# ru-wang/slam-plus-plus

Measured on AMD Instinct MI355X. Metric: Λ-solve block-nnz/sec + batch GN iters/sec, Venice BA, 1→8 MI355X, higher is better.
Workload: dtype f64; 1 GPU; venice871-shaped synthetic BA (871 cams, 530304 points, 2838740 observations, LM-damped); nnzb=3369915, n=1596138, mode=schur+dense, n_reduced=5226, schur_pairs=12875640, parallelism=single GPU

## Files before the change

include/spp_hip.h:

```cpp
#ifndef SPP_HIP_H
#define SPP_HIP_H

#include <stddef.h>
#include <stdint.h>

#ifdef __cplusplus
extern "C" {
#endif

#define SPP_OK            0
#define SPP_NOT_POSDEF    1
#define SPP_E_BADARG     -1
#define SPP_E_NOMEM      -2
#define SPP_E_HIP        -3
#define SPP_E_NO_DEVICE  -4
#define SPP_E_STATE      -5
#define SPP_E_UNSUPPORTED -6

#define SPP_MODE_AUTO     0
#define SPP_MODE_SPARSE   1
#define SPP_MODE_SCHUR    2
#define SPP_MODE_SCHUR_SPARSE 3

#define SPP_FLAG_PROFILE  1
#define SPP_FLAG_SCHUR_PARTIAL 2

typedef struct spp_ctx spp_ctx;

spp_ctx *spp_create(int device, int flags);
void spp_destroy(spp_ctx *ctx);
int spp_free_memory(spp_ctx *ctx);
int spp_last_error(const spp_ctx *ctx, char *buf, size_t buf_size);
double *spp_host_staging(spp_ctx *ctx, int64_t n_doubles);
int spp_set_stream(spp_ctx *ctx, void *hip_stream);
int spp_synchronize(spp_ctx *ctx);

int spp_analyze(spp_ctx *ctx, int64_t nb, const int64_t *h_col_ptr, const int64_t *h_row_idx,
	const int64_t *h_blk_off, const int32_t *h_dim, int mode);

int spp_set_shard(spp_ctx *ctx, int rank, int world_size);

#define SPP_MODE_SCHUR_MIS 4

#define SPP_INFO_MODE           0
#define SPP_INFO_N              1
#define SPP_INFO_NNZB           2
#define SPP_INFO_NVALS          3
#define SPP_INFO_FACTOR_NNZ     4
#define SPP_INFO_FACTOR_FLOPS   5
#define SPP_INFO_N_REDUCED      6
#define SPP_INFO_N_POSES        7
#define SPP_INFO_N_LANDMARKS    8
#define SPP_INFO_SCHUR_PAIRS    9
#define SPP_INFO_N_OBS          10
#define SPP_INFO_SOLVE_BYTES    11
#define SPP_INFO_N_SUPERNODES   12
#define SPP_INFO_N_LEVELS       13
#define SPP_INFO_S_LD           14
#define SPP_INFO_S_NNZB         15
#define SPP_INFO_DENSE_STREAMED 16
#define SPP_INFO_LM_STREAM      17
#define SPP_INFO_BS_GROUPS      18
#define SPP_INFO_SCHUR_SIDE     19
#define SPP_INFO_S_CLEAR        20
#define SPP_INFO_S_DEVICE_PTR   21
#define SPP_INFO_ASM_HUB_CHUNK   22
int spp_get_info(const spp_ctx *ctx, int what, int64_t *out);
int spp_get_ordering(const spp_ctx *ctx, int64_t *h_order);
int64_t spp_sparse_fronts(const spp_ctx *ctx, int64_t capacity, int32_t *h, int32_t *w, int32_t *pad, int32_t *cls, int32_t *level,
	int32_t *parent, int32_t *team);

#define SPP_ORDER_AMD 0
#define SPP_ORDER_ND  1
int spp_block_ordering(int64_t nb, const int64_t *col_ptr, const int64_t *row_idx, int method, int64_t *h_order);

int spp_schur_plan_host(int64_t nb, const int32_t *dim, const int64_t *col_ptr, const int64_t *row_idx, int shard_rank,
	int shard_world, int sparse_S, int64_t *out, double *seconds);

int spp_factor_solve(spp_ctx *ctx, const double *h_vals, double *h_rhs_inout);

int spp_factor_solve_device(spp_ctx *ctx, const double *d_vals, double *d_rhs_inout);

int spp_schur_buffer_size(const spp_ctx *ctx, int64_t *n_doubles);
int spp_schur_form(spp_ctx *ctx, const double *d_vals, const double *d_rhs, double *d_S_rhs);
int spp_schur_finish(spp_ctx *ctx, const double *d_vals, double *d_S_rhs, double *d_rhs_inout);
int spp_schur_packed_size(const spp_ctx *ctx, int64_t *n_doubles);
int spp_schur_pack(spp_ctx *ctx, const double *d_S_rhs, double *d_packed);
int spp_schur_unpack(spp_ctx *ctx, const double *d_packed, double *d_S_rhs);

int spp_assemble_analyze(spp_ctx *ctx, int64_t nv, const int32_t *h_dim,
	int64_t ne, const int64_t *h_v0, const int64_t *h_v1, int d0, int d1, int rd,
	int64_t unary_vertex);
int spp_assemble_get_structure(const spp_ctx *ctx, int64_t *h_col_ptr, int64_t *h_row_idx,
	int64_t *h_blk_off);
int spp_assemble_device(spp_ctx *ctx, const double *d_J0, const double *d_J1,
	const double *d_Omega, const double *d_r, double damping, double *d_vals_out, double *d_eta_out);
int spp_assemble_set_edge_weights(spp_ctx *ctx, const double *d_w);
#define SPP_MAX_EDGE_GROUPS 4
int spp_assemble_analyze_groups(spp_ctx *ctx, int64_t nv, const int32_t *h_dim, int n_groups,
	const int64_t *h_ne, const int64_t *const *h_v0, const int64_t *const *h_v1, const int64_t *const *h_seq,
	const int32_t *h_d0, const int32_t *h_d1, const int32_t *h_rd, int64_t unary_vertex);
int spp_assemble_groups_device(spp_ctx *ctx, const double *const *d_J0, const double *const *d_J1,
	const double *const *d_Omega, const double *const *d_r, double damping, double *d_vals_out, double *d_eta_out);
int spp_assemble_set_group_edge_weights(spp_ctx *ctx, int group, const double *d_w);
int spp_assemble_analyze_ternary(spp_ctx *ctx, int64_t nv, const int32_t *h_dim, int64_t ne, const int64_t *h_v0,
	const int64_t *h_v1, const int64_t *h_v2, int d0, int d1, int d2, int live2, int rd, int64_t unary_vertex);
int spp_assemble_ternary_device(spp_ctx *ctx, const double *d_J0, const double *d_J1, const double *d_J2,
	const double *d_Omega, const double *d_r, double damping, double *d_vals_out, double *d_eta_out);
int spp_edge_robust_weights_device(spp_ctx *ctx, int64_t n_edges, int rd, int kind, double scale, double param,
	const double *d_r, double *d_w_out);

int spp_se2_linearize_device(spp_ctx *ctx, int64_t n_edges, const int32_t *d_v0, const int32_t *d_v1,
	const double *d_poses, const double *d_measurements, double *d_J0, double *d_J1, double *d_r);
int spp_se2_update_device(spp_ctx *ctx, int64_t n_vertices, double *d_poses, const double *d_dx, int apply,
	double *h_dx_norm2);

int spp_se2_linearize_at_device(spp_ctx *ctx, int64_t n_edges, const int64_t *d_off0, const int64_t *d_off1,
	const double *d_state, const double *d_measurements, double *d_J0, double *d_J1, double *d_r);
int spp_se2_rb_linearize_device(spp_ctx *ctx, int64_t n_edges, const int64_t *d_pose_off, const int64_t *d_lm_off,
	const double *d_state, const double *d_measurements, double *d_J0, double *d_J1, double *d_r);
int spp_slam2d_update_device(spp_ctx *ctx, int64_t n, double *d_state, const double *d_dx, int64_t n_pose_angles,
	const int64_t *d_angle_off, int apply, double *h_dx_norm2);

int spp_se3_linearize_device(spp_ctx *ctx, int64_t n_edges, const int32_t *d_v0, const int32_t *d_v1,
	const double *d_poses, const double *d_measurements, double *d_J0, double *d_J1, double *d_r);
int spp_se3_update_device(spp_ctx *ctx, int64_t n_vertices, double *d_poses, const double *d_dx, int apply,
	double *h_dx_norm2);

int spp_se3_linearize_at_device(spp_ctx *ctx, int64_t n_edges, const int64_t *d_off0, const int64_t *d_off1,
	const double *d_state, const double *d_measurements, double *d_J0, double *d_J1, double *d_r);
int spp_se3_xyz_linearize_device(spp_ctx *ctx, int64_t n_edges, const int64_t *d_pose_off, const int64_t *d_lm_off,
	const double *d_state, const double *d_measurements, double *d_J0, double *d_J1, double *d_r);
int spp_slam3d_update_device(spp_ctx *ctx, int64_t n, double *d_state, const double *d_dx, int64_t n_poses,
	const int64_t *d_pose_off, int apply, double *h_dx_norm2);

int spp_rocv_range_linearize_device(spp_ctx *ctx, int64_t n_edges, const int64_t *d_recv_off, const int64_t *d_lm_off,
	const double *d_state, const double *d_measurements, double *d_J0, double *d_J1, double *d_r);
int spp_rocv_cv_linearize_device(spp_ctx *ctx, int64_t n_edges, const int64_t *d_off0, const int64_t *d_off1,
	const double *d_state, const double *d_dt, double *d_J0, double *d_J1, double *d_r);

int spp_ba_linearize_device(spp_ctx *ctx, int64_t n_obs, const int32_t *d_cam_of, const int32_t *d_pt_of,
	const double *d_cams, const double *d_intrinsics, const double *d_points, const double *d_measurements,
	double *d_J0, double *d_J1, double *d_r);
int spp_ba_update_device(spp_ctx *ctx, int64_t n_cams, double *d_cams, const int64_t *d_cam_dxoff,
	int64_t n_points, double *d_points, const int64_t *d_pt_dxoff, const double *d_dx, int64_t n_dx, int apply,
	double *h_dx_norm2);

int spp_ba_stereo_linearize_device(spp_ctx *ctx, int64_t n_obs, const int32_t *d_cam_of, const int32_t *d_pt_of,
	const double *d_cams, const double *d_intrinsics, const double *d_points, const double *d_measurements,
	double *d_J0, double *d_J1, double *d_r);

int spp_ba_intrinsics_linearize_device(spp_ctx *ctx, int64_t n_obs, const int32_t *d_cam_of, const int32_t *d_pt_of,
	const int32_t *d_intr_of, const double *d_cams, const double *d_intrinsics, const double *d_points,
	const double *d_measurements, double *d_J0, double *d_J1, double *d_J2, double *d_r);
int spp_ba_intrinsics_update_device(spp_ctx *ctx, int64_t n_intrinsics, double *d_intrinsics, const int64_t *d_intr_dxoff,
	const double *d_dx, int apply, double *h_dx_norm2);

int spp_edge_chi2_device(spp_ctx *ctx, int64_t n_edges, int rd, const double *d_r, const double *d_Omega, double *h_chi2);
int spp_edge_hessian_maxdiag_device(spp_ctx *ctx, int64_t n_edges, int rd, int d0, int d1, const double *d_J0,
	const double *d_J1, const double *d_Omega, double *h_max);
int spp_lm_gain_denominator_device(spp_ctx *ctx, int64_t n, const double *d_dx, const double *d_eta, double alpha,
	double *h_out);

int spp_device_malloc(spp_ctx *ctx, size_t bytes, void **d_ptr);
int spp_device_free(spp_ctx *ctx, void *d_ptr);
int spp_memcpy_h2d(spp_ctx *ctx, void *d_dst, const void *h_src, size_t bytes);
int spp_memcpy_d2h(spp_ctx *ctx, void *h_dst, const void *d_src, size_t bytes);
int spp_memcpy_d2d(spp_ctx *ctx, void *d_dst, const void *d_src, size_t bytes);

int spp_set_profiling(spp_ctx *ctx, int on);

#define SPP_PHASE_PERMUTE   0
#define SPP_PHASE_SCHUR_INV 1
#define SPP_PHASE_SCHUR_GEMM 2
#define SPP_PHASE_SCHUR_RHS 3
#define SPP_PHASE_FACTOR    4
#define SPP_PHASE_TRISOLVE  5
#define SPP_PHASE_BACKSUBST 6
#define SPP_PHASE_ASSEMBLE  7
#define SPP_PHASE_TOTAL     8
#define SPP_N_PHASES        9
int spp_get_phase_ms(spp_ctx *ctx, double *ms_out );
int spp_get_dominant_kernel(spp_ctx *ctx, double *ms_total, int64_t *n_launches, double *flops);

int spp_microbench_copy(spp_ctx *ctx, size_t bytes, int iters, double *gb_per_s);
int spp_microbench_mfma_f64(spp_ctx *ctx, int iters, double *tflops);
int spp_microbench_ctile(spp_ctx *ctx, int n, int iters, double *gb_per_s);
int spp_microbench_update(spp_ctx *ctx, int64_t m, int iters, double *ms_per_launch);

int spp_dense_potrf_upper(spp_ctx *ctx, double *d_A, int64_t n, int64_t ld);
int spp_dense_posv(spp_ctx *ctx, double *d_A, int64_t n, int64_t ld, double *d_b);
int spp_dense_posv_masked(spp_ctx *ctx, double *d_A, int64_t n, int64_t ld, double *d_b, const uint64_t *words, int64_t nwords);
int spp_tile_mask_host(int64_t n, int bs, int64_t nblk, const int32_t *i1, const int32_t *i2, int has_rhs, int fill,
	uint64_t *words, int64_t *n_updates);
int spp_schur_tile_mask_host(int64_t nb, const int32_t *dim, const int64_t *col_ptr, const int64_t *row_idx, int shard_rank,
	int shard_world, uint64_t *words);
int spp_schur_cam_order_host(int64_t nb, const int32_t *dim, const int64_t *col_ptr, const int64_t *row_idx, int shard_rank,
	int shard_world, int flags, const int64_t *order_in, int64_t *cam_order, double *figures);
int spp_tail_order_host(int64_t n, int has_rhs, const uint64_t *words, int64_t nwords, int resident, int early, double beta,
	int32_t *table, int32_t *info);
int spp_dense_gemm_tn_sub(spp_ctx *ctx, int64_t m, int64_t n, int64_t k,
	const double *d_A, int64_t lda, const double *d_B, int64_t ldb, double *d_C, int64_t ldc);
int spp_dense_gemm_tn_sub_upper(spp_ctx *ctx, int64_t m, int64_t n, int64_t k,
	const double *d_A, int64_t lda, const double *d_B, int64_t ldb, double *d_C, int64_t ldc);
int spp_dense_front_factor(spp_ctx *ctx, double *d_F, int64_t ld, int64_t w, int64_t h, double *d_image);

const char *spp_version(void);

#ifdef __cplusplus
}
#endif
#endif
```

slam_plus_plus_amd/api.py:

```python
import ctypes
import os

import numpy as np

_HERE = os.path.dirname(os.path.abspath(__file__))
LIB_PATH = os.environ.get("SPP_LIB") or os.path.join(_HERE, "libspp_hip.so")

SPP_OK, SPP_NOT_POSDEF = 0, 1
MODE_AUTO, MODE_SPARSE, MODE_SCHUR, MODE_SCHUR_SPARSE, MODE_SCHUR_MIS = 0, 1, 2, 3, 4
FLAG_PROFILE = 1
INFO = dict(MODE=0, N=1, NNZB=2, NVALS=3, FACTOR_NNZ=4, FACTOR_FLOPS=5, N_REDUCED=6, N_POSES=7,
            N_LANDMARKS=8, SCHUR_PAIRS=9, N_OBS=10, SOLVE_BYTES=11, N_SUPERNODES=12, N_LEVELS=13, S_LD=14, S_NNZB=15, DENSE_STREAMED=16,
            LM_STREAM=17, BS_GROUPS=18, SCHUR_SIDE=19, S_CLEAR=20, S_DEVICE_PTR=21, ASM_HUB_CHUNK=22)
PHASES = ["permute", "schur_inv", "schur_gemm", "schur_rhs", "factor", "trisolve", "backsubst", "assemble", "total"]

EXPORTS = [
    "spp_create", "spp_destroy", "spp_free_memory", "spp_last_error", "spp_host_staging", "spp_set_stream", "spp_synchronize",
    "spp_analyze", "spp_set_shard", "spp_get_info", "spp_get_ordering", "spp_sparse_fronts", "spp_factor_solve",
    "spp_factor_solve_device", "spp_schur_buffer_size", "spp_schur_form", "spp_schur_finish",
    "spp_schur_packed_size", "spp_schur_pack", "spp_schur_unpack",
    "spp_assemble_analyze", "spp_assemble_get_structure", "spp_assemble_device", "spp_assemble_set_edge_weights",
    "spp_assemble_analyze_groups", "spp_assemble_groups_device", "spp_assemble_set_group_edge_weights",
    "spp_assemble_analyze_ternary", "spp_assemble_ternary_device", "spp_ba_intrinsics_linearize_device",
    "spp_ba_intrinsics_update_device",
    "spp_se2_linearize_at_device", "spp_se2_rb_linearize_device", "spp_slam2d_update_device",
    "spp_se3_linearize_at_device", "spp_se3_xyz_linearize_device", "spp_slam3d_update_device", "spp_rocv_range_linearize_device",
    "spp_rocv_cv_linearize_device", "spp_device_malloc",
    "spp_device_free", "spp_memcpy_h2d", "spp_memcpy_d2h", "spp_memcpy_d2d", "spp_get_phase_ms", "spp_get_dominant_kernel",
    "spp_microbench_copy", "spp_microbench_mfma_f64", "spp_microbench_ctile", "spp_microbench_update", "spp_block_ordering", "spp_schur_plan_host", "spp_set_profiling", "spp_se2_linearize_device", "spp_se2_update_device", "spp_ba_linearize_device", "spp_ba_stereo_linearize_device", "spp_ba_update_device", "spp_se3_linearize_device", "spp_se3_update_device", "spp_edge_chi2_device", "spp_edge_robust_weights_device", "spp_edge_hessian_maxdiag_device",
    "spp_lm_gain_denominator_device", "spp_dense_potrf_upper", "spp_dense_posv",
    "spp_dense_posv_masked", "spp_tile_mask_host", "spp_schur_tile_mask_host", "spp_tail_order_host", "spp_schur_cam_order_host",
    "spp_dense_gemm_tn_sub", "spp_dense_gemm_tn_sub_upper", "spp_dense_front_factor", "spp_version",
]

_lib = None
_c_i64p = ctypes.POINTER(ctypes.c_int64)
_c_i32p = ctypes.POINTER(ctypes.c_int32)
_c_f64p = ctypes.POINTER(ctypes.c_double)


class SppError(RuntimeError):
    """std::runtime_error of the C++ adapter (reference LinearSolver_Schur_GPU.cpp:734-797)."""


def load_library():
    global _lib
    if _lib is not None:
        return _lib
    if not os.path.exists(LIB_PATH):
        raise SppError("libspp_hip.so is not built: run `python -m slam_plus_plus_amd.build` "
                       "(hipcc --offload-arch=gfx950); there is no CPU fallback")
    lib = ctypes.CDLL(LIB_PATH)
    vp, i64, i32, dbl, cint = ctypes.c_void_p, ctypes.c_int64, ctypes.c_int32, ctypes.c_double, ctypes.c_int
    sig = {
        "spp_create": (vp, [cint, cint]),
        "spp_destroy": (None, [vp]),
        "spp_free_memory": (cint, [vp]),
        "spp_last_error": (cint, [vp, ctypes.c_char_p, ctypes.c_size_t]),
        "spp_host_staging": (vp, [vp, i64]),
        "spp_set_stream": (cint, [vp, vp]),
        "spp_synchronize": (cint, [vp]),
        "spp_analyze": (cint, [vp, i64, vp, vp, vp, vp, cint]),
        "spp_set_shard": (cint, [vp, cint, cint]),
        "spp_get_info": (cint, [vp, cint, _c_i64p]),
        "spp_get_ordering": (cint, [vp, vp]),
        "spp_sparse_fronts": (i64, [vp, i64, vp, vp, vp, vp, vp, vp, vp]),
        "spp_factor_solve": (cint, [vp, vp, vp]),
        "spp_factor_solve_device": (cint, [vp, vp, vp]),
        "spp_schur_buffer_size": (cint, [vp, _c_i64p]),
        "spp_schur_form": (cint, [vp, vp, vp, vp]),
        "spp_schur_finish": (cint, [vp, vp, vp, vp]),
        "spp_schur_packed_size": (cint, [vp, _c_i64p]),
        "spp_schur_pack": (cint, [vp, vp, vp]),
        "spp_schur_unpack": (cint, [vp, vp, vp]),
        "spp_assemble_analyze": (cint, [vp, i64, vp, i64, vp, vp, cint, cint, cint, i64]),
        "spp_assemble_get_structure": (cint, [vp, vp, vp, vp]),
        "spp_assemble_device": (cint, [vp, vp, vp, vp, vp, dbl, vp, vp]),
        "spp_assemble_set_edge_weights": (cint, [vp, vp]),
        "spp_assemble_analyze_groups": (cint, [vp, i64, vp, cint, vp, vp, vp, vp, vp, vp, vp, i64]),
        "spp_assemble_groups_device": (cint, [vp, vp, vp, vp, vp, dbl, vp, vp]),
        "spp_assemble_set_group_edge_weights": (cint, [vp, cint, vp]),
        "spp_assemble_analyze_ternary": (cint, [vp, i64, vp, i64, vp, vp, vp, cint, cint, cint, cint, cint, i64]),
        "spp_assemble_ternary_device": (cint, [vp, vp, vp, vp, vp, vp, dbl, vp, vp]),
        "spp_ba_intrinsics_linearize_device": (cint, [vp, i64, vp, vp, vp, vp, vp, vp, vp, vp, vp, vp, vp]),
        "spp_ba_intrinsics_update_device": (cint, [vp, i64, vp, vp, vp, cint, _c_f64p]),
        "spp_se2_linearize_at_device": (cint, [vp, i64, vp, vp, vp, vp, vp, vp, vp]),
        "spp_se2_rb_linearize_device": (cint, [vp, i64, vp, vp, vp, vp, vp, vp, vp]),
        "spp_slam2d_update_device": (cint, [vp, i64, vp, vp, i64, vp, cint, _c_f64p]),
        "spp_se3_linearize_at_device": (cint, [vp, i64, vp, vp, vp, vp, vp, vp, vp]),
        "spp_se3_xyz_linearize_device": (cint, [vp, i64, vp, vp, vp, vp, vp, vp, vp]),
        "spp_slam3d_update_device": (cint, [vp, i64, vp, vp, i64, vp, cint, _c_f64p]),
        "spp_rocv_range_linearize_device": (cint, [vp, i64, vp, vp, vp, vp, vp, vp, vp]),
        "spp_rocv_cv_linearize_device": (cint, [vp, i64, vp, vp, vp, vp, vp, vp, vp]),
        "spp_device_malloc": (cint, [vp, ctypes.c_size_t, ctypes.POINTER(vp)]),
        "spp_device_free": (cint, [vp, vp]),
        "spp_memcpy_h2d": (cint, [vp, vp, vp, ctypes.c_size_t]),
        "spp_memcpy_d2h": (cint, [vp, vp, vp, ctypes.c_size_t]),
        "spp_memcpy_d2d": (cint, [vp, vp, vp, ctypes.c_size_t]),
        "spp_get_phase_ms": (cint, [vp, _c_f64p]),
        "spp_get_dominant_kernel": (cint, [vp, _c_f64p, _c_i64p, _c_f64p]),
        "spp_microbench_copy": (cint, [vp, ctypes.c_size_t, cint, _c_f64p]),
        "spp_microbench_mfma_f64": (cint, [vp, cint, _c_f64p]),
        "spp_microbench_ctile": (cint, [vp, cint, cint, _c_f64p]),
        "spp_microbench_update": (cint, [vp, ctypes.c_int64, cint, _c_f64p]),
        "spp_block_ordering": (cint, [ctypes.c_int64, vp, vp, cint, vp]),
        "spp_schur_plan_host": (cint, [ctypes.c_int64, vp, vp, vp, cint, cint, cint, vp, vp]),
        "spp_set_profiling": (cint, [vp, cint]),
        "spp_se2_linearize_device": (cint, [vp, ctypes.c_int64, vp, vp, vp, vp, vp, vp, vp]),
        "spp_se2_update_device": (cint, [vp, ctypes.c_int64, vp, vp, cint, _c_f64p]),
        "spp_se3_linearize_device": (cint, [vp, ctypes.c_int64, vp, vp, vp, vp, vp, vp, vp]),
        "spp_se3_update_device": (cint, [vp, ctypes.c_int64, vp, vp, cint, _c_f64p]),
        "spp_edge_chi2_device": (cint, [vp, ctypes.c_int64, cint, vp, vp, _c_f64p]),
        "spp_edge_robust_weights_device": (cint, [vp, ctypes.c_int64, cint, cint, dbl, dbl, vp, vp]),
        "spp_edge_hessian_maxdiag_device": (cint, [vp, ctypes.c_int64, cint, cint, cint, vp, vp, vp, _c_f64p]),
        "spp_lm_gain_denominator_device": (cint, [vp, ctypes.c_int64, vp, vp, ctypes.c_double, _c_f64p]),
        "spp_ba_linearize_device": (cint, [vp, ctypes.c_int64, vp, vp, vp, vp, vp, vp, vp, vp, vp]),
        "spp_ba_stereo_linearize_device": (cint, [vp, ctypes.c_int64, vp, vp, vp, vp, vp, vp, vp, vp, vp]),
        "spp_ba_update_device": (cint, [vp, ctypes.c_int64, vp, vp, ctypes.c_int64, vp, vp, vp, ctypes.c_int64, cint, _c_f64p]),
        "spp_dense_potrf_upper": (cint, [vp, vp, i64, i64]),
        "spp_dense_posv": (cint, [vp, vp, i64, i64, vp]),
        "spp_dense_posv_masked": (cint, [vp, vp, i64, i64, vp, vp, i64]),
        "spp_tile_mask_host": (cint, [i64, cint, i64, vp, vp, cint, cint, vp, vp]),
        "spp_schur_tile_mask_host": (cint, [i64, vp, vp, vp, cint, cint, vp]),
        "spp_tail_order_host": (cint, [i64, cint, vp, i64, cint, cint, dbl, vp, vp]),
        "spp_schur_cam_order_host": (cint, [i64, vp, vp, vp, cint, cint, cint, vp, vp, vp]),
        "spp_dense_gemm_tn_sub": (cint, [vp, i64, i64, i64, vp, i64, vp, i64, vp, i64]),
        "spp_dense_gemm_tn_sub_upper": (cint, [vp, i64, i64, i64, vp, i64, vp, i64, vp, i64]),
        "spp_dense_front_factor": (cint, [vp, vp, i64, i64, i64, vp]),
        "spp_version": (ctypes.c_char_p, []),
    }
    for name, (res, args) in sig.items():
        fn = getattr(lib, name)
        fn.restype = res
        fn.argtypes = args
    _lib = lib
    return lib


def _ptr(a):
    return a.ctypes.data_as(ctypes.c_void_p)


ORDER_AMD, ORDER_ND = 0, 1


def block_ordering(lam, method=ORDER_AMD):
    lib = load_library()
    col_ptr = np.ascontiguousarray(lam.col_ptr, dtype=np.int64)
    row_idx = np.ascontiguousarray(lam.row_idx, dtype=np.int64)
    out = np.empty(lam.nb, dtype=np.int64)
    code = lib.spp_block_ordering(lam.nb, _ptr(col_ptr), _ptr(row_idx), method, _ptr(out))
    if code != 0:
        raise SppError("spp_block_ordering failed: %d" % code)
    return out


def schur_plan_host(lam, shard_rank=0, shard_world=1, sparse_S=False, mis=False):
    lib = load_library()
    col_ptr = np.ascontiguousarray(lam.col_ptr, dtype=np.int64)
    row_idx = np.ascontiguousarray(lam.row_idx, dtype=np.int64)
    dim = np.ascontiguousarray(lam.dim, dtype=np.int32)
    out = np.zeros(9, dtype=np.int64)
    sec = ctypes.c_double(0.0)
    code = lib.spp_schur_plan_host(lam.nb, _ptr(dim), _ptr(col_ptr), _ptr(row_idx), shard_rank, shard_world,
                                   (1 if sparse_S else 0) | (2 if mis else 0), _ptr(out), ctypes.byref(sec))
    if code != 0:
# ... 435 lines not shown
```

slam_plus_plus_amd/csrc/spp_api.cpp:

```cpp

#include "spp_internal.h"
#include <string.h>
#include <new>

using namespace spp;

namespace spp {

void phases_reset(spp_ctx *ctx)
{
	if(!(ctx->flags & SPP_FLAG_PROFILE))
		return;
	if(!ctx->timer.created) {
		for(int i = 0; i < 2 * SPP_N_PHASES; ++ i)
			SPP_HIP_CHECK(hipEventCreate(&ctx->timer.ev[i]));
		ctx->timer.created = true;
	}
	for(int i = 0; i < SPP_N_PHASES; ++ i) {
		ctx->timer.used[i] = false;
		ctx->phase_ms[i] = 0;
	}
	ctx->dom_used = 0;
	ctx->dom_flops = 0;
}

void phase_begin(spp_ctx *ctx, int phase)
{
	if(!(ctx->flags & SPP_FLAG_PROFILE) || !ctx->timer.created)
		return;
	SPP_HIP_CHECK(hipEventRecord(ctx->timer.ev[2 * phase], ctx->stream));
}

void phase_end(spp_ctx *ctx, int phase)
{
	if(!(ctx->flags & SPP_FLAG_PROFILE) || !ctx->timer.created)
		return;
	SPP_HIP_CHECK(hipEventRecord(ctx->timer.ev[2 * phase + 1], ctx->stream));
	ctx->timer.used[phase] = true;
}

void phases_collect(spp_ctx *ctx)
{
	if(!(ctx->flags & SPP_FLAG_PROFILE) || !ctx->timer.created)
		return;
	SPP_HIP_CHECK(hipStreamSynchronize(ctx->stream));
	for(int i = 0; i < SPP_N_PHASES; ++ i) {
		if(!ctx->timer.used[i])
			continue;
		float ms = 0;
		if(hipEventElapsedTime(&ms, ctx->timer.ev[2 * i], ctx->timer.ev[2 * i + 1]) == hipSuccess)
			ctx->phase_ms[i] = ms;
	}
}

void dom_begin(spp_ctx *ctx)
{
	if(!(ctx->flags & SPP_FLAG_PROFILE))
		return;
	if(ctx->dom_used + 2 > ctx->dom_events.size()) {
		size_t old = ctx->dom_events.size();
		ctx->dom_events.resize(old + 64);
		for(size_t i = old; i < ctx->dom_events.size(); ++ i)
			SPP_HIP_CHECK(hipEventCreate(&ctx->dom_events[i]));
	}
	SPP_HIP_CHECK(hipEventRecord(ctx->dom_events[ctx->dom_used], ctx->stream));
}

void dom_end(spp_ctx *ctx, double flops)
{
	if(!(ctx->flags & SPP_FLAG_PROFILE))
		return;
	SPP_HIP_CHECK(hipEventRecord(ctx->dom_events[ctx->dom_used + 1], ctx->stream));
	ctx->dom_used += 2;
	ctx->dom_flops += flops;
}

}

#define SPP_TRY(ctx) try {
#define SPP_CATCH(ctx) } catch(const spp::Error &e) { if(ctx) (ctx)->last_error = e.what(); return e.code; } \
	catch(const std::bad_alloc &) { if(ctx) (ctx)->last_error = "host allocation failed"; return SPP_E_NOMEM; } \
	catch(const std::exception &e) { if(ctx) (ctx)->last_error = e.what(); return SPP_E_HIP; }

static inline void store_if(double *h_out, double value)
{
	if(h_out)
		*h_out = value;
}

template <class Body>
static int geometry_call(spp_ctx *ctx, Body body)
{
	SPP_TRY(ctx)
	SPP_HIP_CHECK(hipSetDevice(ctx->device));
	body();
	return SPP_OK;
	SPP_CATCH(ctx)
}

extern "C" {

const char *spp_version(void)
{
	return "slam_plus_plus_amd 0.1 (gfx950, fp64)";
}

spp_ctx *spp_create(int device, int flags)
{
	int count = 0;
	if(hipGetDeviceCount(&count) != hipSuccess || count <= 0 || device < 0 || device >= count)
		return nullptr;
	if(hipSetDevice(device) != hipSuccess)
		return nullptr;
	spp_ctx *ctx = new(std::nothrow) spp_ctx;
	if(!ctx)
		return nullptr;
	ctx->device = device;
	ctx->flags = flags;
	if(hipStreamCreateWithFlags(&ctx->stream, hipStreamNonBlocking) != hipSuccess) {
		delete ctx;
		return nullptr;
	}
	ctx->own_stream = true;
	return ctx;
}

int spp_free_memory(spp_ctx *ctx)
{
	if(!ctx)
		return SPP_E_BADARG;
	SPP_TRY(ctx)
	(void)hipSetDevice(ctx->device);
	(void)hipStreamSynchronize(ctx->stream);
	ctx->schur.release_all();
	sparse_release(ctx);
	assemble_release(ctx);
	ctx->dense.tinv.release();
	ctx->dense.tinv_all.release();
	ctx->dense.xtmp.release();
	ctx->dense.la_cnt.release();
	ctx->dense.la_trace.release();
	ctx->geom_partial.release();
	ctx->dense.flags.release();
	ctx->dense.trsv_pay.release();
	ctx->dense.trsv_m.release();
	ctx->dense.tail_pub.release();
	ctx->dense.tail_order.release();
	ctx->dense.tail_order_tr = ctx->dense.tail_order_tc = 0;
	ctx->dense.tail_order_bits.clear();
	ctx->dense.tail_dinv.release();
	ctx->dense.tail_epoch = 0;
	ctx->dense.epoch = 0;
	ctx->dense.sync.release();
	ctx->dense.fuse_cnt.release();
	ctx->dense.fuse_expect.clear();
	ctx->dense.sync_epoch = 0;
	ctx->d_vals.release();
	ctx->d_rhs.release();
	ctx->mode = -1;
	return SPP_OK;
	SPP_CATCH(ctx)
}

void spp_destroy(spp_ctx *ctx)
{
	if(!ctx)
		return;
	if(ctx->plan_trash.joinable())
		ctx->plan_trash.join();
	spp_free_memory(ctx);
	ctx->dense.info.release();
	if(ctx->dense.aux) {
		dense_aux_park(ctx->device, ctx->dense.aux);
		(void)hipEventDestroy(ctx->dense.ev[0]);
		(void)hipEventDestroy(ctx->dense.ev[1]);
	}
	if(ctx->dense.chain) {
		(void)hipStreamDestroy(ctx->dense.chain);
		if(ctx->dense.ev_chain)
			(void)hipEventDestroy(ctx->dense.ev_chain);
	}
	if(ctx->side_stream) {
		(void)hipStreamDestroy(ctx->side_stream);
		(void)hipEventDestroy(ctx->side_ev[0]);
		(void)hipEventDestroy(ctx->side_ev[1]);
	}
	if(ctx->dense.h_chain_err)
		(void)hipHostFree(ctx->dense.h_chain_err);
	if(ctx->h_staging)
		(void)hipHostFree(ctx->h_staging);
	if(ctx->timer.created)
		for(int i = 0; i < 2 * SPP_N_PHASES; ++ i)
			(void)hipEventDestroy(ctx->timer.ev[i]);
	for(size_t i = 0; i < ctx->dom_events.size(); ++ i)
		(void)hipEventDestroy(ctx->dom_events[i]);
	if(ctx->own_stream && ctx->stream)
		(void)hipStreamDestroy(ctx->stream);
	delete ctx;
}

int spp_last_error(const spp_ctx *ctx, char *buf, size_t buf_size)
{
	if(!ctx || !buf || !buf_size)
		return SPP_E_BADARG;
	strncpy(buf, ctx->last_error.c_str(), buf_size - 1);
	buf[buf_size - 1] = 0;
	return SPP_OK;
}

double *spp_host_staging(spp_ctx *ctx, int64_t n_doubles)
{
	if(!ctx || n_doubles < 0)
		return nullptr;
	if((size_t)n_doubles <= ctx->h_staging_cap && ctx->h_staging)
		return ctx->h_staging;
	(void)hipSetDevice(ctx->device);
	(void)hipStreamSynchronize(ctx->stream);
	if(ctx->h_staging) {
		(void)hipHostFree(ctx->h_staging);
		ctx->h_staging = nullptr;
		ctx->h_staging_cap = 0;
	}
	const size_t want = (size_t)(n_doubles > 0 ? n_doubles : 1);
	if(hipHostMalloc((void**)&ctx->h_staging, want * sizeof(double), hipHostMallocDefault) != hipSuccess) {
		(void)hipGetLastError();
		ctx->h_staging = nullptr;
		ctx->last_error = "hipHostMalloc of the staging buffer failed";
		return nullptr;
	}
	ctx->h_staging_cap = want;
	return ctx->h_staging;
}

int spp_set_stream(spp_ctx *ctx, void *hip_stream)
{
	if(!ctx)
		return SPP_E_BADARG;
	(void)hipStreamSynchronize(ctx->stream);
	if(ctx->own_stream && ctx->stream)
		(void)hipStreamDestroy(ctx->stream);
	ctx->stream = (hipStream_t)hip_stream;
	ctx->own_stream = false;
	return SPP_OK;
}

int spp_synchronize(spp_ctx *ctx)
{
	if(!ctx)
		return SPP_E_BADARG;
	SPP_TRY(ctx)
	SPP_HIP_CHECK(hipStreamSynchronize(ctx->stream));
	dense_chain_check(ctx);
	return SPP_OK;
	SPP_CATCH(ctx)
}

int spp_set_profiling(spp_ctx *ctx, int on)
{
	if(!ctx)
		return SPP_E_BADARG;
	ctx->flags = on ? (ctx->flags | SPP_FLAG_PROFILE) : (ctx->flags & ~SPP_FLAG_PROFILE);
	return SPP_OK;
}

int spp_set_shard(spp_ctx *ctx, int rank, int world_size)
{
	if(!ctx || world_size < 1 || rank < 0 || rank >= world_size)
		return SPP_E_BADARG;
	ctx->shard_rank = rank;
	ctx->shard_world = world_size;
	return SPP_OK;
}

int spp_analyze(spp_ctx *ctx, int64_t nb, const int64_t *col_ptr, const int64_t *row_idx,
	const int64_t *blk_off, const int32_t *dim, int mode)
{
	if(!ctx)
		return SPP_E_BADARG;
	SPP_TRY(ctx)
	SPP_REQUIRE(nb > 0 && col_ptr && row_idx && blk_off && dim, SPP_E_BADARG, "spp_analyze: null or empty structure");
	SPP_REQUIRE(col_ptr[0] == 0 && col_ptr[nb] >= nb, SPP_E_BADARG, "spp_analyze: column pointers must start at 0 and hold every diagonal block");
	SPP_HIP_CHECK(hipSetDevice(ctx->device));
	ctx->mode = -1;
	VClock clk("spp_analyze");
	Structure st;
	st.nb = nb;
	st.nnzb = col_ptr[nb];
	st.col_ptr.assign(col_ptr, col_ptr + nb + 1);
	SPP_REQUIRE(st.nnzb >= nb, SPP_E_BADARG, "spp_analyze: fewer blocks than block columns");
	for(int64_t j = 0; j < nb; ++ j)
		SPP_REQUIRE(col_ptr[j + 1] > col_ptr[j], SPP_E_BADARG, "every block column needs its diagonal block");
	st.dim.assign(dim, dim + nb);
	st.base.resize(nb + 1);
	st.base[0] = 0;
	for(int64_t j = 0; j < nb; ++ j) {
		SPP_REQUIRE(dim[j] > 0 && dim[j] <= 8, SPP_E_BADARG, "block widths must be in 1..8");
		st.base[j + 1] = st.base[j] + dim[j];
	}
	st.n = st.base[nb];
	st.row_idx.resize(st.nnzb);
	st.blk_off.resize(st.nnzb);
	{
		const int nt = plan_threads(st.nnzb);
		std::vector<int64_t> jcut, nvals_t(nt, 0);
		balanced_cuts(st.col_ptr, nt, jcut);
		run_threads(nt, [&](int t) {
			const int64_t p0 = col_ptr[jcut[t]], p1 = col_ptr[jcut[t + 1]];
			if(p1 > p0) {
				memcpy(st.row_idx.data() + p0, row_idx + p0, (size_t)(p1 - p0) * sizeof(int64_t));
				memcpy(st.blk_off.data() + p0, blk_off + p0, (size_t)(p1 - p0) * sizeof(int64_t));
			}
			int64_t nv = 0;
			for(int64_t j = jcut[t]; j < jcut[t + 1]; ++ j) {
				for(int64_t p = col_ptr[j]; p < col_ptr[j + 1]; ++ p) {
					const int64_t i = row_idx[p];
					SPP_REQUIRE(i >= 0 && i <= j, SPP_E_BADARG, "only the upper triangle may be stored");
					SPP_REQUIRE(p == col_ptr[j] || row_idx[p - 1] < i, SPP_E_BADARG, "rows must ascend within a column");
					SPP_REQUIRE(blk_off[p] >= 0, SPP_E_BADARG, "negative block offset");
					nv = std::max<int64_t>(nv, blk_off[p] + (int64_t)dim[i] * dim[j]);
				}
				SPP_REQUIRE(row_idx[col_ptr[j + 1] - 1] == j, SPP_E_BADARG, "diagonal block missing (must be last in its column)");
			}
			nvals_t[t] = nv;
		});
		st.nvals = 0;
		for(int t = 0; t < nt; ++ t)
			st.nvals = std::max(st.nvals, nvals_t[t]);
	}
	ctx->st = std::move(st);
	Structure &st_ref = ctx->st;
	clk.lap("structure copied + validated");
	ctx->schur.release_all();
	sparse_release(ctx);
	clk.lap("old plans released");
	int dp, dl;
	int chosen = mode;
	if(mode == SPP_MODE_AUTO) {
		chosen = SPP_MODE_SPARSE;
		if(schur_applicable(st_ref, &dp, &dl)) {
			int64_t n_red = 0;
			for(int64_t j = 0; j < nb; ++ j)
				n_red += (dim[j] == dp) ? dp : 0;
			chosen = (n_red <= 16384) ? SPP_MODE_SCHUR : SPP_MODE_SCHUR_SPARSE;
		}
	}
	SPP_REQUIRE(chosen == SPP_MODE_SCHUR || chosen == SPP_MODE_SPARSE || chosen == SPP_MODE_SCHUR_SPARSE ||
		chosen == SPP_MODE_SCHUR_MIS, SPP_E_BADARG, "unknown mode");
	SPP_REQUIRE((chosen != SPP_MODE_SPARSE && chosen != SPP_MODE_SCHUR_MIS) || ctx->shard_world == 1, SPP_E_UNSUPPORTED,
		"only the Schur modes shard (over landmarks); pose graphs run as replicas (DESIGN.md, multi-GPU)");
	ctx->mode = -1;
	if(chosen == SPP_MODE_SCHUR || chosen == SPP_MODE_SCHUR_SPARSE || chosen == SPP_MODE_SCHUR_MIS) {
		const bool mis = chosen == SPP_MODE_SCHUR_MIS;
		const bool sparse_S = chosen != SPP_MODE_SCHUR;
		build_schur_plan(ctx, sparse_S, mis);
		clk.lap("schur plan (all of it)");
		ctx->schur.mis = mis;
		ctx->order.clear();
		ctx->order.reserve((size_t)st_ref.nb);
		if(sparse_S) {
			sparse_analyze(ctx, ctx->schur.s_st);
			std::vector<int64_t> red = ctx->order;
			ctx->order.clear();
			for(size_t i = 0; i < red.size(); ++ i)
				ctx->order.push_back(ctx->schur.pose_block[red[i]]);
			chosen = SPP_MODE_SCHUR;
		} else
		for(size_t i = 0; i < ctx->schur.pose_block.size(); ++ i)
			ctx->order.push_back(ctx->schur.pose_block[i]);
		for(int64_t j = 0; j < st_ref.nb; ++ j)
			if(ctx->schur.is_lm[j])
				ctx->order.push_back(j);
	} else
		sparse_analyze(ctx, ctx->st);
	ctx->mode = chosen;
	clk.lap("plan + ordering");
	return SPP_OK;
	SPP_CATCH(ctx)
}

int spp_get_info(const spp_ctx *ctx, int what, int64_t *out)
{
	if(!ctx || !out)
		return SPP_E_BADARG;
	if(ctx->mode < 0 && what != SPP_INFO_NNZB && what != SPP_INFO_NVALS && what != SPP_INFO_N && what != SPP_INFO_DENSE_STREAMED &&
	   what != SPP_INFO_ASM_HUB_CHUNK)
		return SPP_E_STATE;
	switch(what) {
	case SPP_INFO_MODE: *out = (ctx->mode != SPP_MODE_SCHUR) ? ctx->mode : ctx->schur.mis ? SPP_MODE_SCHUR_MIS :
		ctx->schur.sparse_S ? SPP_MODE_SCHUR_SPARSE : SPP_MODE_SCHUR; break;
	case SPP_INFO_N: *out = ctx->st.n; break;
	case SPP_INFO_NNZB: *out = ctx->st.nnzb; break;
	case SPP_INFO_NVALS: *out = ctx->st.nvals; break;
	case SPP_INFO_FACTOR_NNZ: *out = ctx->factor_nnz; break;
	case SPP_INFO_FACTOR_FLOPS: *out = ctx->factor_flops; break;
	case SPP_INFO_N_REDUCED: *out = (ctx->mode == SPP_MODE_SCHUR) ? ctx->schur.n_red : 0; break;
	case SPP_INFO_N_POSES: *out = (ctx->mode == SPP_MODE_SCHUR) ? ctx->schur.nc : ctx->st.nb; break;
	case SPP_INFO_N_LANDMARKS: *out = (ctx->mode == SPP_MODE_SCHUR) ? ctx->schur.nl : 0; break;
	case SPP_INFO_SCHUR_PAIRS: *out = (ctx->mode == SPP_MODE_SCHUR) ? ctx->schur.n_pairs : 0; break;
	case SPP_INFO_N_OBS: *out = (ctx->mode == SPP_MODE_SCHUR) ? ctx->schur.no : 0; break;
	case SPP_INFO_SOLVE_BYTES: *out = ctx->solve_bytes; break;
	case SPP_INFO_N_SUPERNODES: *out = ctx->sparse ? sparse_info(ctx, what) : 0; break;
	case SPP_INFO_N_LEVELS: *out = ctx->sparse ? sparse_info(ctx, what) : 0; break;
	case SPP_INFO_S_LD: *out = (ctx->mode == SPP_MODE_SCHUR && !ctx->schur.sparse_S) ? ctx->schur.ld : 0; break;
	case SPP_INFO_S_NNZB: *out = (ctx->mode == SPP_MODE_SCHUR) ? ctx->schur.n_sblk : 0; break;
	case SPP_INFO_DENSE_STREAMED: *out = ctx->dense.tail_rows_last; break;
	case SPP_INFO_LM_STREAM: *out = (ctx->mode == SPP_MODE_SCHUR) ? ctx->schur.lm_stream_last : 0; break;
	case SPP_INFO_BS_GROUPS: *out = (ctx->mode == SPP_MODE_SCHUR) ? ctx->schur.n_bs : 0; break;
	case SPP_INFO_SCHUR_SIDE: *out = (ctx->mode == SPP_MODE_SCHUR) ? ctx->schur.side_last : 0; break;
	case SPP_INFO_S_CLEAR: *out = (ctx->mode == SPP_MODE_SCHUR) ? ctx->schur.clear_last : 0; break;
	case SPP_INFO_S_DEVICE_PTR: *out = (ctx->mode == SPP_MODE_SCHUR) ? (int64_t)(uintptr_t)ctx->schur.S.p : 0; break;
	case SPP_INFO_ASM_HUB_CHUNK: *out = ASM_HUB_CHUNK; break;
	default: return SPP_E_BADARG;
	}
	return SPP_OK;
}

int spp_get_ordering(const spp_ctx *ctx, int64_t *h_order)
{
	if(!ctx || !h_order)
		return SPP_E_BADARG;
	if(ctx->mode < 0)
		return SPP_E_STATE;
	for(size_t i = 0; i < ctx->order.size(); ++ i)
		h_order[i] = ctx->order[i];
	return SPP_OK;
}

int64_t spp_sparse_fronts(const spp_ctx *ctx, int64_t capacity, int32_t *h, int32_t *w, int32_t *pad, int32_t *cls, int32_t *level,
	int32_t *parent, int32_t *team)
{
	if(!ctx || capacity < 0)
		return SPP_E_BADARG;
#ifdef SPP_HAVE_SPARSE
	if(ctx->sparse)
		return sparse_fronts(ctx, capacity, h, w, pad, cls, level, parent, team);
#endif
	return 0;
}

int spp_block_ordering(int64_t nb, const int64_t *col_ptr, const int64_t *row_idx, int method, int64_t *h_order)
{
	if(nb <= 0 || !col_ptr || !row_idx || !h_order || (method != SPP_ORDER_AMD && method != SPP_ORDER_ND))
		return SPP_E_BADARG;
	try {
		for(int64_t j = 0; j < nb; ++ j)
			for(int64_t p = col_ptr[j]; p < col_ptr[j + 1]; ++ p)
				if(row_idx[p] < 0 || row_idx[p] > j)
					return SPP_E_BADARG;
		std::vector<int64_t> order;
		if(method == SPP_ORDER_AMD)
			min_degree_order(nb, col_ptr, row_idx, order);
		else
			nested_dissection_order(nb, col_ptr, row_idx, order);
		for(int64_t k = 0; k < nb; ++ k)
			h_order[k] = order[k];
		return SPP_OK;
	} catch(const std::bad_alloc &) {
		return SPP_E_NOMEM;
	} catch(...) {
		return SPP_E_HIP;
	}
}

static bool structure_of_pattern(int64_t nb, const int32_t *dim, const int64_t *col_ptr, const int64_t *row_idx, Structure &st)
{
	st.nb = nb;
	st.nnzb = col_ptr[nb];
	st.col_ptr.assign(col_ptr, col_ptr + nb + 1);
	st.row_idx.assign(row_idx, row_idx + st.nnzb);
	st.dim.assign(dim, dim + nb);
	st.base.resize(nb + 1);
	st.base[0] = 0;
	for(int64_t j = 0; j < nb; ++ j)
		st.base[j + 1] = st.base[j] + dim[j];
	st.n = st.base[nb];
	st.blk_off.resize(st.nnzb);
	int64_t off = 0;
	for(int64_t j = 0; j < nb; ++ j)
		for(int64_t p = col_ptr[j]; p < col_ptr[j + 1]; ++ p) {
			if(row_idx[p] < 0 || row_idx[p] > j)
				return false;
			st.blk_off[p] = off;
			off += (int64_t)dim[row_idx[p]] * dim[j];
		}
	st.nvals = off;
	return true;
}

extern "C++" {
template <class F>
static int schur_host_entry(int64_t nb, const int32_t *dim, const int64_t *col_ptr, const int64_t *row_idx, int shard_rank,
	int shard_world, const void *out, F fn)
{
	if(nb <= 0 || !dim || !col_ptr || !row_idx || !out || shard_world < 1 || shard_rank < 0 || shard_rank >= shard_world)
		return SPP_E_BADARG;
	try {
		Structure st;
		if(!structure_of_pattern(nb, dim, col_ptr, row_idx, st))
			return SPP_E_BADARG;
		return fn(st);
	} catch(const Error &e) {
		return e.code;
	} catch(const std::bad_alloc &) {
		return SPP_E_NOMEM;
	} catch(...) {
		return SPP_E_HIP;
	}
}
}

int spp_schur_plan_host(int64_t nb, const int32_t *dim, const int64_t *col_ptr, const int64_t *row_idx, int shard_rank,
	int shard_world, int sparse_S, int64_t *out, double *seconds)
{
	return schur_host_entry(nb, dim, col_ptr, row_idx, shard_rank, shard_world, out, [&](const Structure &st) {
		const double sec = schur_plan_host_probe(st, shard_rank, shard_world, (sparse_S & 1) != 0, (sparse_S & 2) != 0, out);
		if(seconds)
			*seconds = sec;
		return (int)SPP_OK;
	});
}

int spp_schur_tile_mask_host(int64_t nb, const int32_t *dim, const int64_t *col_ptr, const int64_t *row_idx, int shard_rank,
	int shard_world, uint64_t *words)
{
	return schur_host_entry(nb, dim, col_ptr, row_idx, shard_rank, shard_world, words, [&](const Structure &st) {
		std::vector<uint64_t> w;
		schur_tile_mask_host_probe(st, w);
		for(size_t q = 0; q < w.size(); ++ q)
			words[q] = w[q];
		return (int)w.size();
	});
}

int spp_schur_cam_order_host(int64_t nb, const int32_t *dim, const int64_t *col_ptr, const int64_t *row_idx, int shard_rank,
	int shard_world, int flags, const int64_t *order_in, int64_t *cam_order, double *figures)
{
	if(!figures)
		return SPP_E_BADARG;
	return schur_host_entry(nb, dim, col_ptr, row_idx, shard_rank, shard_world, cam_order, [&](const Structure &st) {
		if(order_in) {
			int64_t nc = 0;
			const int dmax = *std::max_element(dim, dim + nb);
			for(int64_t j = 0; j < nb; ++ j)
				nc += dim[j] == dmax;
			std::vector<char> seen((size_t)nc, 0);
			for(int64_t q = 0; q < nc; ++ q) {
				if(order_in[q] < 0 || order_in[q] >= nc || seen[order_in[q]])
					return (int)SPP_E_BADARG;
				seen[order_in[q]] = 1;
			}
		}
		std::vector<int32_t> order;
		TileDagCost cost[2];
		const bool used = schur_cam_order_host_probe(st, shard_rank, shard_world, (flags & 1) != 0, (flags & 2) != 0, order_in, order, cost);
		for(size_t q = 0; q < order.size(); ++ q)
			cam_order[q] = order[q];
		for(int side = 0; side < 2; ++ side) {
			figures[4 * side] = (double)cost[side].tiles;
			figures[4 * side + 1] = (double)cost[side].updates;
			figures[4 * side + 2] = (double)cost[side].path;
			figures[4 * side + 3] = cost[side].cost_us;
		}
		return used ? 1 : 0;
	});
}

int spp_schur_buffer_size(const spp_ctx *ctx, int64_t *n_doubles)
{
	if(!ctx || !n_doubles)
		return SPP_E_BADARG;
	if(ctx->mode != SPP_MODE_SCHUR)
		return SPP_E_STATE;
	*n_doubles = schur_buffer_doubles(ctx);
	return SPP_OK;
}

int spp_schur_form(spp_ctx *ctx, const double *d_vals, const double *d_rhs, double *d_S_rhs)
{
	if(!ctx || !d_vals || !d_rhs || !d_S_rhs)
		return SPP_E_BADARG;
	SPP_TRY(ctx)
	SPP_REQUIRE(ctx->mode == SPP_MODE_SCHUR, SPP_E_STATE, "spp_schur_form: analyze in Schur mode first");
	SPP_HIP_CHECK(hipSetDevice(ctx->device));
	phases_reset(ctx);
	phase_begin(ctx, SPP_PHASE_TOTAL);
	schur_form(ctx, d_vals, d_rhs, d_S_rhs);
	return SPP_OK;
	SPP_CATCH(ctx)
}

int spp_schur_packed_size(const spp_ctx *ctx, int64_t *n_doubles)
{
	if(!ctx || !n_doubles)
		return SPP_E_BADARG;
	if(ctx->mode != SPP_MODE_SCHUR)
		return SPP_E_STATE;
	if(ctx->schur.sparse_S) {
		*n_doubles = schur_buffer_doubles(ctx);
		return SPP_OK;
	}
	const int64_t nblk = ctx->schur.ld / DENSE_NB;
	*n_doubles = (int64_t)DENSE_NB * DENSE_NB * (nblk * (nblk + 1) / 2);
	return SPP_OK;
}

int spp_schur_pack(spp_ctx *ctx, const double *d_S_rhs, double *d_packed)
{
	if(!ctx || !d_S_rhs || !d_packed)
		return SPP_E_BADARG;
	SPP_TRY(ctx)
	SPP_REQUIRE(ctx->mode == SPP_MODE_SCHUR, SPP_E_STATE, "spp_schur_pack: analyze in Schur mode first");
	SPP_HIP_CHECK(hipSetDevice(ctx->device));
	if(ctx->schur.sparse_S)
		SPP_HIP_CHECK(hipMemcpyAsync(d_packed, d_S_rhs, (size_t)schur_buffer_doubles(ctx) * sizeof(double),
			hipMemcpyDeviceToDevice, ctx->stream));
	else
		schur_pack(ctx, const_cast<double*>(d_S_rhs), d_packed, true);
	return SPP_OK;
	SPP_CATCH(ctx)
}

int spp_schur_unpack(spp_ctx *ctx, const double *d_packed, double *d_S_rhs)
{
	if(!ctx || !d_S_rhs || !d_packed)
		return SPP_E_BADARG;
	SPP_TRY(ctx)
	SPP_REQUIRE(ctx->mode == SPP_MODE_SCHUR, SPP_E_STATE, "spp_schur_unpack: analyze in Schur mode first");
	SPP_HIP_CHECK(hipSetDevice(ctx->device));
	if(ctx->schur.sparse_S)
		SPP_HIP_CHECK(hipMemcpyAsync(d_S_rhs, d_packed, (size_t)schur_buffer_doubles(ctx) * sizeof(double),
			hipMemcpyDeviceToDevice, ctx->stream));
	else
		schur_pack(ctx, d_S_rhs, const_cast<double*>(d_packed), false);
	return SPP_OK;
	SPP_CATCH(ctx)
}

int spp_schur_finish(spp_ctx *ctx, const double *d_vals, double *d_S_rhs, double *d_rhs_inout)
{
	if(!ctx || !d_vals || !d_rhs_inout || !d_S_rhs)
		return SPP_E_BADARG;
	SPP_TRY(ctx)
	SPP_REQUIRE(ctx->mode == SPP_MODE_SCHUR, SPP_E_STATE, "spp_schur_finish: analyze in Schur mode first");
	SPP_HIP_CHECK(hipSetDevice(ctx->device));
	int ret = schur_finish(ctx, d_vals, d_S_rhs, d_rhs_inout);
	phase_end(ctx, SPP_PHASE_TOTAL);
	phases_collect(ctx);
	dense_chain_check(ctx);
	return ret;
	SPP_CATCH(ctx)
}

int spp_factor_solve_device(spp_ctx *ctx, const double *d_vals, double *d_rhs)
{
	if(!ctx || !d_vals || !d_rhs)
		return SPP_E_BADARG;
	SPP_TRY(ctx)
	SPP_REQUIRE(ctx->mode >= 0, SPP_E_STATE, "spp_factor_solve: call spp_analyze first");
	SPP_HIP_CHECK(hipSetDevice(ctx->device));
	phases_reset(ctx);
	phase_begin(ctx, SPP_PHASE_TOTAL);
	int ret;
	if(ctx->mode == SPP_MODE_SCHUR) {
		SPP_REQUIRE(ctx->shard_world == 1, SPP_E_STATE,
			"sharded ctx: use spp_schur_form / all-reduce / spp_schur_finish");
		if(!ctx->schur.S.p || ctx->schur.S.cap < (size_t)schur_buffer_doubles(ctx))
			ctx->schur.unlisted_dirty = true;
		ctx->schur.S.reserve((size_t)schur_buffer_doubles(ctx));
		schur_form(ctx, d_vals, d_rhs, ctx->schur.S.p, true);
		ret = schur_finish(ctx, d_vals, ctx->schur.S.p, d_rhs);
	} else
		ret = sparse_factor_solve(ctx, d_vals, d_rhs);
	phase_end(ctx, SPP_PHASE_TOTAL);
	phases_collect(ctx);
	SPP_HIP_CHECK(hipStreamSynchronize(ctx->stream));
	dense_chain_check(ctx);
	return ret;
	SPP_CATCH(ctx)
}

int spp_factor_solve(spp_ctx *ctx, const double *h_vals, double *h_rhs)
{
	if(!ctx || !h_vals || !h_rhs)
		return SPP_E_BADARG;
	SPP_TRY(ctx)
	SPP_REQUIRE(ctx->mode >= 0, SPP_E_STATE, "spp_factor_solve: call spp_analyze first");
	SPP_HIP_CHECK(hipSetDevice(ctx->device));
	ctx->d_vals.reserve((size_t)ctx->st.nvals);
	ctx->d_rhs.reserve((size_t)ctx->st.n);
	SPP_HIP_CHECK(hipMemcpyAsync(ctx->d_vals.p, h_vals, ctx->st.nvals * sizeof(double), hipMemcpyHostToDevice, ctx->stream));
	SPP_HIP_CHECK(hipMemcpyAsync(ctx->d_rhs.p, h_rhs, ctx->st.n * sizeof(double), hipMemcpyHostToDevice, ctx->stream));
	int ret = spp_factor_solve_device(ctx, ctx->d_vals.p, ctx->d_rhs.p);
	if(ret != SPP_OK)
		return ret;
	SPP_HIP_CHECK(hipMemcpyAsync(h_rhs, ctx->d_rhs.p, ctx->st.n * sizeof(double), hipMemcpyDeviceToHost, ctx->stream));
	SPP_HIP_CHECK(hipStreamSynchronize(ctx->stream));
	return SPP_OK;
	SPP_CATCH(ctx)
}

int spp_assemble_analyze(spp_ctx *ctx, int64_t nv, const int32_t *h_dim, int64_t ne, const int64_t *h_v0,
	const int64_t *h_v1, int d0, int d1, int rd, int64_t unary_vertex)
{
	if(!ctx)
		return SPP_E_BADARG;
	assemble_release(ctx);
	if(!h_dim || !h_v0 || !h_v1 || nv <= 0 || ne <= 0)
		return SPP_E_BADARG;
	SPP_TRY(ctx)
	SPP_HIP_CHECK(hipSetDevice(ctx->device));
	assemble_analyze(ctx, nv, h_dim, 1, &ne, &h_v0, &h_v1, nullptr, &d0, &d1, &rd, unary_vertex);
	return SPP_OK;
	SPP_CATCH(ctx)
}

int spp_assemble_analyze_groups(spp_ctx *ctx, int64_t nv, const int32_t *h_dim, int n_groups, const int64_t *h_ne,
	const int64_t *const *h_v0, const int64_t *const *h_v1, const int64_t *const *h_seq, const int32_t *h_d0,
	const int32_t *h_d1, const int32_t *h_rd, int64_t unary_vertex)
{
	if(!ctx)
		return SPP_E_BADARG;
	assemble_release(ctx);
	if(!h_dim || nv <= 0 || n_groups <= 0 || !h_ne || !h_v0 || !h_v1 || !h_d0 || !h_d1 || !h_rd)
		return SPP_E_BADARG;
	SPP_TRY(ctx)
	SPP_HIP_CHECK(hipSetDevice(ctx->device));
	SPP_REQUIRE(n_groups <= SPP_MAX_EDGE_GROUPS, SPP_E_UNSUPPORTED, "more than SPP_MAX_EDGE_GROUPS edge groups");
	int64_t total = 0;
	for(int g = 0; g < n_groups; ++ g) {
		SPP_REQUIRE(h_ne[g] >= 0 && (!h_ne[g] || (h_v0[g] && (h_v1[g] || h_d1[g] == 0))), SPP_E_BADARG, "edge group without vertex arrays");
		total += h_ne[g];
	}
	SPP_REQUIRE(total > 0, SPP_E_BADARG, "no edges");
	assemble_analyze(ctx, nv, h_dim, n_groups, h_ne, h_v0, h_v1, h_seq, h_d0, h_d1, h_rd, unary_vertex);
	return SPP_OK;
	SPP_CATCH(ctx)
}

int spp_assemble_get_structure(const spp_ctx *ctx, int64_t *h_col_ptr, int64_t *h_row_idx, int64_t *h_blk_off)
{
	if(!ctx || !ctx->assemble)
		return SPP_E_STATE;
	assemble_get_structure(ctx, h_col_ptr, h_row_idx, h_blk_off);
	return SPP_OK;
}

int spp_assemble_device(spp_ctx *ctx, const double *d_J0, const double *d_J1, const double *d_Omega,
	const double *d_r, double damping, double *d_vals_out, double *d_eta_out)
{
	if(!ctx || !d_J0 || !d_J1 || !d_Omega || !d_r || !d_vals_out || !d_eta_out)
		return SPP_E_BADARG;
	SPP_TRY(ctx)
	SPP_REQUIRE(ctx->assemble, SPP_E_STATE, "spp_assemble_device: call spp_assemble_analyze first");
	SPP_REQUIRE(assemble_n_groups(ctx) == 1, SPP_E_STATE, "spp_assemble_device: the plan has several edge groups (spp_assemble_groups_device)");
	SPP_REQUIRE(!assemble_is_ternary(ctx), SPP_E_STATE, "spp_assemble_device: the plan is one of ternary edges (spp_assemble_ternary_device)");
	SPP_REQUIRE(!assemble_group_is_unary(ctx, 0), SPP_E_STATE, "spp_assemble_device: the plan is one of unary edges (spp_assemble_groups_device)");
	SPP_HIP_CHECK(hipSetDevice(ctx->device));
	phases_reset(ctx);
	phase_begin(ctx, SPP_PHASE_ASSEMBLE);
	assemble_run(ctx, d_J0, d_J1, d_Omega, d_r, damping, d_vals_out, d_eta_out);
	phase_end(ctx, SPP_PHASE_ASSEMBLE);
	phases_collect(ctx);
	return SPP_OK;
	SPP_CATCH(ctx)
}

int spp_assemble_groups_device(spp_ctx *ctx, const double *const *d_J0, const double *const *d_J1,
	const double *const *d_Omega, const double *const *d_r, double damping, double *d_vals_out, double *d_eta_out)
{
	if(!ctx || !d_J0 || !d_J1 || !d_Omega || !d_r || !d_vals_out || !d_eta_out)
		return SPP_E_BADARG;
	SPP_TRY(ctx)
	SPP_REQUIRE(ctx->assemble, SPP_E_STATE, "spp_assemble_groups_device: call spp_assemble_analyze_groups first");
	SPP_REQUIRE(!assemble_is_ternary(ctx), SPP_E_STATE, "spp_assemble_groups_device: the plan is one of ternary edges (spp_assemble_ternary_device)");
	for(int g = 0; g < assemble_n_groups(ctx); ++ g)
		SPP_REQUIRE(!assemble_group_edges(ctx, g) || (d_J0[g] && (d_J1[g] || assemble_group_is_unary(ctx, g)) && d_Omega[g] && d_r[g]), SPP_E_BADARG,
			"spp_assemble_groups_device: null array of an edge group");
	SPP_HIP_CHECK(hipSetDevice(ctx->device));
	phases_reset(ctx);
	phase_begin(ctx, SPP_PHASE_ASSEMBLE);
	assemble_groups_run(ctx, d_J0, d_J1, d_Omega, d_r, damping, d_vals_out, d_eta_out);
	phase_end(ctx, SPP_PHASE_ASSEMBLE);
	phases_collect(ctx);
	return SPP_OK;
	SPP_CATCH(ctx)
}

int spp_assemble_analyze_ternary(spp_ctx *ctx, int64_t nv, const int32_t *h_dim, int64_t ne, const int64_t *h_v0,
	const int64_t *h_v1, const int64_t *h_v2, int d0, int d1, int d2, int live2, int rd, int64_t unary_vertex)
{
	if(!ctx)
		return SPP_E_BADARG;
	assemble_release(ctx);
	if(!h_dim || !h_v0 || !h_v1 || !h_v2 || nv <= 0 || ne <= 0)
		return SPP_E_BADARG;
	SPP_TRY(ctx)
	SPP_REQUIRE(d0 == 6 && d1 == 3 && d2 == 6 && live2 == 5 && rd == 2, SPP_E_UNSUPPORTED,
		"ternary edge shape (d0, d1, d2, rd) / live2 not instantiated: (6,3,6,2) / 5");
	SPP_HIP_CHECK(hipSetDevice(ctx->device));
	assemble_analyze_ternary(ctx, nv, h_dim, ne, h_v0, h_v1, h_v2, unary_vertex);
	return SPP_OK;
	SPP_CATCH(ctx)
}

int spp_assemble_ternary_device(spp_ctx *ctx, const double *d_J0, const double *d_J1, const double *d_J2,
	const double *d_Omega, const double *d_r, double damping, double *d_vals_out, double *d_eta_out)
{
	if(!ctx || !d_J0 || !d_J1 || !d_J2 || !d_Omega || !d_r || !d_vals_out || !d_eta_out)
		return SPP_E_BADARG;
	SPP_TRY(ctx)
	SPP_REQUIRE(ctx->assemble && assemble_is_ternary(ctx), SPP_E_STATE, "spp_assemble_ternary_device: call spp_assemble_analyze_ternary first");
	SPP_HIP_CHECK(hipSetDevice(ctx->device));
	phases_reset(ctx);
	phase_begin(ctx, SPP_PHASE_ASSEMBLE);
	assemble_ternary_run(ctx, d_J0, d_J1, d_J2, d_Omega, d_r, damping, d_vals_out, d_eta_out);
	phase_end(ctx, SPP_PHASE_ASSEMBLE);
	phases_collect(ctx);
	return SPP_OK;
	SPP_CATCH(ctx)
}

int spp_ba_intrinsics_linearize_device(spp_ctx *ctx, int64_t n_obs, const int32_t *d_cam_of, const int32_t *d_pt_of,
	const int32_t *d_intr_of, const double *d_cams, const double *d_intrinsics, const double *d_points,
	const double *d_measurements, double *d_J0, double *d_J1, double *d_J2, double *d_r)
{
	if(!ctx || n_obs < 0 || !d_cam_of || !d_pt_of || !d_intr_of || !d_cams || !d_intrinsics || !d_points || !d_measurements ||
	   !d_J0 || !d_J1 || !d_J2 || !d_r)
		return SPP_E_BADARG;
	return geometry_call(ctx, [&] {
		ba_intrinsics_linearize(ctx, n_obs, d_cam_of, d_pt_of, d_intr_of, d_cams, d_intrinsics, d_points, d_measurements, d_J0, d_J1,
			d_J2, d_r);
	});
}

int spp_ba_intrinsics_update_device(spp_ctx *ctx, int64_t n_intrinsics, double *d_intrinsics, const int64_t *d_intr_dxoff,
	const double *d_dx, int apply, double *h_dx_norm2)
{
	if(!ctx || n_intrinsics < 0 || !d_dx || (n_intrinsics && (!d_intrinsics || !d_intr_dxoff)))
		return SPP_E_BADARG;
	return geometry_call(ctx, [&] { store_if(h_dx_norm2, ba_intrinsics_update(ctx, n_intrinsics, d_intrinsics, d_intr_dxoff, d_dx, apply != 0)); });
}

int spp_assemble_set_edge_weights(spp_ctx *ctx, const double *d_w)
{
	if(!ctx)
		return SPP_E_BADARG;
	SPP_TRY(ctx)
	SPP_REQUIRE(ctx->assemble, SPP_E_STATE, "spp_assemble_set_edge_weights: call spp_assemble_analyze first");
	SPP_REQUIRE(!assemble_is_ternary(ctx), SPP_E_UNSUPPORTED, "robust weights on ternary edges");
// ... 63 lines not shown
	return geometry_call(ctx, [&] { se3_linearize(ctx, n_edges, d_v0, d_v1, d_poses, d_measurements, d_J0, d_J1, d_r); });
}

int spp_se3_update_device(spp_ctx *ctx, int64_t n_vertices, double *d_poses, const double *d_dx, int apply,
	double *h_dx_norm2)
{
	if(!ctx || n_vertices < 0 || !d_poses || !d_dx)
		return SPP_E_BADARG;
	return geometry_call(ctx, [&] { store_if(h_dx_norm2, se3_update(ctx, n_vertices, d_poses, d_dx, apply != 0)); });
}

int spp_ba_linearize_device(spp_ctx *ctx, int64_t n_obs, const int32_t *d_cam_of, const int32_t *d_pt_of,
	const double *d_cams, const double *d_intrinsics, const double *d_points, const double *d_measurements,
	double *d_J0, double *d_J1, double *d_r)
{
	if(!ctx || n_obs < 0 || !d_cam_of || !d_pt_of || !d_cams || !d_intrinsics || !d_points || !d_measurements ||
	   !d_J0 || !d_J1 || !d_r)
		return SPP_E_BADARG;
	return geometry_call(ctx, [&] { ba_linearize(ctx, n_obs, d_cam_of, d_pt_of, d_cams, d_intrinsics, d_points, d_measurements, d_J0, d_J1, d_r); });
}

int spp_ba_stereo_linearize_device(spp_ctx *ctx, int64_t n_obs, const int32_t *d_cam_of, const int32_t *d_pt_of,
	const double *d_cams, const double *d_intrinsics, const double *d_points, const double *d_measurements,
	double *d_J0, double *d_J1, double *d_r)
{
	if(!ctx || n_obs < 0 || !d_cam_of || !d_pt_of || !d_cams || !d_intrinsics || !d_points || !d_measurements ||
	   !d_J0 || !d_J1 || !d_r)
		return SPP_E_BADARG;
	return geometry_call(ctx, [&] { ba_stereo_linearize(ctx, n_obs, d_cam_of, d_pt_of, d_cams, d_intrinsics, d_points, d_measurements, d_J0, d_J1, d_r); });
}

int spp_ba_update_device(spp_ctx *ctx, int64_t n_cams, double *d_cams, const int64_t *d_cam_dxoff,
	int64_t n_points, double *d_points, const int64_t *d_pt_dxoff, const double *d_dx, int64_t n_dx, int apply,
	double *h_dx_norm2)
{
	if(!ctx || n_cams < 0 || n_points < 0 || n_dx < 0 || !d_dx || (n_cams && (!d_cams || !d_cam_dxoff)) ||
	   (n_points && (!d_points || !d_pt_dxoff)))
		return SPP_E_BADARG;
	return geometry_call(ctx, [&] { store_if(h_dx_norm2, ba_update(ctx, n_cams, d_cams, d_cam_dxoff, n_points, d_points, d_pt_dxoff, d_dx, n_dx, apply != 0)); });
}

int spp_edge_robust_weights_device(spp_ctx *ctx, int64_t n_edges, int rd, int kind, double scale, double param,
	const double *d_r, double *d_w_out)
{
	if(!ctx || n_edges < 0 || !d_r || !d_w_out)
		return SPP_E_BADARG;
	return geometry_call(ctx, [&] { edge_robust_weights(ctx, n_edges, rd, kind, scale, param, d_r, d_w_out); });
}

int spp_se3_linearize_at_device(spp_ctx *ctx, int64_t n_edges, const int64_t *d_off0, const int64_t *d_off1,
	const double *d_state, const double *d_measurements, double *d_J0, double *d_J1, double *d_r)
{
	if(!ctx || n_edges < 0 || !d_off0 || !d_off1 || !d_state || !d_measurements || !d_J0 || !d_J1 || !d_r)
		return SPP_E_BADARG;
	return geometry_call(ctx, [&] { se3_linearize_at(ctx, n_edges, d_off0, d_off1, d_state, d_measurements, d_J0, d_J1, d_r); });
}

int spp_se3_xyz_linearize_device(spp_ctx *ctx, int64_t n_edges, const int64_t *d_pose_off, const int64_t *d_lm_off,
	const double *d_state, const double *d_measurements, double *d_J0, double *d_J1, double *d_r)
{
	if(!ctx || n_edges < 0 || !d_pose_off || !d_lm_off || !d_state || !d_measurements || !d_J0 || !d_J1 || !d_r)
		return SPP_E_BADARG;
	return geometry_call(ctx, [&] { se3_xyz_linearize(ctx, n_edges, d_pose_off, d_lm_off, d_state, d_measurements, d_J0, d_J1, d_r); });
}

int spp_slam3d_update_device(spp_ctx *ctx, int64_t n, double *d_state, const double *d_dx, int64_t n_poses,
	const int64_t *d_pose_off, int apply, double *h_dx_norm2)
{
	if(!ctx || n < 0 || n_poses < 0 || !d_state || !d_dx || (n_poses && !d_pose_off))
		return SPP_E_BADARG;
	return geometry_call(ctx, [&] { store_if(h_dx_norm2, slam3d_update(ctx, n, d_state, d_dx, n_poses, d_pose_off, apply != 0)); });
}

int spp_rocv_range_linearize_device(spp_ctx *ctx, int64_t n_edges, const int64_t *d_recv_off, const int64_t *d_lm_off,
	const double *d_state, const double *d_measurements, double *d_J0, double *d_J1, double *d_r)
{
	if(!ctx || n_edges < 0 || !d_recv_off || !d_lm_off || !d_state || !d_measurements || !d_J0 || !d_J1 || !d_r)
		return SPP_E_BADARG;
	return geometry_call(ctx, [&] { rocv_range_linearize(ctx, n_edges, d_recv_off, d_lm_off, d_state, d_measurements, d_J0, d_J1, d_r); });
}

int spp_rocv_cv_linearize_device(spp_ctx *ctx, int64_t n_edges, const int64_t *d_off0, const int64_t *d_off1,
	const double *d_state, const double *d_dt, double *d_J0, double *d_J1, double *d_r)
{
	if(!ctx || n_edges < 0 || !d_off0 || !d_off1 || !d_state || !d_dt || !d_J0 || !d_J1 || !d_r)
		return SPP_E_BADARG;
	return geometry_call(ctx, [&] { rocv_cv_linearize(ctx, n_edges, d_off0, d_off1, d_state, d_dt, d_J0, d_J1, d_r); });
}

int spp_edge_chi2_device(spp_ctx *ctx, int64_t n_edges, int rd, const double *d_r, const double *d_Omega, double *h_chi2)
{
	if(!ctx || n_edges < 0 || !d_r || !d_Omega || !h_chi2)
		return SPP_E_BADARG;
	return geometry_call(ctx, [&] { *h_chi2 = edge_chi2(ctx, n_edges, rd, d_r, d_Omega); });
}

int spp_edge_hessian_maxdiag_device(spp_ctx *ctx, int64_t n_edges, int rd, int d0, int d1, const double *d_J0,
	const double *d_J1, const double *d_Omega, double *h_max)
{
	if(!ctx || n_edges < 0 || !d_J0 || !d_J1 || !d_Omega || !h_max)
		return SPP_E_BADARG;
	return geometry_call(ctx, [&] { *h_max = edge_hessian_maxdiag(ctx, n_edges, rd, d0, d1, d_J0, d_J1, d_Omega); });
}

int spp_lm_gain_denominator_device(spp_ctx *ctx, int64_t n, const double *d_dx, const double *d_eta, double alpha,
	double *h_out)
{
	if(!ctx || n < 0 || !d_dx || !d_eta || !h_out)
		return SPP_E_BADARG;
	return geometry_call(ctx, [&] { *h_out = lm_gain_denominator(ctx, n, d_dx, d_eta, alpha); });
}

int spp_device_malloc(spp_ctx *ctx, size_t bytes, void **d_ptr)
{
	if(!ctx || !d_ptr)
		return SPP_E_BADARG;
	(void)hipSetDevice(ctx->device);
	if(hipMalloc(d_ptr, bytes ? bytes : 8) != hipSuccess) {
		ctx->last_error = "hipMalloc failed";
		return SPP_E_NOMEM;
	}
	return SPP_OK;
}

int spp_device_free(spp_ctx *ctx, void *d_ptr)
{
	if(!ctx)
		return SPP_E_BADARG;
	(void)hipSetDevice(ctx->device);
	(void)hipStreamSynchronize(ctx->stream);
	return hipFree(d_ptr) == hipSuccess ? SPP_OK : SPP_E_HIP;
}

int spp_memcpy_h2d(spp_ctx *ctx, void *d_dst, const void *h_src, size_t bytes)
{
	if(!ctx)
		return SPP_E_BADARG;
	SPP_TRY(ctx)
	SPP_HIP_CHECK(hipSetDevice(ctx->device));
	SPP_HIP_CHECK(hipMemcpyAsync(d_dst, h_src, bytes, hipMemcpyHostToDevice, ctx->stream));
	SPP_HIP_CHECK(hipStreamSynchronize(ctx->stream));
	return SPP_OK;
	SPP_CATCH(ctx)
}

int spp_memcpy_d2h(spp_ctx *ctx, void *h_dst, const void *d_src, size_t bytes)
{
	if(!ctx)
		return SPP_E_BADARG;
	SPP_TRY(ctx)
	SPP_HIP_CHECK(hipSetDevice(ctx->device));
	SPP_HIP_CHECK(hipMemcpyAsync(h_dst, d_src, bytes, hipMemcpyDeviceToHost, ctx->stream));
	SPP_HIP_CHECK(hipStreamSynchronize(ctx->stream));
	return SPP_OK;
	SPP_CATCH(ctx)
}

int spp_memcpy_d2d(spp_ctx *ctx, void *d_dst, const void *d_src, size_t bytes)
{
	if(!ctx)
		return SPP_E_BADARG;
	SPP_TRY(ctx)
	SPP_HIP_CHECK(hipSetDevice(ctx->device));
	SPP_HIP_CHECK(hipMemcpyAsync(d_dst, d_src, bytes, hipMemcpyDeviceToDevice, ctx->stream));
	return SPP_OK;
	SPP_CATCH(ctx)
}

int spp_get_phase_ms(spp_ctx *ctx, double *ms_out)
{
	if(!ctx || !ms_out)
		return SPP_E_BADARG;
	for(int i = 0; i < SPP_N_PHASES; ++ i)
		ms_out[i] = ctx->phase_ms[i];
	return SPP_OK;
}

int spp_get_dominant_kernel(spp_ctx *ctx, double *ms_total, int64_t *n_launches, double *flops)
{
	if(!ctx || !ms_total || !n_launches || !flops)
		return SPP_E_BADARG;
	SPP_TRY(ctx)
	SPP_HIP_CHECK(hipStreamSynchronize(ctx->stream));
	double total = 0;
	for(size_t i = 0; i + 1 < ctx->dom_used; i += 2) {
		float ms = 0;
		SPP_HIP_CHECK(hipEventElapsedTime(&ms, ctx->dom_events[i], ctx->dom_events[i + 1]));
		total += ms;
	}
	*ms_total = total;
	*n_launches = (int64_t)(ctx->dom_used / 2);
	*flops = ctx->dom_flops;
	return SPP_OK;
	SPP_CATCH(ctx)
}

int spp_microbench_copy(spp_ctx *ctx, size_t bytes, int iters, double *gb_per_s)
{
	if(!ctx || !gb_per_s)
		return SPP_E_BADARG;
	SPP_TRY(ctx)
	SPP_HIP_CHECK(hipSetDevice(ctx->device));
	*gb_per_s = microbench_copy(ctx, bytes, iters);
	return SPP_OK;
	SPP_CATCH(ctx)
}

int spp_microbench_ctile(spp_ctx *ctx, int n, int iters, double *gb_per_s)
{
	if(!ctx || !gb_per_s)
		return SPP_E_BADARG;
	SPP_TRY(ctx)
	SPP_HIP_CHECK(hipSetDevice(ctx->device));
	*gb_per_s = microbench_ctile(ctx, n, iters);
	return SPP_OK;
	SPP_CATCH(ctx)
}

int spp_microbench_update(spp_ctx *ctx, int64_t m, int iters, double *ms_per_launch)
{
	if(!ctx || !ms_per_launch || m < 128 || iters < 1)
		return SPP_E_BADARG;
	SPP_TRY(ctx)
	SPP_HIP_CHECK(hipSetDevice(ctx->device));
	*ms_per_launch = microbench_update(ctx, m, iters);
	return SPP_OK;
	SPP_CATCH(ctx)
}

int spp_microbench_mfma_f64(spp_ctx *ctx, int iters, double *tflops)
{
	if(!ctx || !tflops)
		return SPP_E_BADARG;
	SPP_TRY(ctx)
	SPP_HIP_CHECK(hipSetDevice(ctx->device));
	*tflops = microbench_mfma_f64(ctx, iters);
	return SPP_OK;
	SPP_CATCH(ctx)
}

int spp_dense_potrf_upper(spp_ctx *ctx, double *d_A, int64_t n, int64_t ld)
{
	if(!ctx || !d_A || n <= 0 || ld < n)
		return SPP_E_BADARG;
	SPP_TRY(ctx)
	SPP_HIP_CHECK(hipSetDevice(ctx->device));
	const int64_t ldp = ((n + 1 + DENSE_NB - 1) / DENSE_NB) * DENSE_NB;
	DevBuf<double> tmp;
	tmp.reserve((size_t)ldp * ldp);
	SPP_HIP_CHECK(hipMemsetAsync(tmp.p, 0, (size_t)ldp * ldp * sizeof(double), ctx->stream));
	SPP_HIP_CHECK(hipMemcpy2DAsync(tmp.p, ldp * sizeof(double), d_A, ld * sizeof(double), n * sizeof(double), n,
		hipMemcpyDeviceToDevice, ctx->stream));
	dense_set_padding(ctx, tmp.p, ldp, n);
	int ret = dense_potrf_upper(ctx, tmp.p, n, ldp, true);
	SPP_HIP_CHECK(hipMemcpy2DAsync(d_A, ld * sizeof(double), tmp.p, ldp * sizeof(double), n * sizeof(double), n,
		hipMemcpyDeviceToDevice, ctx->stream));
	SPP_HIP_CHECK(hipStreamSynchronize(ctx->stream));
	return ret;
	SPP_CATCH(ctx)
}

int spp_dense_posv(spp_ctx *ctx, double *d_A, int64_t n, int64_t ld, double *d_b)
{
	return spp_dense_posv_masked(ctx, d_A, n, ld, d_b, nullptr, 0);
}

int spp_tile_mask_host(int64_t n, int bs, int64_t nblk, const int32_t *i1, const int32_t *i2, int has_rhs, int fill,
	uint64_t *words, int64_t *n_updates)
{
	if(n <= 0 || bs <= 0 || nblk < 0 || (nblk && (!i1 || !i2)) || !words)
		return SPP_E_BADARG;
	try {
		std::vector<uint64_t> w;
		tile_mask_mark(n, bs, nblk, i1, i2, w);
		const int64_t upd = tile_mask_close(n, has_rhs != 0, fill != 0, w);
		if(n_updates)
			*n_updates = upd;
		for(size_t q = 0; q < w.size(); ++ q)
			words[q] = w[q];
		return (int)w.size();
	} catch(...) {
		return SPP_E_NOMEM;
	}
}

int spp_tail_order_host(int64_t n, int has_rhs, const uint64_t *words, int64_t nwords, int resident, int early, double beta,
	int32_t *table, int32_t *info)
{
	const int64_t Tr = (n + DENSE_NB - 1) / DENSE_NB, Tc = has_rhs ? n / DENSE_NB + 1 : Tr;
	if(n <= 0 || Tr > 64 || Tc > 64 || nwords < 0 || (nwords && (!words || nwords != Tr)) || !table || !(beta >= 0))
		return SPP_E_BADARG;
	try {
		std::vector<uint64_t> bits((size_t)Tr + 1);
		const uint64_t all_cols = Tc == 64 ? ~0ull : (1ull << Tc) - 1;
		bits[0] = all_cols;
		for(int64_t i = 0; i < Tr; ++ i)
			bits[(size_t)i + 1] = (((nwords ? words[i] : all_cols) | (1ull << i)) & ~((1ull << i) - 1)) & all_cols;
		std::vector<int> order;
		int oinfo[5];
		const bool use = nwords && early;
		tail_order_table(bits, (int)Tr, (int)Tc, false, beta, use ? resident : 0, use, order, oinfo);
		for(size_t q = 0; q < order.size(); ++ q)
			table[q] = order[q];
		if(info)
			for(int q = 0; q < 5; ++ q)
				info[q] = oinfo[q];
// ... 79 lines not shown
```

slam_plus_plus_amd/csrc/spp_dense.hip:

```cpp

#include "spp_internal.h"
#include "spp_tiles.h"
#include "spp_dense_dev.h"
#include <stdio.h>
#include <stdlib.h>
#include <string.h>
#include <algorithm>
#include <vector>
#include <mutex>

namespace spp {


constexpr int BK = 16;
constexpr int LDS_STRIDE = 18;

template <int BM, int BN, int WM, int WN, int MODE, int DEPTH, int BKT, int SC1 = 0>
__device__ __forceinline__ void gemm_tn_tile(const int64_t m0, const int64_t n0, int64_t M, int64_t N, int K,
	const double *__restrict__ A, int64_t lda, const double *B, int64_t ldb, double *C, int64_t ldc, double *gemm_lds)
{
	constexpr int NWM = BM / WM, NWN = BN / WN, NT = NWM * NWN * 64;
	constexpr int TA = WM / 16, TB = WN / 16;
	constexpr int PPC = BKT / 2, LSTR = BKT + 2;
	constexpr int PA = (BM * PPC) / NT, PB = (BN * PPC) / NT;
// ... 358 lines not shown
		const int r = e & 63, c = e >> 6;
		T0[r + c * TF_STRIDE] = tv[r + (size_t)c * NB];
		R01[r + c * TF_STRIDE] = tv[r + (size_t)(64 + c) * NB];
		T1[r + c * TF_STRIDE] = tv[64 + r + (size_t)(64 + c) * NB];
	}
	__syncthreads();
	const int it = wave & 3, jt = wave >> 2;
	{
		v4f64 acc = (v4f64){0, 0, 0, 0};
		for(int kt = 0; kt <= jt; ++ kt) {
			const v4f64 m = tile_atb(R01 + 16 * it + 16 * kt * TF_STRIDE, TF_STRIDE, 1, T1 + 16 * kt + 16 * jt * TF_STRIDE, 1, TF_STRIDE, lane);
			acc += m;
		}
#pragma unroll
		for(int r = 0; r < 4; ++ r)
			Nm[16 * it + l4 + 4 * r + (16 * jt + l15) * TF_STRIDE] = acc[r];
	}
	__syncthreads();
	{
		v4f64 acc = (v4f64){0, 0, 0, 0};
		for(int kt = it; kt < 4; ++ kt) {
			const v4f64 m = tile_atb(T0 + 16 * it + 16 * kt * TF_STRIDE, TF_STRIDE, 1, Nm + 16 * kt + 16 * jt * TF_STRIDE, 1, TF_STRIDE, lane);
			acc += m;
		}
#pragma unroll
		for(int r = 0; r < 4; ++ r)
			tv[16 * it + l4 + 4 * r + (size_t)(64 + 16 * jt + l15) * NB] = -acc[r];
	}
}


__global__ __launch_bounds__(POTRF_THREADS)
void update_potrf_kernel(int64_t M, int64_t N, const double *P, int64_t ld, double *C, int nA, int target, int do_potrf,
	int n_valid, int has_rhs, double *tinv, int *info, int64_t k0_next, int *counter, int *abort, long long timeout_ticks)
{
	extern __shared__ double sm[];
	const int b = (int)blockIdx.x, tid = threadIdx.x;
	if(b < nA) {
		if(tid >= 256)
			return;
		const int ti = (int)((((M < NB) ? M : NB) + 31) >> 5);
		int j = 0, rem = b;
		for(;; ++ j) {
			const int cnt = ((j < ti - 1) ? j : ti - 1) + 1;
			if(rem < cnt)
				break;
			rem -= cnt;
		}
		gemm_tn_staged_tile<32, 32, 16, 16, 0, 0>((int64_t)rem * 32, (int64_t)j * 32, M, N, P, ld, P, ld, C, ld, sm);
		asm volatile("s_waitcnt vmcnt(0)" ::: "memory");
		__syncthreads();
		if(tid == 0) {
			__builtin_amdgcn_fence(__ATOMIC_RELEASE, "agent");
			asm volatile("s_waitcnt vmcnt(0)" ::: "memory");
			__hip_atomic_fetch_add(counter, 1, __ATOMIC_RELAXED, __HIP_MEMORY_SCOPE_AGENT);
		}
		return;
	}
	if(do_potrf && b == nA) {
		__shared__ int go;
		if(tid == 0) {
			const long long t0 = wall_clock64();
			int ok = 1;
			for(int it = 0; __hip_atomic_load(counter, __ATOMIC_RELAXED, __HIP_MEMORY_SCOPE_AGENT) < target; ++ it) {
				if((it & 15) == 15) {
					if(__hip_atomic_load(abort, __ATOMIC_RELAXED, __HIP_MEMORY_SCOPE_AGENT) != 0) {
						ok = 0;
						break;
					}
					if(wall_clock64() - t0 > timeout_ticks) {
						__hip_atomic_store(abort, 1, __ATOMIC_RELAXED, __HIP_MEMORY_SCOPE_AGENT);
						ok = 0;
						break;
					}
				}
				__builtin_amdgcn_s_sleep(1);
			}
			__builtin_amdgcn_fence(__ATOMIC_ACQUIRE, "agent");
			asm volatile("s_waitcnt vmcnt(0)" ::: "memory");
			go = ok;
		}
		__syncthreads();
		if(!go)
			return;
		potrf_diag_body<false, 0, 1>(C, ld, n_valid, has_rhs, tinv, info, k0_next, sm);
		return;
	}
	const int64_t q = b - nA - (do_potrf ? 1 : 0);
	const int64_t nbi = (M + 63) >> 6;
	const int64_t bi = q % nbi, bj = q / nbi;
	if(bi > bj || (bi < 2 && bj < 2))
		return;
	gemm_tn_staged_tile<64, 64, 16, 16, 0, 0>(bi * 64, bj * 64, M, N, P, ld, P, ld, C, ld, sm);
}

}
#include "spp_dense_la.h"
#include "spp_dense_tail.h"
namespace spp {

__global__ __launch_bounds__(256)
void trsv_back_kernel(const double *__restrict__ R, int64_t ld, int64_t k0, int nv, const double *__restrict__ tinv,
	double *__restrict__ y, double *__restrict__ xout)
{
	__shared__ double xk[NB];
	__shared__ double part[2][NB];
	const int tid = threadIdx.x;
	{
		const int r = tid & (NB - 1), h = tid >> 7;
		double s8[8] = {0, 0, 0, 0, 0, 0, 0, 0};
#pragma unroll
		for(int c8 = 0; c8 < 64; c8 += 8) {
#pragma unroll
			for(int u = 0; u < 8; ++ u) {
				const int c = h * 64 + c8 + u;
				const double t = tinv[r + c * NB], yy = y[k0 + c];
				s8[u] += (c < nv) ? t * yy : 0.0;
			}
		}
		part[h][r] = ((s8[0] + s8[1]) + (s8[2] + s8[3])) + ((s8[4] + s8[5]) + (s8[6] + s8[7]));
	}
	__syncthreads();
	if(tid < NB)
		xk[tid] = part[0][tid] + part[1][tid];
	__syncthreads();
	if(blockIdx.x == 0 && tid < NB)
		xout[k0 + tid] = xk[tid];
	if(blockIdx.x == 0)
		return;
	const int64_t i = (int64_t)(blockIdx.x - 1) * 256 + tid;
	if(i < k0) {
		const double *row = R + i + k0 * ld;
		double s16[16];
#pragma unroll
		for(int u = 0; u < 16; ++ u)
			s16[u] = 0;
		int c = 0;
		for(; c + 16 <= nv; c += 16) {
#pragma unroll
			for(int u = 0; u < 16; ++ u)
				s16[u] += row[(int64_t)(c + u) * ld] * xk[c + u];
		}
		for(; c < nv; ++ c)
			s16[0] += row[(int64_t)c * ld] * xk[c];
		double s = 0;
#pragma unroll
		for(int u = 0; u < 16; ++ u)
			s += s16[u];
		y[i] -= s;
	}
}


__global__ __launch_bounds__(256)
void trsv_back_chain_kernel(const double *__restrict__ R, int64_t ld, int64_t n, int nblk,
	const double *__restrict__ tinv_all, const double *__restrict__ y, double *xout, int *flags, int epoch, int *err)
{
	__shared__ double xs[NB];
	__shared__ double part[2][NB];
	__shared__ int ok;
	const int b = nblk - 1 - (int)blockIdx.x, tid = threadIdx.x, r = tid & (NB - 1), h = tid >> 7;
	const int64_t r0 = (int64_t)NB * b;
	double tv[64], rt[64];
	{
		const double *tinv = tinv_all + (size_t)b * NB * NB + r + (size_t)(64 * h) * NB;
#pragma unroll
		for(int c = 0; c < 64; ++ c)
			tv[c] = tinv[(size_t)c * NB];
	}
	auto load_tile = [&](int k) {
		const double *row = R + (r0 + r) + ((int64_t)NB * k + 64 * h) * ld;
#pragma unroll
		for(int c = 0; c < 64; ++ c)
			rt[c] = row[(int64_t)c * ld];
	};
	if(nblk - 1 > b)
		load_tile(nblk - 1);
	double acc = (h == 0 && r0 + r < n) ? y[r0 + r] : 0.0;
	for(int k = nblk - 1; k > b; -- k) {
		if(tid == 0) {
			int spins = 0;
			while(__hip_atomic_load(&flags[k], __ATOMIC_RELAXED, __HIP_MEMORY_SCOPE_AGENT) != epoch && spins < (1 << 22)) {
				__builtin_amdgcn_s_sleep(1);
				++ spins;
			}
			ok = spins < (1 << 22);
		}
		__syncthreads();
		if(!ok) {
			if(tid == 0)
				*err = 1;
			return;
		}
		if(tid < NB)
			xs[tid] = __hip_atomic_load(&xout[(int64_t)NB * k + tid], __ATOMIC_RELAXED, __HIP_MEMORY_SCOPE_AGENT);
		__syncthreads();
		const int64_t c0 = (int64_t)NB * k;
		const int nvk = (int)((n - c0 < NB) ? (n - c0) : NB);
		double s8[8] = {0, 0, 0, 0, 0, 0, 0, 0};
#pragma unroll
		for(int c = 0; c < 64; ++ c)
			s8[c & 7] += (64 * h + c < nvk) ? rt[c] * xs[64 * h + c] : 0.0;
		acc -= ((s8[0] + s8[1]) + (s8[2] + s8[3])) + ((s8[4] + s8[5]) + (s8[6] + s8[7]));
		if(k - 1 > b)
			load_tile(k - 1);
		__syncthreads();
	}
	part[h][r] = acc;
	__syncthreads();
	if(tid < NB)
		xs[tid] = part[0][tid] + part[1][tid];
	__syncthreads();
	{
		const int nv = (int)((n - r0 < NB) ? (n - r0) : NB);
		double s8[8] = {0, 0, 0, 0, 0, 0, 0, 0};
#pragma unroll
		for(int c = 0; c < 64; ++ c)
			s8[c & 7] += (64 * h + c < nv) ? tv[c] * xs[64 * h + c] : 0.0;
		part[h][r] = ((s8[0] + s8[1]) + (s8[2] + s8[3])) + ((s8[4] + s8[5]) + (s8[6] + s8[7]));
	}
	__syncthreads();
	if(tid < NB)
		__hip_atomic_store(&xout[r0 + tid], part[0][tid] + part[1][tid], __ATOMIC_RELAXED, __HIP_MEMORY_SCOPE_AGENT);
	asm volatile("s_waitcnt vmcnt(0)" ::: "memory");
	__syncthreads();
	if(tid == 0)
		__hip_atomic_store(&flags[b], epoch, __ATOMIC_RELAXED, __HIP_MEMORY_SCOPE_AGENT);
}

struct TrsvPay { double v; unsigned long long c; };

__device__ __forceinline__ void pay_store(TrsvPay *p, double v, unsigned long long K)
{
	__hip_atomic_store(&p->v, v, __ATOMIC_RELAXED, __HIP_MEMORY_SCOPE_AGENT);
	__hip_atomic_store(&p->c, (unsigned long long)__double_as_longlong(v) ^ K, __ATOMIC_RELAXED, __HIP_MEMORY_SCOPE_AGENT);
}

__device__ __forceinline__ bool pay_load(const TrsvPay *p, double &v, unsigned long long K)
{
	v = __hip_atomic_load(&p->v, __ATOMIC_RELAXED, __HIP_MEMORY_SCOPE_AGENT);
	const unsigned long long c = __hip_atomic_load(&p->c, __ATOMIC_RELAXED, __HIP_MEMORY_SCOPE_AGENT);
	return ((unsigned long long)__double_as_longlong(v) ^ c) == K;
}

template <int NW>
struct TileRegs { double2 v[NB / NW]; };

template <bool TRI, int NW>
__device__ __forceinline__ void tile_fetch(TileRegs<NW> &t, const double *T, const int64_t ld, const int lane, const int wave)
{
#pragma unroll
	for(int j = 0; j < NB / NW; ++ j) {
		const int c = wave + NW * j;
		const double *col = T + (int64_t)c * ld;
		const uint32_t loff = 2u * (uint32_t)lane;
		if(!TRI || 2 * lane <= c)
			t.v[j] = *(const double2*)(col + loff);
		else
			t.v[j] = make_double2(0, 0);
	}
}

template <int NW>
__device__ __forceinline__ void tile_dot(double2 &a, const TileRegs<NW> &t, const double *x, const int wave, const int nv)
{
	double2 s0 = make_double2(0, 0), s1 = make_double2(0, 0);
	if(nv >= NB) {
#pragma unroll
		for(int j = 0; j < NB / NW; j += 2) {
			const double x0 = x[wave + NW * j], x1 = x[wave + NW * j + NW];
			s0.x += t.v[j].x * x0; s0.y += t.v[j].y * x0;
			s1.x += t.v[j + 1].x * x1; s1.y += t.v[j + 1].y * x1;
		}
	} else {
#pragma unroll
		for(int j = 0; j < NB / NW; ++ j) {
			const int c = wave + NW * j;
			const double xv = (c < nv) ? x[c] : 0.0;
			s0.x += (c < nv) ? t.v[j].x * xv : 0.0;
			s0.y += (c < nv) ? t.v[j].y * xv : 0.0;
		}
	}
	a.x += s0.x + s1.x;
	a.y += s0.y + s1.y;
}

template <int NW, bool MFORM>
__global__ __launch_bounds__(64 * NW)
void trsv_back_chain2_kernel(const double *__restrict__ R, int64_t ld, int64_t n, int nblk,
	const double *__restrict__ tinv_all, const double *__restrict__ mbuf, double *y, TrsvPay *xpay, TrsvPay *wpay, unsigned long long K, int *err)
{
	__shared__ double xs[2][NB];
	__shared__ double zs[NB];
	__shared__ __attribute__((aligned(16))) double part[NW][NB];
	__shared__ int ok[2];
	constexpr int L = 1;
	const int tid = threadIdx.x, lane = tid & 63, wave = __builtin_amdgcn_readfirstlane(tid >> 6);
	constexpr int SPIN_MAX = 1 << 22;
	auto part_sum = [&](const int row) {
		double s = 0;
#pragma unroll
		for(int w = 0; w < NW; w += 2)
			s += part[w][row] + part[w + 1][row];
		return s;
	};
	if(blockIdx.x > 0) {
		const int b = nblk - (int)blockIdx.x;
		const int64_t r0 = (int64_t)NB * b;
		TileRegs<NW> ra, rb;
		TileRegs<NW> tvh;
		if(MFORM)
			tile_fetch<true, NW>(tvh, tinv_all + (size_t)b * NB * NB, NB, lane, wave);
		const int klast = b + L + 1;
		double2 acc = make_double2(0, 0);
		const double yb = (tid < NB && r0 + tid < n) ? y[r0 + tid] : 0.0;
		bool alive = true;
		auto step = [&](const int k, TileRegs<NW> &t, const int slot) {
			double *xk = xs[slot];
			if(tid < 64) {
				const TrsvPay *src = xpay + (size_t)k * NB + 2 * tid;
				double v0 = 0, v1 = 0;
				int spins = 0;
				for(;;) {
					const bool g0 = pay_load(src, v0, K), g1 = pay_load(src + 1, v1, K);
					if(__all(g0 && g1) || ++ spins >= SPIN_MAX)
						break;
					__builtin_amdgcn_s_sleep(2);
				}
				xk[2 * tid] = v0;
				xk[2 * tid + 1] = v1;
				if(tid == 0)
					ok[slot] = spins < SPIN_MAX;
			}
			lds_barrier();
			if(!ok[slot]) {
				if(tid == 0)
					*err = 1;
				alive = false;
				return;
			}
			const int64_t c0 = (int64_t)NB * k;
			const int nvk = (int)((n - c0 < NB) ? (n - c0) : NB);
			double2 s = make_double2(0, 0);
			tile_dot<NW>(s, t, xk, wave, nvk);
			acc.x -= s.x;
			acc.y -= s.y;
			asm volatile("" ::: "memory");
			__builtin_amdgcn_sched_barrier(0);
			if(k - 2 >= klast)
				tile_fetch<false, NW>(t, R + r0 + (int64_t)NB * (k - 2) * ld, ld, lane, wave);
		};
		int k = nblk - 1;
		if(k >= klast)
			tile_fetch<false, NW>(ra, R + r0 + (int64_t)NB * k * ld, ld, lane, wave);
		if(k - 1 >= klast)
			tile_fetch<false, NW>(rb, R + r0 + (int64_t)NB * (k - 1) * ld, ld, lane, wave);
		while(k >= klast && alive) {
			step(k, ra, 0);
			-- k;
			if(k < klast || !alive)
				break;
			step(k, rb, 1);
			-- k;
		}
		if(!alive)
			return;
		*(double2*)&part[wave][2 * lane] = acc;
		lds_barrier();
		if(!MFORM) {
			if(tid < NB)
				pay_store(wpay + (size_t)b * NB + tid, yb + part_sum(tid), K);
			return;
		}
		if(tid < NB)
			zs[tid] = yb + part_sum(tid);
		lds_barrier();
		{
			double2 s2 = make_double2(0, 0);
			tile_dot<NW>(s2, tvh, zs, wave, (int)((n - r0 < NB) ? (n - r0) : NB));
			*(double2*)&part[wave][2 * lane] = s2;
		}
		lds_barrier();
		if(tid < NB)
			pay_store(wpay + (size_t)b * NB + tid, part_sum(tid), K);
		return;
	}
	if(MFORM) {
		TileRegs<NW> ma, mb2;
		double uv = 0;
		unsigned long long uc = 0;
		auto ask_u = [&](int b, double &v, unsigned long long &c) {
			const TrsvPay *p = wpay + (size_t)b * NB + tid;
			v = __hip_atomic_load(&p->v, __ATOMIC_RELAXED, __HIP_MEMORY_SCOPE_AGENT);
			c = __hip_atomic_load(&p->c, __ATOMIC_RELAXED, __HIP_MEMORY_SCOPE_AGENT);
		};
		auto fetch_m = [&](int b, TileRegs<NW> &t) {
			if(b >= 0 && b + 1 < nblk)
				tile_fetch<false, NW>(t, mbuf + (size_t)b * NB * NB, NB, lane, wave);
		};
		auto hop = [&](const int b, TileRegs<NW> &t) {
			const int64_t r0 = (int64_t)NB * b;
			{
				double2 s2 = make_double2(0, 0);
				if(b + 1 < nblk)
					tile_dot<NW>(s2, t, xs[(b + 1) & 1], wave, NB);
				*(double2*)&part[wave][2 * lane] = s2;
			}
			asm volatile("" ::: "memory");
			__builtin_amdgcn_sched_barrier(0);
			fetch_m(b - 2, t);
			lds_barrier();
			if(tid < NB) {
				int spins = 0;
				while(((unsigned long long)__double_as_longlong(uv) ^ uc) != K && spins < SPIN_MAX) {
					__builtin_amdgcn_s_sleep(1);
					ask_u(b, uv, uc);
					++ spins;
				}
				if(spins >= SPIN_MAX)
					*err = 1;
				const double xr = uv - part_sum(tid);
				xs[b & 1][tid] = xr;
				pay_store(xpay + (size_t)b * NB + tid, xr, K);
				if(r0 + tid < n)
					y[r0 + tid] = xr;
				if(b > 0)
					ask_u(b - 1, uv, uc);
			}
			lds_barrier();
		};
		fetch_m(nblk - 2, mb2);
		if(tid < NB)
			ask_u(nblk - 1, uv, uc);
		for(int b = nblk - 1; b >= 0; b -= 2) {
			hop(b, ma);
			if(b >= 1)
				hop(b - 1, mb2);
		}
		return;
	}
	TileRegs<NW> t1a, tva;
	auto ask_w = [&](int b, double &v, unsigned long long &c) {
		const TrsvPay *p = wpay + (size_t)b * NB + tid;
		v = __hip_atomic_load(&p->v, __ATOMIC_RELAXED, __HIP_MEMORY_SCOPE_AGENT);
		c = __hip_atomic_load(&p->c, __ATOMIC_RELAXED, __HIP_MEMORY_SCOPE_AGENT);
	};
	auto fetch_tile = [&](int b, TileRegs<NW> &t1) {
		if(b >= 0 && b + 1 < nblk)
			tile_fetch<false, NW>(t1, R + (int64_t)NB * b + (int64_t)NB * (b + 1) * ld, ld, lane, wave);
	};
	auto fetch_inv = [&](int b, TileRegs<NW> &tv) {
		if(b >= 0)
			tile_fetch<true, NW>(tv, tinv_all + (size_t)b * NB * NB, NB, lane, wave);
	};
	double wv = 0;
	unsigned long long wc = 0;
	auto hop = [&](const int b, TileRegs<NW> &t1, TileRegs<NW> &tv) {
		const int64_t r0 = (int64_t)NB * b;
		{
			double2 s = make_double2(0, 0);
			if(b + 1 < nblk) {
				const int64_t c0 = (int64_t)NB * (b + 1);
				tile_dot<NW>(s, t1, xs[(b + 1) & 1], wave, (int)((n - c0 < NB) ? (n - c0) : NB));
			}
			*(double2*)&part[wave][2 * lane] = s;
		}
		asm volatile("" ::: "memory");
		__builtin_amdgcn_sched_barrier(0);
		fetch_tile(b - 1, t1);
		lds_barrier();
		if(tid < NB) {
			int spins = 0;
			while(((unsigned long long)__double_as_longlong(wv) ^ wc) != K && spins < SPIN_MAX) {
				__builtin_amdgcn_s_sleep(1);
				ask_w(b, wv, wc);
				++ spins;
			}
			if(spins >= SPIN_MAX)
				*err = 1;
			zs[tid] = wv - part_sum(tid);
		}
		lds_barrier();
		{
			double2 s = make_double2(0, 0);
			tile_dot<NW>(s, tv, zs, wave, (int)((n - r0 < NB) ? (n - r0) : NB));
			*(double2*)&part[wave][2 * lane] = s;
		}
		asm volatile("" ::: "memory");
		__builtin_amdgcn_sched_barrier(0);
		fetch_inv(b - 1, tv);
		lds_barrier();
		if(tid < NB) {
			const double xr = part_sum(tid);
			xs[b & 1][tid] = xr;
			pay_store(xpay + (size_t)b * NB + tid, xr, K);
			if(r0 + tid < n)
				y[r0 + tid] = xr;
			if(b > 0)
				ask_w(b - 1, wv, wc);
		}
		lds_barrier();
	};
	fetch_inv(nblk - 1, tva);
	if(tid < NB)
		ask_w(nblk - 1, wv, wc);
	for(int b = nblk - 1; b >= 0; -- b)
		hop(b, t1a, tva);
}

constexpr int TRSVM_LDS_DOUBLES = NB * TS + 16 * TS;
__global__ __launch_bounds__(1024)
void trsv_m_kernel(const double *__restrict__ R, int64_t ld, int64_t n, const double *__restrict__ tinv_all, double *__restrict__ mbuf)
{
	extern __shared__ double sm[];
	double *Ti = sm, *Xs = sm + NB * TS;
	const int b = blockIdx.x, sl = blockIdx.y, tid = threadIdx.x, lane = tid & 63, wave = tid >> 6, l15 = lane & 15, l4 = lane >> 4;
	const double *tv = tinv_all + (size_t)b * NB * NB;
	for(int e = tid; e < NB * NB / 2; e += 1024) {
		const int i = (e & (NB / 2 - 1)) * 2, k = e >> 6;
		if((i >> 4) <= (k >> 4)) {
			const double2 v = *(const double2*)(tv + i + (size_t)k * NB);
			Ti[i + k * TS] = (i <= k) ? v.x : 0.0;
			Ti[i + 1 + k * TS] = (i + 1 <= k) ? v.y : 0.0;
		}
	}
	const int64_t c0 = (int64_t)NB * (b + 1) + 16 * sl;
	for(int e = tid; e < NB * 16; e += 1024) {
		const int k = e & (NB - 1), j = e >> 7;
		Xs[k + j * TS] = (c0 + j < n) ? R[(int64_t)NB * b + k + (c0 + j) * ld] : 0.0;
	}
	__syncthreads();
	const int it = wave & 7, half = wave >> 3;
	v4f64 acc = (v4f64){0, 0, 0, 0};
	for(int kt = it + half; kt < NB / 16; kt += 2) {
		const v4f64 m = tile_atb(Ti + 16 * it + 16 * kt * TS, TS, 1, Xs + 16 * kt, 1, TS, lane);
		acc += m;
	}
	double *Pp = Ti + 16 * 7 + (16 * it) * TS;
	if(half && it < 7) {
#pragma unroll
		for(int r = 0; r < 4; ++ r)
			Pp[(l4 + 4 * r) + l15 * TS] = acc[r];
	}
	__syncthreads();
	if(!half) {
		double *M = mbuf + (size_t)b * NB * NB;
#pragma unroll
		for(int r = 0; r < 4; ++ r)
			M[(16 * it + l4 + 4 * r) + (size_t)(16 * sl + l15) * NB] = acc[r] + (it < 7 ? Pp[(l4 + 4 * r) + l15 * TS] : 0.0);
	}
}

__global__ void set_info_kernel(int *info) { info[0] = 0; info[1] = 0; }

__global__ void pad_diag_kernel(double *S, int64_t ld, int64_t n)
{
	const int64_t i = n + (int64_t)blockIdx.x * blockDim.x + threadIdx.x;
	if(i < ld) {
		S[i + n * ld] = 0.0;
		S[i + i * ld] = 1.0;
	}
}

void dense_set_padding_on(hipStream_t st, double *d_A, int64_t ld, int64_t n)
{
	hipLaunchKernelGGL(pad_diag_kernel, dim3((unsigned)((ld - n + 255) / 256)), dim3(256), 0, st,
		d_A, ld, n);
}

void dense_set_padding(spp_ctx *ctx, double *d_A, int64_t ld, int64_t n)
{
	dense_set_padding_on(ctx->stream, d_A, ld, n);
}

static void ensure_info(spp_ctx *ctx)
{
	if(!ctx->dense.info.p) {
		ctx->dense.info.reserve(4);
		SPP_HIP_CHECK(hipMemsetAsync(ctx->dense.info.p, 0, 4 * sizeof(int), ctx->stream));
	}
}

static std::mutex aux_pool_mutex;
static std::vector<std::pair<int, hipStream_t> > aux_pool;

static hipStream_t dense_aux_take(int device)
{
	std::lock_guard<std::mutex> lock(aux_pool_mutex);
	for(size_t i = 0; i < aux_pool.size(); ++ i)
		if(aux_pool[i].first == device) {
			hipStream_t s = aux_pool[i].second;
			aux_pool.erase(aux_pool.begin() + i);
			return s;
		}
	return nullptr;
}

void dense_aux_park(int device, hipStream_t s)
{
	if(hipStreamSynchronize(s) != hipSuccess) {
		(void)hipGetLastError();
		(void)hipStreamDestroy(s);
		return;
	}
	std::lock_guard<std::mutex> lock(aux_pool_mutex);
	if(aux_pool.size() >= 16) {
		(void)hipStreamDestroy(s);
		return;
	}
	static bool registered = false;
	if(!registered) {
		registered = true;
		atexit([]() {
			std::lock_guard<std::mutex> lock2(aux_pool_mutex);
			for(size_t i = 0; i < aux_pool.size(); ++ i)
				(void)hipStreamDestroy(aux_pool[i].second);
			aux_pool.clear();
		});
	}
	aux_pool.push_back(std::make_pair(device, s));
}

static void ensure_dense_work(spp_ctx *ctx, int64_t nblk)
{
	VClock clk("dense workspaces");
	ensure_info(ctx);
	clk.lap("status words");
	if(ctx->dense.tinv_all.cap < (size_t)nblk * NB * NB) {
		ctx->dense.tinv_all.reserve((size_t)nblk * NB * NB);
		SPP_HIP_CHECK(hipMemsetAsync(ctx->dense.tinv_all.p, 0, ctx->dense.tinv_all.cap * sizeof(double), ctx->stream));
	}
	ctx->dense.xtmp.reserve((size_t)(nblk + 1) * NB);
// ... 466 lines not shown
	}
	static_assert(POTRF_LDS_DOUBLES >= (64 + 64) * FS_STRIDE, "the fused kernel's LDS is sized by the factorization");
	auto fused_update_potrf = [&](int64_t r0, int64_t m, int64_t kp0, int64_t kn) {
		const int64_t N = ncols - r0;
		if(m <= 0 || N <= 0)
			return false;
		const int64_t md = std::min<int64_t>(NB, m), nd = std::min<int64_t>(NB, N);
		const int ti = (int)((md + 31) / 32), tj = (int)((nd + 31) / 32);
		int nA = 0;
		for(int j = 0; j < tj; ++ j)
			nA += std::min(j, ti - 1) + 1;
		const int64_t nbi = (m + 63) / 64, nbj = (N + 63) / 64;
		const int do_potrf = kn >= 0 ? 1 : 0;
		const int64_t kn0 = (kn >= 0 ? kn : 0) * NB;
		const int n_valid = (int)std::max<int64_t>(0, std::min<int64_t>(NB, n_id - kn0));
		const size_t slot = (size_t)(kn >= 0 ? kn : nsteps + 1);
		dw.fuse_expect[slot] += nA;
		hipLaunchKernelGGL(update_potrf_kernel, dim3((unsigned)(nA + do_potrf + nbi * nbj)), dim3(POTRF_THREADS),
			POTRF_LDS_DOUBLES * sizeof(double), s, m, N, d_A + kp0 + r0 * ld, ld, d_A + r0 + r0 * ld, nA, dw.fuse_expect[slot], do_potrf,
			n_valid, (has_rhs && n_valid < NB) ? 1 : 0, dw.tinv_all.p + (size_t)(kn >= 0 ? kn : 0) * NB * NB, dw.info.p, kn0,
			dw.fuse_cnt.p + slot, dw.info.p + 2, WAIT_TICKS_DEFAULT);
		return true;
	};
	auto potrf_and_panel = [&](int64_t k, bool potrf_done = false) {
		const int64_t k0 = k * NB;
		const int n_valid = (int)std::max<int64_t>(0, std::min<int64_t>(NB, n_id - k0));
		double *tinv = ctx->dense.tinv_all.p + (size_t)k * NB * NB;
		if(!potrf_done)
			hipLaunchKernelGGL(potrf_diag_kernel, dim3(1), dim3(POTRF_THREADS), POTRF_LDS_DOUBLES * sizeof(double), s,
				d_A + k0 + k0 * ld, ld, n_valid, (has_rhs && n_valid < NB) ? 1 : 0, tinv, ctx->dense.info.p, k0);
		const int64_t c1 = k0 + NB;
		if(c1 < ncols)
			launch_panel_solve(s, ncols - c1, tinv, d_A + k0 + c1 * ld, ld);
	};
	auto tile_row = [&](int64_t r0, int64_t kp0) {
		const int64_t m = std::min<int64_t>(NB, rows - r0);
		if(m <= 0 || r0 >= ncols)
			return;
		const double *P = d_A + kp0 + r0 * ld;
		flush_wait_b();
		launch_gemm_staged<32, 32, 16, 16, 0>(s, m, ncols - r0, NB, P, ld, P, ld, d_A + r0 + r0 * ld, ld, true);
	};
	if(allow_fused && nsteps >= 2 && switches().tail_rows * NB >= rows && dense_tail_applies(ctx, rows, nsteps) &&
		launch_dense_tail(ctx, d_A, ld, rows, ncols, nsteps, -1, has_rhs)) {
		dw.tinv_half = 0;
		SPP_HIP_CHECK(hipGetLastError());
		return;
	}
	potrf_and_panel(0);
	const int64_t single_below = 2560, single_mixed_above = 1280;
	for(int64_t k = 0; k < nsteps; ++ k) {
		const int64_t k0 = k * NB, c1 = k0 + NB, c2 = c1 + NB;
		if(c1 >= ncols || rows - c1 <= 0)
			break;
		if(rows - c1 <= single_below || (allow_fused && switches().tail_rows * NB >= rows - c1 && dense_tail_applies(ctx, rows, nsteps))) {
			if(bulk_pending) {
				wait_b_now();
				bulk_pending = false;
			}
			const double *P = d_A + k0 + c1 * ld;
			if(allow_fused && launch_dense_tail(ctx, d_A, ld, rows, ncols, nsteps, k, has_rhs)) {
				dw.tinv_half = k + 1;
				break;
			}
			if(fused && k + 1 < nsteps && rows - c1 >= NB) {
				fused_update_potrf(c1, rows - c1, k0, k + 1);
				potrf_and_panel(k + 1, true);
				continue;
			}
			if(rows - c1 >= single_mixed_above) {
				dom_begin(ctx);
				const bool big = dense_gemm_tn_sub(ctx, rows - c1, ncols - c1, NB, P, ld, P, ld, d_A + c1 + c1 * ld, ld, true);
				const double mr = (double)(rows - c1);
				if(big)
					dom_end(ctx, 2.0 * NB * (0.5 * mr * (mr + 1.0) + mr * (double)(ncols - rows)));
			} else
				launch_gemm_staged<32, 32, 16, 16, 0>(s, rows - c1, ncols - c1, NB, P, ld, P, ld, d_A + c1 + c1 * ld, ld, true);
			if(k + 1 < nsteps)
				potrf_and_panel(k + 1);
			continue;
		}
		record_a(k);
		if(bulk_pending) {
			wait_b_deferred();
			bulk_pending = false;
		}
		const bool have_bulk = rows - c2 > 0 && c2 < ncols;
		bool fused_done = false;
		if(have_bulk) {
			wait_a_on_bulk();
			const double *P = d_A + k0 + c2 * ld;
			hipStream_t keep = ctx->stream;
			ctx->stream = s2;
			dom_begin(ctx);
			const bool big = dense_gemm_tn_sub(ctx, rows - c2, ncols - c2, NB, P, ld, P, ld, d_A + c2 + c2 * ld, ld, true);
			const double mr = (double)(rows - c2);
			if(big)
				dom_end(ctx, 2.0 * NB * (0.5 * mr * (mr + 1.0) + mr * (double)(ncols - rows)));
			ctx->stream = keep;
			record_b(k);
			bulk_pending = true;
		}
		if(fused && k + 1 < nsteps && rows - c1 >= NB) {
			flush_wait_b();
			fused_update_potrf(c1, NB, k0, k + 1);
			fused_done = true;
		} else
			tile_row(c1, k0);
		flush_wait_b();
		if(k + 1 < nsteps)
			potrf_and_panel(k + 1, fused_done);
	}
	if(bulk_pending) {
		pend_sig_b = -1;
		if(use_flags)
			SPP_HIP_CHECK(hipEventRecord(evB, s2));
		SPP_HIP_CHECK(hipStreamWaitEvent(s, evB, 0));
	}
	SPP_HIP_CHECK(hipGetLastError());
}

void dense_reserve(spp_ctx *ctx, int64_t nblk)
{
	ensure_dense_work(ctx, nblk);
}

void dense_info_ensure(spp_ctx *ctx)
{
	ensure_info(ctx);
}

void dense_info_reset_on(spp_ctx *ctx, hipStream_t st)
{
	hipLaunchKernelGGL(set_info_kernel, dim3(1), dim3(1), 0, st, ctx->dense.info.p);
}

void dense_info_reset(spp_ctx *ctx)
{
	ensure_info(ctx);
	dense_info_reset_on(ctx, ctx->stream);
}

void dense_chain_check(spp_ctx *ctx)
{
	if(ctx->dense.h_chain_err && *ctx->dense.h_chain_err) {
		*ctx->dense.h_chain_err = 0;
		throw Error(SPP_E_HIP, "backward substitution: a workgroup of the chain kernel timed out waiting for its predecessor");
	}
}

int dense_info_fetch(spp_ctx *ctx, bool *dag_aborted)
{
	int h_info[4] = {0, 0, 0, 0};
	SPP_HIP_CHECK(hipMemcpyAsync(h_info, ctx->dense.info.p, 4 * sizeof(int), hipMemcpyDeviceToHost, ctx->stream));
	SPP_HIP_CHECK(hipStreamSynchronize(ctx->stream));
	if(h_info[3]) {
		SPP_HIP_CHECK(hipMemset(ctx->dense.info.p + 3, 0, sizeof(int)));
		sparse_dag_disable(ctx);
		if(dag_aborted) {
			*dag_aborted = true;
			return 0;
		}
		throw Error(SPP_E_HIP, "sparse factorization: a front timed out waiting for another front's flag; "
			"the following calls launch level by level");
	}
	if(h_info[2] && h_info[0]) {
		SPP_HIP_CHECK(hipMemset(ctx->dense.info.p + 2, 0, sizeof(int)));
		return h_info[0];
	}
	if(h_info[2] == TAIL_ABORT_TIMEOUT) {
		SPP_HIP_CHECK(hipMemset(ctx->dense.info.p + 2, 0, sizeof(int)));
		ctx->dense.tail_disabled = true;
		ctx->dense.fuse_dirty = true;
		throw Error(SPP_E_HIP, "dense factorization: the streamed launch (spp_dense_tail.h) timed out waiting for a tile; "
			"the following calls use the per-step schedule");
	}
	if(h_info[2]) {
		SPP_HIP_CHECK(hipMemset(ctx->dense.info.p + 2, 0, sizeof(int)));
		ctx->dense.sync_state = -1;
		ctx->dense.fuse_dirty = true;
		throw Error(SPP_E_HIP, "dense factorization: a cross-stream flag wait timed out (streams not concurrent?); "
			"the following calls use the event schedule");
	}
	return h_info[0];
}

bool dense_potrf_upper_enqueue(spp_ctx *ctx, double *d_A, int64_t n, int64_t ld, bool info_reset)
{
	SPP_REQUIRE(ld % NB == 0 && n < ld, SPP_E_BADARG, "dense_potrf_upper: ld must be a multiple of 128 and > n");
	if(info_reset)
		dense_info_reset(ctx);
	dense_factor_steps(ctx, d_A, ld, n, n, n + 1, (n + NB - 1) / NB, true);
	return ctx->dense.tail_masked_whole;
}

int dense_potrf_upper(spp_ctx *ctx, double *d_A, int64_t n, int64_t ld, bool )
{
	SPP_REQUIRE(ld % NB == 0 && n < ld, SPP_E_BADARG, "dense_potrf_upper: ld must be a multiple of 128 and > n");
	dense_info_reset(ctx);
	dense_factor_steps(ctx, d_A, ld, n, n, n + 1, (n + NB - 1) / NB, true);
	return dense_info_fetch(ctx) ? SPP_NOT_POSDEF : SPP_OK;
}

__global__ __launch_bounds__(256)
void front_image_kernel(double *F, int64_t ld, double *P, int64_t ldp, int w, int pad, int h, int to_image)
{
	const int c = (int)blockIdx.x, hp = h + pad;
	const bool cpad = c >= w && c < w + pad;
	const int cu = c < w ? c : c - pad;
	for(int r = threadIdx.x; r < hp; r += 256) {
		const bool rpad = r >= w && r < w + pad;
		const int ru = r < w ? r : r - pad;
		if(to_image)
			P[r + (int64_t)c * ldp] = (cpad || rpad) ? (r == c ? 1.0 : 0.0) : (r <= c ? F[ru + (int64_t)cu * ld] : 0.0);
		else if(!cpad && !rpad)
			F[ru + (int64_t)cu * ld] = P[r + (int64_t)c * ldp];
	}
}

int dense_front_factor(spp_ctx *ctx, double *d_F, int64_t ld, int64_t w, int64_t h, double *d_image)
{
	SPP_REQUIRE(w > 0 && h >= w && ld >= h && h < (1 << 20), SPP_E_BADARG, "front factor: need 0 < w <= h <= ld");
	hipStream_t s = ctx->stream;
	const int64_t pad = ((w + NB - 1) / NB) * NB - w, hp = h + pad, ldp = (hp + 1) & ~int64_t(1);
	const size_t img = (size_t)ldp * hp, band = (size_t)ldp * NB;
	DevBuf<double> P;
	P.reserve(img + band);
	SPP_HIP_CHECK(hipMemsetAsync(P.p + img, 0xff, band * sizeof(double), s));
	hipLaunchKernelGGL(front_image_kernel, dim3((unsigned)hp), dim3(256), 0, s, d_F, ld, P.p, ldp, (int)w, (int)pad, (int)h, 1);
	dense_info_reset(ctx);
	{
		struct IdentGuard {
			DenseWork &d;
			IdentGuard(DenseWork &dw, int64_t from) : d(dw) { d.ident_from = from; }
			~IdentGuard() { d.ident_from = -1; }
		} guard(ctx->dense, w);
		dense_factor_steps(ctx, P.p, ldp, w + pad, hp, hp, (w + pad) / NB, false);
	}
	const int info = dense_info_fetch(ctx);
	hipLaunchKernelGGL(front_image_kernel, dim3((unsigned)hp), dim3(256), 0, s, d_F, ld, P.p, ldp, (int)w, (int)pad, (int)h, 0);
	if(d_image)
		SPP_HIP_CHECK(hipMemcpyAsync(d_image, P.p, (size_t)hp * ldp * sizeof(double), hipMemcpyDeviceToDevice, s));
	std::vector<unsigned long long> hb(band);
	SPP_HIP_CHECK(hipMemcpyAsync(hb.data(), P.p + img, band * sizeof(double), hipMemcpyDeviceToHost, s));
	SPP_HIP_CHECK(hipStreamSynchronize(s));
	for(size_t q = 0; q < band; ++ q)
		SPP_REQUIRE(hb[q] == ~0ull, SPP_E_HIP, "front factor: a write past the end of the front's image");
	return info ? SPP_NOT_POSDEF : SPP_OK;
}

void dense_potrs_upper(spp_ctx *ctx, const double *d_R, int64_t n, int64_t ld, double *d_b)
{
	const int64_t nblk = (n + NB - 1) / NB;
	hipStream_t s = ctx->stream;
	if(ctx->dense.tinv_half > 0) {
		hipLaunchKernelGGL(tinv_finish_kernel, dim3((unsigned)ctx->dense.tinv_half), dim3(1024), 0, s, ctx->dense.tinv_all.p);
		ctx->dense.tinv_half = 0;
	}
	const int use_chain = capturing(s) ? 0 : switches().trsv_chain;
	if(use_chain == 2 && nblk > 1 && nblk <= 4096) {
		DenseWork &dw = ctx->dense;
		const size_t need = (size_t)nblk * NB * 4;
		if(dw.trsv_pay.cap < need) {
			dw.trsv_pay.reserve(need);
			SPP_HIP_CHECK(hipMemsetAsync(dw.trsv_pay.p, 0, dw.trsv_pay.cap * sizeof(double), s));
		}
		if(!dw.h_chain_err) {
			SPP_HIP_CHECK(hipHostMalloc((void**)&dw.h_chain_err, sizeof(int), hipHostMallocDefault));
			*dw.h_chain_err = 0;
		}
		++ dw.epoch;
		const unsigned long long K = (2ull * (unsigned long long)dw.epoch + 1ull) * 0x9E3779B97F4A7C15ull;
		TrsvPay *xpay = (TrsvPay*)dw.trsv_pay.p, *wpay = xpay + (size_t)nblk * NB;
		if(switches().trsv_mform) {
			if(dw.trsv_m.cap < (size_t)nblk * NB * NB)
				dw.trsv_m.reserve((size_t)nblk * NB * NB);
			static uint64_t attr_seen = 0;
			if(first_on_this_device(attr_seen))
				SPP_HIP_CHECK(hipFuncSetAttribute((const void*)trsv_m_kernel, hipFuncAttributeMaxDynamicSharedMemorySize, TRSVM_LDS_DOUBLES * (int)sizeof(double)));
			hipLaunchKernelGGL(trsv_m_kernel, dim3((unsigned)nblk - 1, 8), dim3(1024), TRSVM_LDS_DOUBLES * sizeof(double), s, d_R, ld, n, dw.tinv_all.p, dw.trsv_m.p);
			hipLaunchKernelGGL((trsv_back_chain2_kernel<8, true>), dim3((unsigned)nblk + 1), dim3(512), 0, s,
				d_R, ld, n, (int)nblk, dw.tinv_all.p, dw.trsv_m.p, d_b, xpay, wpay, K, dw.info.p + 1);
		} else
			hipLaunchKernelGGL((trsv_back_chain2_kernel<8, false>), dim3((unsigned)nblk + 1), dim3(512), 0, s,
				d_R, ld, n, (int)nblk, dw.tinv_all.p, (const double*)nullptr, d_b, xpay, wpay, K, dw.info.p + 1);
		SPP_HIP_CHECK(hipGetLastError());
		SPP_HIP_CHECK(hipMemcpyAsync(dw.h_chain_err, dw.info.p + 1, sizeof(int), hipMemcpyDeviceToHost, s));
		return;
	}
	if(use_chain && nblk > 1 && nblk <= 1024) {
		DenseWork &dw = ctx->dense;
		if(dw.flags.cap < (size_t)nblk) {
			dw.flags.reserve((size_t)nblk);
			SPP_HIP_CHECK(hipMemsetAsync(dw.flags.p, 0, (size_t)nblk * sizeof(int), s));
			dw.epoch = 0;
		}
		if(!dw.h_chain_err) {
			SPP_HIP_CHECK(hipHostMalloc((void**)&dw.h_chain_err, sizeof(int), hipHostMallocDefault));
			*dw.h_chain_err = 0;
		}
		++ dw.epoch;
		hipLaunchKernelGGL(trsv_back_chain_kernel, dim3((unsigned)nblk), dim3(256), 0, s, d_R, ld, n, (int)nblk,
			dw.tinv_all.p, d_b, dw.xtmp.p, dw.flags.p, (int)dw.epoch, dw.info.p + 1);
		SPP_HIP_CHECK(hipGetLastError());
		SPP_HIP_CHECK(hipMemcpyAsync(d_b, dw.xtmp.p, n * sizeof(double), hipMemcpyDeviceToDevice, s));
		SPP_HIP_CHECK(hipMemcpyAsync(dw.h_chain_err, dw.info.p + 1, sizeof(int), hipMemcpyDeviceToHost, s));
		return;
	}
	for(int64_t k = nblk; k > 0;) {
		-- k;
		const int64_t k0 = k * NB;
		const double *tinv = ctx->dense.tinv_all.p + (size_t)k * NB * NB;
		unsigned nwg = 1 + (unsigned)((k0 + 255) / 256);
		const int nv = (int)((n - k0 < NB) ? (n - k0) : NB);
		hipLaunchKernelGGL(trsv_back_kernel, dim3(nwg), dim3(256), 0, s, d_R, ld, k0, nv, tinv, d_b, ctx->dense.xtmp.p);
	}
	SPP_HIP_CHECK(hipGetLastError());
	SPP_HIP_CHECK(hipMemcpyAsync(d_b, ctx->dense.xtmp.p, n * sizeof(double), hipMemcpyDeviceToDevice, s));
}

__global__ void copy_kernel(const double2 *__restrict__ src, double2 *__restrict__ dst, size_t n)
{
	size_t i = (size_t)blockIdx.x * blockDim.x + threadIdx.x, stride = (size_t)gridDim.x * blockDim.x;
	for(; i < n; i += stride)
		dst[i] = src[i];
}

double microbench_copy(spp_ctx *ctx, size_t bytes, int iters)
{
	DevBuf<double2> a, b;
	size_t n = bytes / sizeof(double2);
	a.reserve(n);
	b.reserve(n);
	SPP_HIP_CHECK(hipMemsetAsync(a.p, 0, n * sizeof(double2), ctx->stream));
	hipEvent_t e0, e1;
	SPP_HIP_CHECK(hipEventCreate(&e0));
	SPP_HIP_CHECK(hipEventCreate(&e1));
	hipLaunchKernelGGL(copy_kernel, dim3(2048), dim3(256), 0, ctx->stream, a.p, b.p, n);
	SPP_HIP_CHECK(hipEventRecord(e0, ctx->stream));
	for(int i = 0; i < iters; ++ i)
		hipLaunchKernelGGL(copy_kernel, dim3(2048), dim3(256), 0, ctx->stream, a.p, b.p, n);
	SPP_HIP_CHECK(hipEventRecord(e1, ctx->stream));
	SPP_HIP_CHECK(hipEventSynchronize(e1));
	float ms = 0;
	SPP_HIP_CHECK(hipEventElapsedTime(&ms, e0, e1));
	(void)hipEventDestroy(e0);
	(void)hipEventDestroy(e1);
	return 2.0 * n * sizeof(double2) * iters / (ms * 1e-3) * 1e-9;
}

__global__ __launch_bounds__(1024)
void ctile_rw_kernel(double *C, int64_t ldc)
{
	const int lane = threadIdx.x & 63, wave = threadIdx.x >> 6;
	const int l15 = lane & 15, l4 = lane >> 4;
	const int64_t m0 = (int64_t)blockIdx.x * 128 + (wave % 4) * 32, n0 = (int64_t)blockIdx.y * 128 + (wave / 4) * 32;
	double v[2][2][4];
#pragma unroll
	for(int b = 0; b < 2; ++ b)
#pragma unroll
		for(int a = 0; a < 2; ++ a)
#pragma unroll
			for(int r = 0; r < 4; ++ r)
				v[b][a][r] = C[m0 + a * 16 + l15 + (n0 + b * 16 + l4 + 4 * r) * ldc];
#pragma unroll
	for(int b = 0; b < 2; ++ b)
#pragma unroll
		for(int a = 0; a < 2; ++ a)
#pragma unroll
			for(int r = 0; r < 4; ++ r)
				C[m0 + a * 16 + l15 + (n0 + b * 16 + l4 + 4 * r) * ldc] = -v[b][a][r];
}

double microbench_ctile(spp_ctx *ctx, int n, int iters)
{
	SPP_REQUIRE(n > 0 && n % 128 == 0, SPP_E_BADARG, "ctile microbenchmark: n must be a multiple of 128");
	DevBuf<double> c;
	c.reserve((size_t)n * n);
	SPP_HIP_CHECK(hipMemsetAsync(c.p, 0, (size_t)n * n * sizeof(double), ctx->stream));
	hipEvent_t e0, e1;
	SPP_HIP_CHECK(hipEventCreate(&e0));
	SPP_HIP_CHECK(hipEventCreate(&e1));
	hipLaunchKernelGGL(ctile_rw_kernel, dim3(n / 128, n / 128), dim3(1024), 0, ctx->stream, c.p, (int64_t)n);
	SPP_HIP_CHECK(hipEventRecord(e0, ctx->stream));
	for(int i = 0; i < iters; ++ i)
		hipLaunchKernelGGL(ctile_rw_kernel, dim3(n / 128, n / 128), dim3(1024), 0, ctx->stream, c.p, (int64_t)n);
	SPP_HIP_CHECK(hipEventRecord(e1, ctx->stream));
	SPP_HIP_CHECK(hipEventSynchronize(e1));
	float ms = 0;
	SPP_HIP_CHECK(hipEventElapsedTime(&ms, e0, e1));
	(void)hipEventDestroy(e0);
	(void)hipEventDestroy(e1);
	return 2.0 * n * n * sizeof(double) * iters / (ms * 1e-3) * 1e-9;
}

__global__ __launch_bounds__(256)
void mfma_f64_peak_kernel(double *out, int iters)
{
	double fn[8], fm[2];
#pragma unroll
	for(int i = 0; i < 8; ++ i)
		fn[i] = 0.25 + 1e-3 * ((threadIdx.x * 7 + i * 13) & 63);
#pragma unroll
	for(int i = 0; i < 2; ++ i)
		fm[i] = 0.5 - 1e-3 * ((threadIdx.x * 5 + i * 11 + blockIdx.x) & 63);
	v4f64 acc[2][2];
#pragma unroll
	for(int i = 0; i < 2; ++ i)
#pragma unroll
		for(int j = 0; j < 2; ++ j)
			acc[i][j] = (v4f64){0, 0, 0, 0};
	for(int it = 0; it < iters; ++ it) {
#pragma unroll
		for(int r = 0; r < 4; ++ r)
#pragma unroll
			for(int i = 0; i < 2; ++ i)
#pragma unroll
				for(int j = 0; j < 2; ++ j)
					acc[i][j] = __builtin_amdgcn_mfma_f64_16x16x4f64(fn[i + 2 * r], fm[j], acc[i][j], 0, 0, 0);
		fm[0] = -fm[0];
	}
	double s = 0;
#pragma unroll
	for(int i = 0; i < 2; ++ i)
#pragma unroll
		for(int j = 0; j < 2; ++ j)
			s += acc[i][j][0] + acc[i][j][1] + acc[i][j][2] + acc[i][j][3];
	out[(size_t)blockIdx.x * blockDim.x + threadIdx.x] = s;
}

double microbench_mfma_f64(spp_ctx *ctx, int iters)
{
	const int nblk = 256 * 8;
	DevBuf<double> out;
	out.reserve((size_t)nblk * 256);
	hipEvent_t e0, e1;
	SPP_HIP_CHECK(hipEventCreate(&e0));
	SPP_HIP_CHECK(hipEventCreate(&e1));
	hipLaunchKernelGGL(mfma_f64_peak_kernel, dim3(nblk), dim3(256), 0, ctx->stream, out.p, 16);
	SPP_HIP_CHECK(hipEventRecord(e0, ctx->stream));
	hipLaunchKernelGGL(mfma_f64_peak_kernel, dim3(nblk), dim3(256), 0, ctx->stream, out.p, iters);
	SPP_HIP_CHECK(hipEventRecord(e1, ctx->stream));
	SPP_HIP_CHECK(hipEventSynchronize(e1));
	float ms = 0;
	SPP_HIP_CHECK(hipEventElapsedTime(&ms, e0, e1));
	(void)hipEventDestroy(e0);
	(void)hipEventDestroy(e1);
	double flops = (double)nblk * 4 * (double)iters * 16 * 2048.0;
	return flops / (ms * 1e-3) * 1e-12;
}

double microbench_update(spp_ctx *ctx, int64_t m, int iters)
{
	const int64_t ld = ((m + 1 + 127) / 128) * 128;
	DevBuf<double> p, c;
	p.reserve((size_t)ld * 128);
	c.reserve((size_t)ld * ld);
	SPP_HIP_CHECK(hipMemsetAsync(p.p, 0, (size_t)ld * 128 * sizeof(double), ctx->stream));
	SPP_HIP_CHECK(hipMemsetAsync(c.p, 0, (size_t)ld * ld * sizeof(double), ctx->stream));
// ... 18 lines not shown
```

slam_plus_plus_amd/csrc/spp_internal.h:

```cpp
#pragma once

#include <hip/hip_runtime.h>
#include <stdint.h>
#include <string>
#include <vector>
#include <sys/mman.h>
#include <utility>
#include <new>
#include <exception>
#include <thread>
#include <stdexcept>
#include <algorithm>
#include <string.h>
#include <chrono>
#include <stdio.h>
#include <stdlib.h>
#include "../../include/spp_hip.h"
#include "spp_switches.h"

namespace spp {

struct Error : std::runtime_error {
	int code;
	Error(int c, const std::string &what) : std::runtime_error(what), code(c) {}
// ... 59 lines not shown
	template <class U> bool operator!=(const HugeAlloc<U>&) const { return false; }
};
template <class T> using HVec = std::vector<T, HugeAlloc<T> >;

template <class T>
struct DevBuf {
	T *p = nullptr;
	size_t cap = 0;
	bool owned = true;
	DevBuf() {}
	DevBuf(const DevBuf&) = delete;
	DevBuf &operator=(const DevBuf&) = delete;
	~DevBuf() { release(); }
	void release()
	{
		if(p && owned)
			(void)hipFree(p);
		p = nullptr;
		cap = 0;
		owned = true;
	}
	void view(T *ptr, size_t n)
	{
		release();
		p = ptr;
		cap = n;
		owned = false;
	}
	void reserve(size_t n)
	{
		if(n <= cap && owned)
			return;
		release();
		size_t want = n;
		hipError_t e = hipMalloc((void**)&p, want * sizeof(T));
		if(e != hipSuccess) {
			p = nullptr;
			throw Error(SPP_E_NOMEM, "hipMalloc of " + std::to_string(want * sizeof(T)) + " bytes failed");
		}
		cap = want;
	}
	template <class A>
	void upload(const std::vector<T, A> &h, hipStream_t s)
	{
		reserve(h.size() ? h.size() : 1);
		if(!h.empty())
			SPP_HIP_CHECK(hipMemcpyAsync(p, h.data(), h.size() * sizeof(T), hipMemcpyHostToDevice, s));
	}
};

struct UploadArena {
	hipStream_t stream;
	std::vector<unsigned char> host;
	struct Item { void **pp; size_t *pcap; bool *powned; size_t off, n; };
	std::vector<Item> items;
	explicit UploadArena(hipStream_t s) : stream(s) { host.reserve(size_t(1) << 20); }
	template <class T, class A>
	void add(DevBuf<T> &b, const std::vector<T, A> &v)
	{
		if(v.size() * sizeof(T) > (size_t(256) << 10)) {
			b.upload(v, stream);
			return;
		}
		b.release();
		const size_t off = (host.size() + 255) & ~(size_t)255, bytes = std::max<size_t>(v.size(), 1) * sizeof(T);
		host.resize(off + bytes);
		if(!v.empty())
			memcpy(host.data() + off, v.data(), v.size() * sizeof(T));
		Item it = {(void**)&b.p, &b.cap, &b.owned, off, std::max<size_t>(v.size(), 1)};
		items.push_back(it);
	}
	void commit(DevBuf<unsigned char> &store)
	{
		store.release();
		store.reserve(std::max<size_t>(host.size(), 256));
		if(!host.empty())
			SPP_HIP_CHECK(hipMemcpyAsync(store.p, host.data(), host.size(), hipMemcpyHostToDevice, stream));
		for(size_t i = 0; i < items.size(); ++ i) {
			*items[i].pp = store.p + items[i].off;
			*items[i].pcap = items[i].n;
			*items[i].powned = false;
		}
	}
};

struct Structure {
	int64_t nb = 0, n = 0, nnzb = 0, nvals = 0;
	HVec<int64_t> col_ptr, row_idx, blk_off, base;
	HVec<int32_t> dim;
};

struct SaccItem {
	int32_t beg, end;
	int32_t kind;
	int32_t a_tr;
	int64_t dst;
	int64_t aoff;
};

struct SchurDims {
	int dp = 0, dl = 0;
	int64_t nc = 0, nl = 0;
	int64_t nl_total = 0;
	int64_t no = 0;
	int64_t n_red = 0, ld = 0;
	int64_t n_sblk = 0;
	int64_t n_pairs = 0;
	int64_t n_items = 0, n_multi = 0;
	int32_t xcd_max_items = 0;
	bool u_landmark_major = true;
	bool factored = true;
};

struct SchurPlan : SchurDims {
	bool add_A = true;
	bool sparse_S = false;
	bool mis = false;
	Structure s_st;
	DevBuf<int64_t> sblk_voff;
	std::vector<int64_t> pose_block;
	std::vector<int64_t> lm_block;
	std::vector<uint8_t> is_lm;
	std::vector<uint64_t> tile_mask;
	DevBuf<int32_t> lm_ptr;
	DevBuf<int32_t> bs_ptr;
	int64_t n_bs = 0;
	int lm_stream_last = 0;
	DevBuf<int64_t> lm_coff;
	DevBuf<int64_t> lm_rbase;
	DevBuf<int32_t> obs_pose;
	DevBuf<int32_t> obs_lm;
	DevBuf<int64_t> obs_off;
	DevBuf<int64_t> pose_rbase;
	DevBuf<int32_t> cam_ptr;
	DevBuf<int32_t> cam_obs;
	DevBuf<int32_t> obs_wpos;
	DevBuf<SaccItem> items;
	DevBuf<int32_t> xcd_beg;
	DevBuf<int32_t> sblk_i1, sblk_i2;
	DevBuf<int64_t> sblk_aoff;
	DevBuf<int32_t> pair_a, pair_b;
	DevBuf<int32_t> multi_blk;
	DevBuf<int32_t> multi_ptr;
	DevBuf<double> cinv;
	DevBuf<double> lfac;
	DevBuf<double> W;
	DevBuf<double> Up;
	DevBuf<double> xw;
	DevBuf<double> partial;
	DevBuf<double> S;
	bool unlisted_dirty = true;
	bool side_pending = false, side_padded = false;
	int side_last = 0, clear_last = 0;
	void release_all();
};

struct DenseWork {
	DevBuf<double> tinv;
	DevBuf<int> info;
	DevBuf<double> tinv_all;
	int64_t tinv_half = 0;
	DevBuf<double> xtmp;
	DevBuf<int> flags;
	DevBuf<int> tail_pub;
	DevBuf<double> tail_dinv;
	int tail_epoch = 0;
	DevBuf<int> tail_order;
	std::vector<int> tail_order_host;
	int tail_order_tr = 0, tail_order_tc = 0;
	std::vector<uint64_t> tail_order_bits;
	bool tail_order_pre = false, tail_order_masked = false;
	int tail_resident = -1;
	const std::vector<uint64_t> *tile_mask = nullptr;
	bool tail_masked_whole = false;
	int tail_rows_last = 0;
	bool tail_disabled = false;
	DevBuf<double> trsv_m;
	DevBuf<double> trsv_pay;
	uint64_t epoch = 0;
	int *h_chain_err = nullptr;
	hipStream_t aux = nullptr;
	hipEvent_t ev[2] = {nullptr, nullptr};
	DevBuf<int> sync;
	DevBuf<int> fuse_cnt;
	std::vector<int> fuse_expect;
	bool fuse_dirty = false;
	int64_t ident_from = -1;
	hipStream_t chain = nullptr;
	hipEvent_t ev_chain = nullptr;
	DevBuf<int> la_cnt;
	DevBuf<long long> la_trace;
	int la_state = 0;
	int la_reserve = 0;
	int la_ncu = 0;
	int sync_epoch = 0;
	int sync_state = 0;
	hipStream_t sync_stream = nullptr;
};

struct SparsePlan;

struct AssemblePlan;

struct PhaseTimer {
	hipEvent_t ev[2 * SPP_N_PHASES];
	bool used[SPP_N_PHASES];
	bool created = false;
};

}

struct spp_ctx {
	int device = 0;
	int flags = 0;
	hipStream_t stream = nullptr;
	bool own_stream = false;
	hipStream_t side_stream = nullptr;
	hipEvent_t side_ev[2] = {nullptr, nullptr};
	std::string last_error;
	int mode = -1;
	int shard_rank = 0, shard_world = 1;
	spp::Structure st;
	std::vector<int64_t> order;
	std::thread plan_trash;
	spp::SchurPlan schur;
	spp::DenseWork dense;
	spp::SparsePlan *sparse = nullptr;
	spp::AssemblePlan *assemble = nullptr;
	spp::DevBuf<double> d_vals, d_rhs;
	double *h_staging = nullptr;
	size_t h_staging_cap = 0;
	spp::DevBuf<double> geom_partial;
	spp::PhaseTimer timer;
	double phase_ms[SPP_N_PHASES] = {0};
	std::vector<hipEvent_t> dom_events;
	size_t dom_used = 0;
	double dom_flops = 0;
	int64_t factor_flops = 0, solve_bytes = 0, factor_nnz = 0;
};

namespace spp {

void se2_linearize(spp_ctx *ctx, int64_t ne, const int32_t *d_v0, const int32_t *d_v1, const double *d_poses,
	const double *d_meas, double *d_J0, double *d_J1, double *d_r);
double se2_update(spp_ctx *ctx, int64_t nv, double *d_poses, const double *d_dx, bool apply);
void se2_linearize_at(spp_ctx *ctx, int64_t ne, const int64_t *d_off0, const int64_t *d_off1, const double *d_state,
	const double *d_meas, double *d_J0, double *d_J1, double *d_r);
void se2_rb_linearize(spp_ctx *ctx, int64_t ne, const int64_t *d_off0, const int64_t *d_off1, const double *d_state,
	const double *d_meas, double *d_J0, double *d_J1, double *d_r);
double slam2d_update(spp_ctx *ctx, int64_t n, double *d_state, const double *d_dx, int64_t n_angles,
	const int64_t *d_angle_off, bool apply);
void se3_linearize_at(spp_ctx *ctx, int64_t ne, const int64_t *d_off0, const int64_t *d_off1, const double *d_state,
	const double *d_meas, double *d_J0, double *d_J1, double *d_r);
void se3_xyz_linearize(spp_ctx *ctx, int64_t ne, const int64_t *d_pose_off, const int64_t *d_lm_off, const double *d_state,
	const double *d_meas, double *d_J0, double *d_J1, double *d_r);
double slam3d_update(spp_ctx *ctx, int64_t n, double *d_state, const double *d_dx, int64_t n_poses,
	const int64_t *d_pose_off, bool apply);
void rocv_range_linearize(spp_ctx *ctx, int64_t ne, const int64_t *d_recv_off, const int64_t *d_lm_off, const double *d_state,
	const double *d_meas, double *d_J0, double *d_J1, double *d_r);
void rocv_cv_linearize(spp_ctx *ctx, int64_t ne, const int64_t *d_off0, const int64_t *d_off1, const double *d_state,
	const double *d_dt, double *d_J0, double *d_J1, double *d_r);
double edge_chi2(spp_ctx *ctx, int64_t ne, int rd, const double *d_r, const double *d_Om);
void edge_robust_weights(spp_ctx *ctx, int64_t ne, int rd, int kind, double scale, double param, const double *d_r, double *d_w);
double edge_hessian_maxdiag(spp_ctx *ctx, int64_t ne, int rd, int d0, int d1, const double *d_J0, const double *d_J1,
	const double *d_Om);
double lm_gain_denominator(spp_ctx *ctx, int64_t n, const double *d_dx, const double *d_rhs, double alpha);
void se3_linearize(spp_ctx *ctx, int64_t ne, const int32_t *d_v0, const int32_t *d_v1, const double *d_poses,
	const double *d_meas, double *d_J0, double *d_J1, double *d_r);
double se3_update(spp_ctx *ctx, int64_t nv, double *d_poses, const double *d_dx, bool apply);
void ba_linearize(spp_ctx *ctx, int64_t no, const int32_t *d_cam_of, const int32_t *d_pt_of, const double *d_cams,
	const double *d_intr, const double *d_pts, const double *d_meas, double *d_J0, double *d_J1, double *d_r);
void ba_stereo_linearize(spp_ctx *ctx, int64_t no, const int32_t *d_cam_of, const int32_t *d_pt_of, const double *d_cams,
	const double *d_intr, const double *d_pts, const double *d_meas, double *d_J0, double *d_J1, double *d_r);
void ba_intrinsics_linearize(spp_ctx *ctx, int64_t no, const int32_t *d_cam_of, const int32_t *d_pt_of, const int32_t *d_intr_of,
	const double *d_cams, const double *d_intr, const double *d_pts, const double *d_meas, double *d_J0, double *d_J1, double *d_J2,
	double *d_r);
double ba_intrinsics_update(spp_ctx *ctx, int64_t ni, double *d_intr, const int64_t *d_intr_dxoff, const double *d_dx, bool apply);
double ba_update(spp_ctx *ctx, int64_t nc, double *d_cams, const int64_t *d_cam_dxoff, int64_t np, double *d_pts,
	const int64_t *d_pt_dxoff, const double *d_dx, int64_t n_dx, bool apply);

void min_degree_order(int64_t nb, const int64_t *col_ptr, const int64_t *row_idx, std::vector<int64_t> &order);
void nested_dissection_order(int64_t nb, const int64_t *col_ptr, const int64_t *row_idx, std::vector<int64_t> &order);

void tile_mask_mark(int64_t n, int bs, int64_t nblk, const int32_t *i1, const int32_t *i2, std::vector<uint64_t> &words);
int64_t tile_mask_close(int64_t n, bool has_rhs, bool fill, std::vector<uint64_t> &words);
constexpr double TAIL_MODEL_STEP_US = 36.5, TAIL_MODEL_UPDATE_US = 2.0, TAIL_MODEL_START_US = 45.0;
constexpr int TAIL_MODEL_RESIDENT = 256;
struct TileDagCost {
	int64_t tiles = 0, updates = 0, path = 0;
	double cost_us = 0;
};
TileDagCost tile_dag_cost(int64_t n, const std::vector<uint64_t> &filled, int resident);
void tail_order_table(const std::vector<uint64_t> &bits, int Tr, int Tc, bool have_pre, double beta, int resident, bool early,
	std::vector<int> &order, int *info);

void build_schur_plan(spp_ctx *ctx, bool sparse_S, bool mis = false);
int64_t schur_buffer_doubles(const spp_ctx *ctx);
bool schur_applicable(const Structure &st, int *dp, int *dl);
double schur_plan_host_probe(const Structure &st, int shard_rank, int shard_world, bool sparse_S, bool mis, int64_t *out);
void schur_tile_mask_host_probe(const Structure &st, std::vector<uint64_t> &words);
bool schur_cam_order_host_probe(const Structure &st, int shard_rank, int shard_world, bool sparse_S, bool mis, const int64_t *order_in,
	std::vector<int32_t> &cam_order, TileDagCost cost[2]);

void sparse_analyze(spp_ctx *ctx, const Structure &st);
int sparse_factor_solve(spp_ctx *ctx, const double *d_vals, double *d_rhs);
void sparse_release(spp_ctx *ctx);
void sparse_dag_disable(spp_ctx *ctx);
int64_t sparse_info(const spp_ctx *ctx, int what);
int64_t sparse_fronts(const spp_ctx *ctx, int64_t capacity, int32_t *h, int32_t *w, int32_t *pad, int32_t *cls, int32_t *level,
	int32_t *parent, int32_t *team);

constexpr int64_t SCHUR_SIDE_MIN_OBS = 500000;
void schur_form(spp_ctx *ctx, const double *d_vals, const double *d_rhs, double *d_S_rhs, bool one_call = false);
int schur_finish(spp_ctx *ctx, const double *d_vals, double *d_S_rhs, double *d_rhs);
void schur_pack(spp_ctx *ctx, double *S, double *packed, bool pack);

constexpr int DENSE_NB = 128;
int dense_potrf_upper(spp_ctx *ctx, double *d_A, int64_t n, int64_t ld, bool keep_inverses);
bool dense_potrf_upper_enqueue(spp_ctx *ctx, double *d_A, int64_t n, int64_t ld, bool info_reset = true);
int dense_info_fetch(spp_ctx *ctx, bool *dag_aborted = nullptr);
void dense_potrs_upper(spp_ctx *ctx, const double *d_R, int64_t n, int64_t ld, double *d_b);
void dense_aux_park(int device, hipStream_t s);
void dense_factor_steps(spp_ctx *ctx, double *d_A, int64_t ld, int64_t n, int64_t rows, int64_t ncols,
	int64_t nsteps, bool has_rhs);
void dense_info_reset(spp_ctx *ctx);
void dense_info_ensure(spp_ctx *ctx);
void dense_info_reset_on(spp_ctx *ctx, hipStream_t st);
void dense_reserve(spp_ctx *ctx, int64_t nblk);

void dense_chain_check(spp_ctx *ctx);
void dense_set_padding(spp_ctx *ctx, double *d_A, int64_t ld, int64_t n);
void dense_set_padding_on(hipStream_t st, double *d_A, int64_t ld, int64_t n);
struct TileMaskGuard {
	DenseWork &d;
	TileMaskGuard(DenseWork &dw, const std::vector<uint64_t> *m) : d(dw) { d.tile_mask = (m && !m->empty()) ? m : nullptr; }
	~TileMaskGuard() { d.tile_mask = nullptr; }
};
int dense_front_factor(spp_ctx *ctx, double *d_F, int64_t ld, int64_t w, int64_t h, double *d_image);
bool dense_gemm_tn_sub(spp_ctx *ctx, int64_t m, int64_t n, int64_t k, const double *A, int64_t lda,
	const double *B, int64_t ldb, double *C, int64_t ldc, bool upper_only);
double microbench_copy(spp_ctx *ctx, size_t bytes, int iters);
double microbench_mfma_f64(spp_ctx *ctx, int iters);
double microbench_ctile(spp_ctx *ctx, int n, int iters);
double microbench_update(spp_ctx *ctx, int64_t m, int iters);

void assemble_analyze(spp_ctx *ctx, int64_t nv, const int32_t *dim, int n_groups, const int64_t *g_ne,
	const int64_t *const *g_v0, const int64_t *const *g_v1, const int64_t *const *g_seq, const int *g_d0, const int *g_d1,
	const int *g_rd, int64_t unary_vertex, const uint8_t *skip_vertex = nullptr);
int assemble_n_groups(const spp_ctx *ctx);
int64_t assemble_group_edges(const spp_ctx *ctx, int group);
bool assemble_group_is_unary(const spp_ctx *ctx, int group);
void assemble_run(spp_ctx *ctx, const double *J0, const double *J1, const double *Om, const double *r,
	double damping, double *vals, double *eta);
void assemble_groups_run(spp_ctx *ctx, const double *const *J0, const double *const *J1, const double *const *Om,
	const double *const *r, double damping, double *vals, double *eta);
void assemble_set_edge_weights(spp_ctx *ctx, int group, const double *d_w);
void assemble_release(spp_ctx *ctx);
bool assemble_is_ternary(const spp_ctx *ctx);
constexpr int ASM_HUB_CHUNK = 4096;
void assemble_analyze_ternary(spp_ctx *ctx, int64_t nv, const int32_t *dim, int64_t ne, const int64_t *v0, const int64_t *v1,
	const int64_t *v2, int64_t unary_vertex);
void assemble_ternary_run(spp_ctx *ctx, const double *J0, const double *J1, const double *J2, const double *Om, const double *r,
	double damping, double *vals, double *eta);
void assemble_get_structure(const spp_ctx *ctx, int64_t *col_ptr, int64_t *row_idx, int64_t *blk_off);

void phase_begin(spp_ctx *ctx, int phase);
void phase_end(spp_ctx *ctx, int phase);
void phases_reset(spp_ctx *ctx);
void phases_collect(spp_ctx *ctx);
void dom_begin(spp_ctx *ctx);
void dom_end(spp_ctx *ctx, double flops);

template <class F>
inline void run_threads(int nt, F fn)
{
	if(nt <= 1) {
		fn(0);
		return;
	}
	std::vector<std::thread> th;
	std::exception_ptr err[64];
	for(int t = 1; t < nt; ++ t)
		th.emplace_back([&, t]() { try { fn(t); } catch(...) { err[t] = std::current_exception(); } });
	try { fn(0); } catch(...) { err[0] = std::current_exception(); }
	for(size_t t = 0; t < th.size(); ++ t)
		th[t].join();
	for(int t = 0; t < nt; ++ t)
		if(err[t])
			std::rethrow_exception(err[t]);
}

inline int plan_threads(int64_t work)
{
	const int env = switches().plan_threads;
	int nt = env ? env : (int)std::min<unsigned>(16u, std::max(1u, std::thread::hardware_concurrency()));
	if(work < switches().plan_min_work)
		nt = 1;
	return std::min(nt, 64);
}

template <class V>
inline void balanced_cuts(const V &w_prefix, int nt, std::vector<int64_t> &cut)
{
	const int64_t n = (int64_t)w_prefix.size() - 1, total = w_prefix[n];
	cut.assign(nt + 1, n);
	cut[0] = 0;
	for(int t = 1; t < nt; ++ t)
		cut[t] = std::lower_bound(w_prefix.begin(), w_prefix.end(), total * t / nt) - w_prefix.begin();
	for(int t = 1; t <= nt; ++ t)
		cut[t] = std::max(cut[t], cut[t - 1]);
	cut[nt] = n;
}


}
```

slam_plus_plus_amd/csrc/spp_schur.hip:

```cpp

#include "spp_internal.h"

namespace spp {

template <int DL>
__device__ __forceinline__ void cinv_block(const double *__restrict__ m, double *o)
{
	if(DL == 3) {
#define M_(i, j) m[(i) + 3 * (j)]
#define COF_(i, j) (M_(((i) + 1) % 3, ((j) + 1) % 3) * M_(((i) + 2) % 3, ((j) + 2) % 3) - \
	M_(((i) + 1) % 3, ((j) + 2) % 3) * M_(((i) + 2) % 3, ((j) + 1) % 3))
		const double c00 = COF_(0, 0), c10 = COF_(1, 0), c20 = COF_(2, 0);
		const double det = c00 * M_(0, 0) + c10 * M_(1, 0) + c20 * M_(2, 0);
		const double id = -1.0 / det;
		o[0] = c00 * id; o[3] = c10 * id; o[6] = c20 * id;
		o[1] = COF_(0, 1) * id; o[4] = COF_(1, 1) * id; o[7] = COF_(2, 1) * id;
		o[2] = COF_(0, 2) * id; o[5] = COF_(1, 2) * id; o[8] = COF_(2, 2) * id;
#undef COF_
#undef M_
	} else if(DL == 2) {
		const double det = m[0] * m[3] - m[2] * m[1];
		const double id = -1.0 / det;
		o[0] = m[3] * id; o[2] = -m[2] * id;
		o[1] = -m[1] * id; o[3] = m[0] * id;
// ... 922 lines not shown
	dbl2_a8 pc[BLK / 2] = {};
	double dv[DP];
	int32_t l0, l1, a0, na;
	bool transposed;
	auto request = [&](int32_t g) {
		l0 = bs_ptr[g], l1 = bs_ptr[g + 1];
		a0 = lm_ptr[l0], na = lm_ptr[l1] - a0;
		const int64_t oo = (t < na) ? obs_off[(int64_t)a0 + t] : 0;
		const double *d = dx + (int64_t)((t < na) ? obs_pose[(int64_t)a0 + t] : 0) * DP;
		transposed = (oo & 1) != 0;
		off[lane] = oo;
		wave_lds_sync();
#pragma unroll
		for(int r = 0; r < DP; ++ r)
			dv[r] = d[r];
		const int rest = na - 64 * wave;
		if(rest > 0)
			fetch_U_pieces<BLK>(vals, off, (rest < 64) ? rest : 64, lane, pc);
	};
	if(g0 < g1)
		request(g0);
	for(int32_t g = g0; g < g1; ++ g) {
		double *tq = tq_all[(g - g0) & 1];
		store_U_pieces<BLK>(img, lane, pc);
		wave_lds_sync();
		if(t < na) {
			double u[BLK];
			take_U<DP, DL>(img + lane * ST, transposed, u);
#pragma unroll
			for(int q = 0; q < DL; ++ q) {
				double sum = 0;
#pragma unroll
				for(int r = 0; r < DP; ++ r)
					sum += dv[r] * u[r + DP * q];
				tq[t * DL + q] = sum;
			}
		}
		const int32_t nlg = l1 - l0, ga0 = a0;
		const bool lm_lane = t < nlg;
		const int64_t l = (int64_t)l0 + (lm_lane ? t : 0);
		const int64_t rb = lm_rbase[l];
		const int32_t pa = lm_ptr[l] - ga0, pe = lm_ptr[l + 1] - ga0;
		double tv[DL], m[DL * DL];
#pragma unroll
		for(int q = 0; q < DL; ++ q)
			tv[q] = -rhs[rb + q];
		{
			const double *src = cinv ? cinv + l * DL * DL : vals + lm_coff[l];
#pragma unroll
			for(int e = 0; e < DL * DL; ++ e)
				m[e] = src[e];
		}
		if(g + 1 < g1)
			request(g + 1);
		else {
#pragma unroll
			for(int q = 0; q < DL; ++ q)
				asm volatile("" : "+v"(tv[q]));
#pragma unroll
			for(int e = 0; e < DL * DL; ++ e)
				asm volatile("" : "+v"(m[e]));
			asm volatile("" :: "v"(pa), "v"(pe));
		}
		asm volatile("s_waitcnt lgkmcnt(0)\n\ts_barrier" ::: "memory");
		if(lm_lane) {
			for(int32_t p = pa; p < pe; ++ p) {
#pragma unroll
				for(int q = 0; q < DL; ++ q)
					tv[q] += tq[p * DL + q];
			}
			double Ci[DL * DL];
			if(cinv) {
#pragma unroll
				for(int e = 0; e < DL * DL; ++ e)
					Ci[e] = m[e];
			} else
				cinv_block<DL>(m, Ci);
#pragma unroll
			for(int q = 0; q < DL; ++ q) {
				double sum = 0;
#pragma unroll
				for(int u = 0; u < DL; ++ u)
					sum += Ci[q + DL * u] * tv[u];
				rhs[rb + q] = sum;
			}
		}
	}
}

template <int DP>
__global__ __launch_bounds__(256)
void scatter_dx_kernel(int64_t nc, const int64_t *__restrict__ pose_rbase, const double *__restrict__ dx,
	double *__restrict__ rhs)
{
	const int64_t e = (int64_t)blockIdx.x * blockDim.x + threadIdx.x;
	if(e >= nc * DP)
		return;
	rhs[pose_rbase[e / DP] + e % DP] = dx[e];
}

template <int DP, int DL>
static int lm_stream_form(const SchurPlan &sp)
{
	if(!(DP == 6 && DL == 3) || !sp.factored)
		return 0;
	const int v = switches().lm_stream;
	return (v == 1 || v == 2) ? v : 0;
}

template <int DP, int DL, typename... Args>
static void launch_obs_fact_stream(bool xw_obs, dim3 grid, hipStream_t s, Args... args)
{
	if constexpr(DP == 6 && DL == 3) {
		if(xw_obs)
			hipLaunchKernelGGL((obs_fact_stream_kernel<DP, DL, true>), grid, dim3(256), 0, s, args...);
		else
			hipLaunchKernelGGL((obs_fact_stream_kernel<DP, DL, false>), grid, dim3(256), 0, s, args...);
	}
}

template <int DP, int DL, typename... Args>
static void launch_backsubst_stream(dim3 grid, hipStream_t s, Args... args)
{
	if constexpr(DP == 6 && DL == 3)
		hipLaunchKernelGGL((backsubst_stream_kernel<DP, DL>), grid, dim3(256), 0, s, args...);
}

struct ClearArgs {
	uint64_t rowbits[64];
	int n_rows;
};

__global__ __launch_bounds__(256)
void s_clear_tiles_kernel(double *__restrict__ S, int64_t ld, ClearArgs a)
{
	const int j = (int)blockIdx.x, i = (int)blockIdx.y;
	if(j < i || (i < a.n_rows && !((a.rowbits[i] >> j) & 1)))
		return;
	double *T = S + (int64_t)i * 128 + (int64_t)j * 128 * ld;
	const int t = threadIdx.x, r = 2 * (t & 63), c0 = t >> 6;
	const dbl2_a8 z = {0.0, 0.0};
#pragma unroll 4
	for(int c = c0; c < 128; c += 4)
		*(dbl2_a8*)(T + r + (int64_t)c * ld) = z;
}

static void side_stream_ensure(spp_ctx *ctx)
{
	if(ctx->side_stream)
		return;
	SPP_HIP_CHECK(hipStreamCreateWithFlags(&ctx->side_stream, hipStreamNonBlocking));
	SPP_HIP_CHECK(hipEventCreateWithFlags(&ctx->side_ev[0], hipEventDisableTiming));
	SPP_HIP_CHECK(hipEventCreateWithFlags(&ctx->side_ev[1], hipEventDisableTiming));
}

static void side_stream_join(spp_ctx *ctx)
{
	if(!ctx->schur.side_pending)
		return;
	SPP_HIP_CHECK(hipStreamWaitEvent(ctx->stream, ctx->side_ev[1], 0));
	ctx->schur.side_pending = false;
}

static bool stream_capturing(hipStream_t s)
{
	hipStreamCaptureStatus cs = hipStreamCaptureStatusNone;
	return hipStreamIsCapturing(s, &cs) != hipSuccess || cs != hipStreamCaptureStatusNone;
}

template <int DP, int DL>
static void schur_form_t(spp_ctx *ctx, const double *d_vals, const double *d_rhs, double *S, bool one_call)
{
	SchurPlan &sp = ctx->schur;
	hipStream_t s = ctx->stream;
	const int64_t ld = sp.ld;
	const int64_t *voff = sp.sparse_S ? sp.sblk_voff.p : nullptr;
	double *xcol = sp.sparse_S ? S + sp.s_st.nvals : S + sp.n_red * ld;
	side_stream_join(ctx);
	sp.side_padded = false;
	phase_begin(ctx, SPP_PHASE_SCHUR_INV);
	const bool own_dense = S == sp.S.p && !sp.sparse_S && ctx->shard_world == 1;
	const int64_t n_trows = ld / 128;
	if(own_dense && sp.n_sblk == sp.nc * (sp.nc + 1) / 2 && sp.n_red == sp.nc * DP) {
		SPP_HIP_CHECK(hipMemsetAsync(S + sp.n_red * ld, 0, (size_t)(schur_buffer_doubles(ctx) - sp.n_red * ld) * sizeof(double), s));
		sp.clear_last = 2;
	} else if(own_dense && !sp.unlisted_dirty && !sp.tile_mask.empty() && (int64_t)sp.tile_mask.size() <= n_trows && n_trows <= 64) {
		ClearArgs ca;
		memset(ca.rowbits, 0, sizeof(ca.rowbits));
		for(size_t q = 0; q < sp.tile_mask.size(); ++ q)
			ca.rowbits[q] = sp.tile_mask[q];
		ca.n_rows = (int)sp.tile_mask.size();
		hipLaunchKernelGGL(s_clear_tiles_kernel, dim3((unsigned)n_trows, (unsigned)n_trows), dim3(256), 0, s, S, ld, ca);
		sp.clear_last = 1;
	} else {
		SPP_HIP_CHECK(hipMemsetAsync(S, 0, (size_t)schur_buffer_doubles(ctx) * sizeof(double), s));
		sp.clear_last = 0;
		if(own_dense)
			sp.unlisted_dirty = false;
	}
	constexpr int VIL = VSplit<DP * DL>::IL;
	double *Vm = sp.W.p, *Vs = sp.W.p + sp.no * VIL;
	const bool onfly = sp.factored && DL <= 3;
	if(sp.nl && !onfly)
		hipLaunchKernelGGL((cinv_kernel<DL>), dim3((unsigned)((sp.nl + 255) / 256)), dim3(256), 0, s,
			sp.nl, sp.lm_coff.p, d_vals, sp.cinv.p, sp.factored ? sp.lfac.p : nullptr);
	const int lm_stream = lm_stream_form<DP, DL>(sp);
	sp.lm_stream_last = lm_stream;
	const double *lfac_arg = onfly ? (const double*)nullptr : (const double*)sp.lfac.p;
	const dim3 obs_grid((unsigned)((sp.no + 255) / 256));
	if(sp.no && lm_stream)
		launch_obs_fact_stream<DP, DL>(lm_stream == 1, obs_grid, s, sp.no, sp.obs_lm.p, sp.obs_off.p, sp.lm_rbase.p, d_vals, d_rhs, lfac_arg,
			sp.lm_coff.p, sp.obs_wpos.p, Vm, Vs, sp.xw.p);
	else if(sp.no && sp.factored)
		hipLaunchKernelGGL((obs_fact_kernel<DP, DL>), obs_grid, dim3(256), 0, s,
			sp.no, sp.obs_lm.p, sp.obs_off.p, sp.lm_rbase.p, d_vals, d_rhs, lfac_arg, sp.lm_coff.p,
			sp.obs_wpos.p, Vm, Vs, sp.xw.p);
	else if(sp.no)
		hipLaunchKernelGGL((obs_kernel<DP, DL>), obs_grid, dim3(256), 0, s,
			sp.no, sp.obs_lm.p, sp.obs_off.p, sp.lm_rbase.p, d_vals, d_rhs, sp.cinv.p, sp.obs_wpos.p, sp.W.p, sp.Up.p, sp.xw.p, sp.u_landmark_major ? 1 : 0);
	phase_end(ctx, SPP_PHASE_SCHUR_INV);
	const int side_sw = switches().schur_side;
	const bool side = side_sw != 0 && sp.nc > 0 && (side_sw == 2 || sp.no >= SCHUR_SIDE_MIN_OBS) &&
		!(ctx->flags & SPP_FLAG_PROFILE) && !stream_capturing(s);
	sp.side_last = side ? 1 : 0;
	auto launch_rhs = [&](hipStream_t st) {
		if(sp.nc && lm_stream == 1)
			hipLaunchKernelGGL((rhs_kernel<DP, true>), dim3((unsigned)((sp.nc + 3) / 4)), dim3(256), 0, st,
				sp.nc, sp.cam_ptr.p, sp.cam_obs.p, sp.pose_rbase.p, sp.xw.p, d_rhs, sp.add_A ? 1 : 0, xcol);
		else if(sp.nc)
			hipLaunchKernelGGL((rhs_kernel<DP, false>), dim3((unsigned)((sp.nc + 3) / 4)), dim3(256), 0, st,
				sp.nc, sp.cam_ptr.p, sp.cam_obs.p, sp.pose_rbase.p, sp.xw.p, d_rhs, sp.add_A ? 1 : 0, xcol);
	};
	if(side) {
		side_stream_ensure(ctx);
		const bool pad_here = one_call && own_dense;
		if(pad_here)
			dense_info_ensure(ctx);
		SPP_HIP_CHECK(hipEventRecord(ctx->side_ev[0], s));
		SPP_HIP_CHECK(hipStreamWaitEvent(ctx->side_stream, ctx->side_ev[0], 0));
		launch_rhs(ctx->side_stream);
		if(pad_here) {
			dense_set_padding_on(ctx->side_stream, S, ld, sp.n_red);
			dense_info_reset_on(ctx, ctx->side_stream);
			sp.side_padded = true;
		}
		SPP_HIP_CHECK(hipEventRecord(ctx->side_ev[1], ctx->side_stream));
		sp.side_pending = true;
	}
	phase_begin(ctx, SPP_PHASE_SCHUR_GEMM);
	if(sp.n_items) {
		int chunk = switches().sacc_chunk;
		if(chunk <= 0)
			chunk = (int)((sp.xcd_max_items + SACC_WAVES * 64 - 1) / (SACC_WAVES * 64));
		const int64_t per = (int64_t)SACC_WAVES * chunk;
		if(sp.factored)
			hipLaunchKernelGGL((s_accum_kernel<DP, DL, true>), dim3((unsigned)(8 * ((sp.xcd_max_items + per - 1) / per))), dim3(SACC_WAVES * 64), 0, s,
				sp.items.p, sp.xcd_beg.p, chunk, sp.pair_a.p, sp.pair_b.p, Vm, Vs, d_vals, S, ld, sp.partial.p);
		else
			hipLaunchKernelGGL((s_accum_kernel<DP, DL, false>), dim3((unsigned)(8 * ((sp.xcd_max_items + per - 1) / per))), dim3(SACC_WAVES * 64), 0, s,
				sp.items.p, sp.xcd_beg.p, chunk, sp.pair_a.p, sp.pair_b.p, sp.W.p, sp.Up.p, d_vals, S, ld, sp.partial.p);
	}
	if(sp.n_multi)
		hipLaunchKernelGGL((s_multi_kernel<DP>), dim3((unsigned)((sp.n_multi + 3) / 4)), dim3(256), 0, s,
			sp.n_multi, sp.multi_blk.p, sp.multi_ptr.p, sp.sblk_i1.p, sp.sblk_i2.p, sp.sblk_aoff.p,
			sp.partial.p, d_vals, sp.add_A ? 1 : 0, S, ld, voff);
	phase_end(ctx, SPP_PHASE_SCHUR_GEMM);
	phase_begin(ctx, SPP_PHASE_SCHUR_RHS);
	if(!side)
		launch_rhs(s);
	else if(!one_call)
		side_stream_join(ctx);
	phase_end(ctx, SPP_PHASE_SCHUR_RHS);
	SPP_HIP_CHECK(hipGetLastError());
}

template <int DP, int DL>
static int schur_finish_t(spp_ctx *ctx, const double *d_vals, double *S, double *d_rhs)
{
	SchurPlan &sp = ctx->schur;
	hipStream_t s = ctx->stream;
	const int64_t ld = sp.ld;
	double *xcol;
	side_stream_join(ctx);
	if(sp.sparse_S) {
		xcol = S + sp.s_st.nvals;
		const int ret = sparse_factor_solve(ctx, S, xcol);
		if(ret != SPP_OK)
			return ret;
	} else {
		phase_begin(ctx, SPP_PHASE_FACTOR);
		if(!sp.side_padded)
			dense_set_padding(ctx, S, ld, sp.n_red);
		{
			TileMaskGuard guard(ctx->dense, &sp.tile_mask);
			const bool own = S == sp.S.p;
			if(own)
				sp.unlisted_dirty = true;
			const bool masked_whole = dense_potrf_upper_enqueue(ctx, S, sp.n_red, ld, !sp.side_padded);
			if(own && masked_whole)
				sp.unlisted_dirty = false;
		}
		sp.side_padded = false;
		phase_end(ctx, SPP_PHASE_FACTOR);
		xcol = S + sp.n_red * ld;
		phase_begin(ctx, SPP_PHASE_TRISOLVE);
		dense_potrs_upper(ctx, S, sp.n_red, ld, xcol);
		phase_end(ctx, SPP_PHASE_TRISOLVE);
	}
	phase_begin(ctx, SPP_PHASE_BACKSUBST);
	static_assert(DL <= DP, "the products U^T dx reuse the W l buffer (DP doubles per observation)");
	const int bs_fused = switches().backsubst_fused;
	const double *cinv_arg = (sp.factored && DL <= 3) ? (const double*)nullptr : (const double*)sp.cinv.p;
	const int32_t bs_per = (sp.n_bs >= 1024) ? 4 : 1;
	const bool bs_stream = bs_fused && sp.n_bs > 0 && lm_stream_form<DP, DL>(sp);
	const int32_t bs_scatter = bs_stream ? (int32_t)((sp.nc * DP + BS_SCATTER_PER - 1) / BS_SCATTER_PER) : 0;
	if(bs_stream)
		launch_backsubst_stream<DP, DL>(dim3((unsigned)((sp.n_bs + bs_per - 1) / bs_per + bs_scatter)), s,
			(int32_t)sp.n_bs, bs_per, (const int32_t*)sp.bs_ptr.p, (const int32_t*)sp.lm_ptr.p, (const int32_t*)sp.obs_pose.p, (const int64_t*)sp.obs_off.p,
			(const int64_t*)sp.lm_rbase.p, cinv_arg, (const int64_t*)sp.lm_coff.p, d_vals, (const double*)xcol, d_rhs,
			bs_scatter, (int64_t)sp.nc, (const int64_t*)sp.pose_rbase.p);
	else if(bs_fused && sp.n_bs > 0)
		hipLaunchKernelGGL((backsubst_fused_kernel<DP, DL>), dim3((unsigned)sp.n_bs), dim3(256), 0, s,
			sp.bs_ptr.p, sp.lm_ptr.p, sp.obs_pose.p, sp.obs_off.p, sp.lm_rbase.p, cinv_arg, sp.lm_coff.p, d_vals, xcol, d_rhs);
	else {
		if(sp.no)
			hipLaunchKernelGGL((backsubst_obs_kernel<DP, DL>), dim3((unsigned)((sp.no + 255) / 256)), dim3(256), 0, s,
				sp.no, sp.obs_pose.p, sp.obs_off.p, d_vals, xcol, sp.xw.p);
		if(sp.nl)
			hipLaunchKernelGGL((backsubst_lm_kernel<DL>), dim3((unsigned)((sp.nl + 255) / 256)), dim3(256), 0, s,
				sp.nl, sp.lm_ptr.p, sp.lm_rbase.p, sp.xw.p, cinv_arg, sp.lm_coff.p, d_vals, d_rhs);
	}
	if(sp.nc && !bs_stream)
		hipLaunchKernelGGL((scatter_dx_kernel<DP>), dim3((unsigned)((sp.nc * DP + 255) / 256)), dim3(256), 0, s,
			sp.nc, sp.pose_rbase.p, xcol, d_rhs);
	phase_end(ctx, SPP_PHASE_BACKSUBST);
	SPP_HIP_CHECK(hipGetLastError());
	if(!sp.sparse_S && dense_info_fetch(ctx))
		return SPP_NOT_POSDEF;
	return SPP_OK;
}

template <bool PACK>
__global__ __launch_bounds__(256)
void schur_pack_kernel(double *__restrict__ S, int64_t ld, double *__restrict__ packed)
{
	const int64_t k = blockIdx.y;
	const int64_t rows = 128 * (k + 1);
	const int64_t e = (int64_t)blockIdx.x * 256 + threadIdx.x;
	if(e >= rows * 128)
		return;
	const int64_t r = e % rows, c = e / rows;
	double *ps = S + r + (128 * k + c) * ld;
	double *pp = packed + 128 * 128 * (k * (k + 1) / 2) + e;
	if(PACK)
		*pp = *ps;
	else
		*ps = *pp;
}

void schur_pack(spp_ctx *ctx, double *S, double *packed, bool pack)
{
	const int64_t ld = ctx->schur.ld, nblk = ld / 128;
	dim3 grid((unsigned)((ld * 128 + 255) / 256), (unsigned)nblk);
	if(pack)
		hipLaunchKernelGGL((schur_pack_kernel<true>), grid, dim3(256), 0, ctx->stream, S, ld, packed);
	else
		hipLaunchKernelGGL((schur_pack_kernel<false>), grid, dim3(256), 0, ctx->stream, S, ld, packed);
	SPP_HIP_CHECK(hipGetLastError());
}

void schur_form(spp_ctx *ctx, const double *d_vals, const double *d_rhs, double *d_S_rhs, bool one_call)
{
	const int dp = ctx->schur.dp, dl = ctx->schur.dl;
	if(dp == 6 && dl == 3) schur_form_t<6, 3>(ctx, d_vals, d_rhs, d_S_rhs, one_call);
	else if(dp == 3 && dl == 2) schur_form_t<3, 2>(ctx, d_vals, d_rhs, d_S_rhs, one_call);
	else if(dp == 3 && dl == 3) schur_form_t<3, 3>(ctx, d_vals, d_rhs, d_S_rhs, one_call);
	else if(dp == 6 && dl == 6) schur_form_t<6, 6>(ctx, d_vals, d_rhs, d_S_rhs, one_call);
	else throw Error(SPP_E_UNSUPPORTED, "Schur kernels: block widths not instantiated");
}

int schur_finish(spp_ctx *ctx, const double *d_vals, double *d_S_rhs, double *d_rhs)
{
	const int dp = ctx->schur.dp, dl = ctx->schur.dl;
	if(dp == 6 && dl == 3) return schur_finish_t<6, 3>(ctx, d_vals, d_S_rhs, d_rhs);
	if(dp == 3 && dl == 2) return schur_finish_t<3, 2>(ctx, d_vals, d_S_rhs, d_rhs);
	if(dp == 3 && dl == 3) return schur_finish_t<3, 3>(ctx, d_vals, d_S_rhs, d_rhs);
	if(dp == 6 && dl == 6) return schur_finish_t<6, 6>(ctx, d_vals, d_S_rhs, d_rhs);
	throw Error(SPP_E_UNSUPPORTED, "Schur kernels: block widths not instantiated");
}

}
```

slam_plus_plus_amd/csrc/spp_switches.h:

```cpp
#pragma once

#include <stdint.h>
#include <stdlib.h>
#include <string.h>
#include <algorithm>

namespace spp {

constexpr long long WAIT_TICKS_PER_MS = 100000;
constexpr long long WAIT_TICKS_DEFAULT = 500 * WAIT_TICKS_PER_MS;

enum Ordering { ORDERING_AUTO, ORDERING_AMD, ORDERING_ND };
constexpr int MID_FRONT_MAX = 640;

struct Switches {
	bool verbose;
	int plan_threads;
	int64_t plan_min_work;

	int dense_sched;
	int fused;
	int aux_reserve_cus;
	int tile_444;
	int dense_la;
	int la_chain_mask;
	int la_g2;
	int la_bulk_acquire;
	int64_t la_slots;
	int la_trace;
	int tail_rows;
	int tail_mask;
	double tail_order_beta;
	int tail_early;
	long long tail_timeout_ticks;
	int tail_trace;
	int trsv_chain;
	int trsv_mform;

	bool sacc_ulm;
	bool sacc_factored;
	int64_t sacc_tile;
	int64_t sacc_tile_cols;
	int sacc_xcd;
	int sacc_chunk;
	int schur_cam_order;
	int backsubst_fused;
	int schur_side;
	int lm_stream;

	int mid_front_max;
	Ordering ordering;
	int64_t amalg_small;
	double amalg_zeros;
	int64_t amalg_relax_h;
	double amalg_zeros_small;
	bool sparse_teams;
	int sparse_team_max;
	int sparse_team_cols;
	int sparse_dag;
	int dag_split;
	long long dag_timeout_ticks;
	int dag_trace;
};

inline int env_int(const char *name, int dflt)
{
	const char *e = getenv(name);
	return e ? atoi(e) : dflt;
}

inline long long env_i64(const char *name, long long dflt)
{
	const char *e = getenv(name);
	return e ? atoll(e) : dflt;
}

inline double env_double(const char *name, double dflt)
{
	const char *e = getenv(name);
	return e ? atof(e) : dflt;
}

inline Switches parse_switches()
{
	Switches w;
	w.verbose = getenv("SPP_VERBOSE") != nullptr;
	const char *threads = getenv("SPP_PLAN_THREADS");
	w.plan_threads = threads ? std::max(1, atoi(threads)) : 0;
	w.plan_min_work = std::max<int64_t>(1, env_i64("SPP_PLAN_MIN_WORK", int64_t(1) << 18));

	w.dense_sched = env_int("SPP_DENSE_SCHED", 1);
	w.fused = env_int("SPP_FUSED", 1);
	w.aux_reserve_cus = env_int("SPP_AUX_RESERVE_CUS", 32);
	w.tile_444 = env_int("SPP_TILE_444", 0);
	w.dense_la = env_int("SPP_DENSE_LA", 0);
	w.la_chain_mask = env_int("SPP_LA_CHAIN_MASK", 1);
	w.la_g2 = env_int("SPP_LA_G2", 0);
	w.la_bulk_acquire = env_int("SPP_LA_BULK_ACQUIRE", 1);
	w.la_slots = env_i64("SPP_LA_SLOTS", 0);
	w.la_trace = env_int("SPP_LA_TRACE", 0);
	w.tail_rows = env_int("SPP_DENSE_TAIL", 1) ? env_int("SPP_TAIL_ROWS", 44) : 0;
	w.tail_mask = env_int("SPP_TAIL_MASK", 1);
	w.tail_order_beta = env_double("SPP_TAIL_ORDER_BETA", 0.0);
	w.tail_early = env_int("SPP_TAIL_EARLY", 1);
	w.tail_timeout_ticks = env_i64("SPP_TAIL_TIMEOUT_TICKS", WAIT_TICKS_DEFAULT);
	w.tail_trace = env_int("SPP_TAIL_TRACE", 0);
	w.trsv_chain = env_int("SPP_TRSV_CHAIN", 2);
	w.trsv_mform = env_int("SPP_TRSV_MFORM", 1);

	w.sacc_ulm = env_int("SPP_SACC_ULM", 1) != 0;
	w.sacc_factored = env_int("SPP_SACC_FACTORED", 1) != 0;
	w.sacc_tile = std::max<int64_t>(1, env_i64("SPP_SACC_TILE", 4));
	w.sacc_tile_cols = env_i64("SPP_SACC_TILE_COLS", -2);
	w.sacc_xcd = env_int("SPP_SACC_XCD", 1);
	w.sacc_chunk = env_int("SPP_SACC_CHUNK", 1);
	w.schur_cam_order = env_int("SPP_SCHUR_CAM_ORDER", 1);
	w.backsubst_fused = env_int("SPP_BACKSUBST_FUSED", 1);
	w.schur_side = env_int("SPP_SCHUR_SIDE", 1);
	w.lm_stream = env_int("SPP_LM_STREAM", 1);

	w.mid_front_max = std::max(128, std::min(MID_FRONT_MAX, env_int("SPP_MID_FRONT_MAX", 320)));
	const char *ordering = getenv("SPP_ORDERING");
	w.ordering = !ordering ? ORDERING_AUTO : (!strcmp(ordering, "nd") ? ORDERING_ND : ORDERING_AMD);
	w.amalg_small = env_i64("SPP_AMALG_SMALL", 32);
	w.amalg_zeros = env_double("SPP_AMALG_ZEROS", 0.12);
	w.amalg_relax_h = env_i64("SPP_AMALG_RELAX_H", 96);
	w.amalg_zeros_small = env_double("SPP_AMALG_ZEROS_SMALL", 0.2);
	w.sparse_teams = env_int("SPP_SPARSE_TEAMS", 1) != 0;
	w.sparse_team_max = std::max(1, std::min(64, env_int("SPP_SPARSE_TEAM_MAX", 40)));
	w.sparse_team_cols = std::max(8, std::min(256, env_int("SPP_SPARSE_TEAM_COLS", 16)));
	w.sparse_dag = env_int("SPP_SPARSE_DAG", 1);
	w.dag_split = env_int("SPP_DAG_SPLIT", 1);
	w.dag_timeout_ticks = env_i64("SPP_DAG_TIMEOUT_TICKS", WAIT_TICKS_DEFAULT);
	w.dag_trace = env_int("SPP_DAG_TRACE", 0);
	return w;
}

inline const Switches &switches()
{
	static const Switches w = parse_switches();
	return w;
}

}
```

Measured before the change: 1.319 billion block-nnz/s.

## Overlap factor status readback on side stream and skip final stream sync

After the dense Schur factorization, the info status copy is issued on a side stream behind an event, so the host only waits for that small copy rather than draining the main stream after backsubstitution. The final stream synchronize in factor_solve_device is skipped when this async path is active. The chain-error flag becomes a mapped, coherent host buffer written with system-scope atomics, which removes a D2H memcpy. Drains are added at state-changing entry points, and deferred error checks at D2H points; the risk is that work is still in flight when control returns to the caller.

Measured after the change: 1.334 billion block-nnz/s (median of 6 runs). 1.01x the previous value.

```diff
diff --git a/include/spp_hip.h b/include/spp_hip.h
--- a/include/spp_hip.h
+++ b/include/spp_hip.h
@@ -65,6 +65,7 @@
 #define SPP_INFO_S_CLEAR        20
 #define SPP_INFO_S_DEVICE_PTR   21
 #define SPP_INFO_ASM_HUB_CHUNK   22
+#define SPP_INFO_SOLVE_ASYNC    23
 int spp_get_info(const spp_ctx *ctx, int what, int64_t *out);
 int spp_get_ordering(const spp_ctx *ctx, int64_t *h_order);
 int64_t spp_sparse_fronts(const spp_ctx *ctx, int64_t capacity, int32_t *h, int32_t *w, int32_t *pad, int32_t *cls, int32_t *level,
diff --git a/slam_plus_plus_amd/api.py b/slam_plus_plus_amd/api.py
--- a/slam_plus_plus_amd/api.py
+++ b/slam_plus_plus_amd/api.py
@@ -11,7 +11,7 @@
 FLAG_PROFILE = 1
 INFO = dict(MODE=0, N=1, NNZB=2, NVALS=3, FACTOR_NNZ=4, FACTOR_FLOPS=5, N_REDUCED=6, N_POSES=7,
             N_LANDMARKS=8, SCHUR_PAIRS=9, N_OBS=10, SOLVE_BYTES=11, N_SUPERNODES=12, N_LEVELS=13, S_LD=14, S_NNZB=15, DENSE_STREAMED=16,
-            LM_STREAM=17, BS_GROUPS=18, SCHUR_SIDE=19, S_CLEAR=20, S_DEVICE_PTR=21, ASM_HUB_CHUNK=22)
+            LM_STREAM=17, BS_GROUPS=18, SCHUR_SIDE=19, S_CLEAR=20, S_DEVICE_PTR=21, ASM_HUB_CHUNK=22, SOLVE_ASYNC=23)
 PHASES = ["permute", "schur_inv", "schur_gemm", "schur_rhs", "factor", "trisolve", "backsubst", "assemble", "total"]
 
 EXPORTS = [
diff --git a/slam_plus_plus_amd/csrc/spp_api.cpp b/slam_plus_plus_amd/csrc/spp_api.cpp
--- a/slam_plus_plus_amd/csrc/spp_api.cpp
+++ b/slam_plus_plus_amd/csrc/spp_api.cpp
@@ -77,6 +77,14 @@
 
 }
 
+static void ctx_drain(spp_ctx *ctx)
+{
+	(void)hipStreamSynchronize(ctx->stream);
+	if(ctx->side_stream)
+		(void)hipStreamSynchronize(ctx->side_stream);
+	ctx->status_pending = false;
+}
+
 #define SPP_TRY(ctx) try {
 #define SPP_CATCH(ctx) } catch(const spp::Error &e) { if(ctx) (ctx)->last_error = e.what(); return e.code; } \
 	catch(const std::bad_alloc &) { if(ctx) (ctx)->last_error = "host allocation failed"; return SPP_E_NOMEM; } \
@@ -131,7 +139,7 @@
 		return SPP_E_BADARG;
 	SPP_TRY(ctx)
 	(void)hipSetDevice(ctx->device);
-	(void)hipStreamSynchronize(ctx->stream);
+	ctx_drain(ctx);
 	ctx->schur.release_all();
 	sparse_release(ctx);
 	assemble_release(ctx);
@@ -185,6 +193,11 @@
 		(void)hipEventDestroy(ctx->side_ev[0]);
 		(void)hipEventDestroy(ctx->side_ev[1]);
 	}
+	for(int i = 0; i < 2; ++ i)
+		if(ctx->status_ev[i])
+			(void)hipEventDestroy(ctx->status_ev[i]);
+	if(ctx->h_status)
+		(void)hipHostFree(ctx->h_status);
 	if(ctx->dense.h_chain_err)
 		(void)hipHostFree(ctx->dense.h_chain_err);
 	if(ctx->h_staging)
@@ -236,7 +249,7 @@
 {
 	if(!ctx)
 		return SPP_E_BADARG;
-	(void)hipStreamSynchronize(ctx->stream);
+	ctx_drain(ctx);
 	if(ctx->own_stream && ctx->stream)
 		(void)hipStreamDestroy(ctx->stream);
 	ctx->stream = (hipStream_t)hip_stream;
@@ -282,6 +295,7 @@
 	SPP_REQUIRE(col_ptr[0] == 0 && col_ptr[nb] >= nb, SPP_E_BADARG, "spp_analyze: column pointers must start at 0 and hold every diagonal block");
 	SPP_HIP_CHECK(hipSetDevice(ctx->device));
 	ctx->mode = -1;
+	ctx_drain(ctx);
 	VClock clk("spp_analyze");
 	Structure st;
 	st.nb = nb;
@@ -407,6 +421,7 @@
 	case SPP_INFO_LM_STREAM: *out = (ctx->mode == SPP_MODE_SCHUR) ? ctx->schur.lm_stream_last : 0; break;
 	case SPP_INFO_BS_GROUPS: *out = (ctx->mode == SPP_MODE_SCHUR) ? ctx->schur.n_bs : 0; break;
 	case SPP_INFO_SCHUR_SIDE: *out = (ctx->mode == SPP_MODE_SCHUR) ? ctx->schur.side_last : 0; break;
+	case SPP_INFO_SOLVE_ASYNC: *out = (ctx->mode == SPP_MODE_SCHUR) ? ctx->schur.async_last : 0; break;
 	case SPP_INFO_S_CLEAR: *out = (ctx->mode == SPP_MODE_SCHUR) ? ctx->schur.clear_last : 0; break;
 	case SPP_INFO_S_DEVICE_PTR: *out = (ctx->mode == SPP_MODE_SCHUR) ? (int64_t)(uintptr_t)ctx->schur.S.p : 0; break;
 	case SPP_INFO_ASM_HUB_CHUNK: *out = ASM_HUB_CHUNK; break;
@@ -664,8 +679,10 @@
 	if(ctx->mode == SPP_MODE_SCHUR) {
 		SPP_REQUIRE(ctx->shard_world == 1, SPP_E_STATE,
 			"sharded ctx: use spp_schur_form / all-reduce / spp_schur_finish");
-		if(!ctx->schur.S.p || ctx->schur.S.cap < (size_t)schur_buffer_doubles(ctx))
+		if(!ctx->schur.S.p || ctx->schur.S.cap < (size_t)schur_buffer_doubles(ctx)) {
 			ctx->schur.unlisted_dirty = true;
+			ctx_drain(ctx);
+		}
 		ctx->schur.S.reserve((size_t)schur_buffer_doubles(ctx));
 		schur_form(ctx, d_vals, d_rhs, ctx->schur.S.p, true);
 		ret = schur_finish(ctx, d_vals, ctx->schur.S.p, d_rhs);
@@ -673,7 +690,8 @@
 		ret = sparse_factor_solve(ctx, d_vals, d_rhs);
 	phase_end(ctx, SPP_PHASE_TOTAL);
 	phases_collect(ctx);
-	SPP_HIP_CHECK(hipStreamSynchronize(ctx->stream));
+	if(!(ctx->mode == SPP_MODE_SCHUR && ctx->schur.async_last))
+		SPP_HIP_CHECK(hipStreamSynchronize(ctx->stream));
 	dense_chain_check(ctx);
 	return ret;
 	SPP_CATCH(ctx)
@@ -695,6 +713,7 @@
 		return ret;
 	SPP_HIP_CHECK(hipMemcpyAsync(h_rhs, ctx->d_rhs.p, ctx->st.n * sizeof(double), hipMemcpyDeviceToHost, ctx->stream));
 	SPP_HIP_CHECK(hipStreamSynchronize(ctx->stream));
+	dense_chain_check(ctx);
 	return SPP_OK;
 	SPP_CATCH(ctx)
 }
@@ -1064,6 +1083,7 @@
 	SPP_HIP_CHECK(hipSetDevice(ctx->device));
 	SPP_HIP_CHECK(hipMemcpyAsync(h_dst, d_src, bytes, hipMemcpyDeviceToHost, ctx->stream));
 	SPP_HIP_CHECK(hipStreamSynchronize(ctx->stream));
+	dense_chain_check(ctx);
 	return SPP_OK;
 	SPP_CATCH(ctx)
 }
diff --git a/slam_plus_plus_amd/csrc/spp_dense.hip b/slam_plus_plus_amd/csrc/spp_dense.hip
--- a/slam_plus_plus_amd/csrc/spp_dense.hip
+++ b/slam_plus_plus_amd/csrc/spp_dense.hip
@@ -534,6 +534,11 @@
 }
 
 
+__device__ __forceinline__ void chain_raise(int *err)
+{
+	__hip_atomic_store(err, 1, __ATOMIC_RELAXED, __HIP_MEMORY_SCOPE_SYSTEM);
+}
+
 __global__ __launch_bounds__(256)
 void trsv_back_chain_kernel(const double *__restrict__ R, int64_t ld, int64_t n, int nblk,
 	const double *__restrict__ tinv_all, const double *__restrict__ y, double *xout, int *flags, int epoch, int *err)
@@ -571,7 +576,7 @@
 		__syncthreads();
 		if(!ok) {
 			if(tid == 0)
-				*err = 1;
+				chain_raise(err);
 			return;
 		}
 		if(tid < NB)
@@ -717,7 +722,7 @@
 			lds_barrier();
 			if(!ok[slot]) {
 				if(tid == 0)
-					*err = 1;
+					chain_raise(err);
 				alive = false;
 				return;
 			}
@@ -800,7 +805,7 @@
 					++ spins;
 				}
 				if(spins >= SPIN_MAX)
-					*err = 1;
+					chain_raise(err);
 				const double xr = uv - part_sum(tid);
 				xs[b & 1][tid] = xr;
 				pay_store(xpay + (size_t)b * NB + tid, xr, K);
@@ -859,7 +864,7 @@
 				++ spins;
 			}
 			if(spins >= SPIN_MAX)
-				*err = 1;
+				chain_raise(err);
 			zs[tid] = wv - part_sum(tid);
 		}
 		lds_barrier();
@@ -1632,8 +1637,21 @@
 int dense_info_fetch(spp_ctx *ctx, bool *dag_aborted)
 {
 	int h_info[4] = {0, 0, 0, 0};
-	SPP_HIP_CHECK(hipMemcpyAsync(h_info, ctx->dense.info.p, 4 * sizeof(int), hipMemcpyDeviceToHost, ctx->stream));
+	dense_info_copy_on(ctx, ctx->stream, h_info);
 	SPP_HIP_CHECK(hipStreamSynchronize(ctx->stream));
+	return dense_info_eval(ctx, h_info, dag_aborted);
+}
+
+void dense_info_copy_on(spp_ctx *ctx, hipStream_t st, int *h_status4)
+{
+	SPP_HIP_CHECK(hipMemcpyAsync(h_status4, ctx->dense.info.p, 4 * sizeof(int), hipMemcpyDeviceToHost, st));
+}
+
+int dense_info_eval(spp_ctx *ctx, const int *h_status4, bool *dag_aborted, bool drain_first)
+{
+	const int h_info[4] = {h_status4[0], h_status4[1], h_status4[2], h_status4[3]};
+	if(drain_first && (h_info[0] | h_info[2] | h_info[3]))
+		SPP_HIP_CHECK(hipStreamSynchronize(ctx->stream));
 	if(h_info[3]) {
 		SPP_HIP_CHECK(hipMemset(ctx->dense.info.p + 3, 0, sizeof(int)));
 		sparse_dag_disable(ctx);
@@ -1729,6 +1747,15 @@
 	return info ? SPP_NOT_POSDEF : SPP_OK;
 }
 
+static void chain_err_ensure(DenseWork &dw)
+{
+	if(dw.h_chain_err)
+		return;
+	SPP_HIP_CHECK(hipHostMalloc((void**)&dw.h_chain_err, sizeof(int), hipHostMallocMapped | hipHostMallocCoherent));
+	*dw.h_chain_err = 0;
+	SPP_HIP_CHECK(hipHostGetDevicePointer((void**)&dw.d_chain_err, dw.h_chain_err, 0));
+}
+
 void dense_potrs_upper(spp_ctx *ctx, const double *d_R, int64_t n, int64_t ld, double *d_b)
 {
 	const int64_t nblk = (n + NB - 1) / NB;
@@ -1745,10 +1772,7 @@
 			dw.trsv_pay.reserve(need);
 			SPP_HIP_CHECK(hipMemsetAsync(dw.trsv_pay.p, 0, dw.trsv_pay.cap * sizeof(double), s));
 		}
-		if(!dw.h_chain_err) {
-			SPP_HIP_CHECK(hipHostMalloc((void**)&dw.h_chain_err, sizeof(int), hipHostMallocDefault));
-			*dw.h_chain_err = 0;
-		}
+		chain_err_ensure(dw);
 		++ dw.epoch;
 		const unsigned long long K = (2ull * (unsigned long long)dw.epoch + 1ull) * 0x9E3779B97F4A7C15ull;
 		TrsvPay *xpay = (TrsvPay*)dw.trsv_pay.p, *wpay = xpay + (size_t)nblk * NB;
@@ -1760,12 +1784,11 @@
 				SPP_HIP_CHECK(hipFuncSetAttribute((const void*)trsv_m_kernel, hipFuncAttributeMaxDynamicSharedMemorySize, TRSVM_LDS_DOUBLES * (int)sizeof(double)));
 			hipLaunchKernelGGL(trsv_m_kernel, dim3((unsigned)nblk - 1, 8), dim3(1024), TRSVM_LDS_DOUBLES * sizeof(double), s, d_R, ld, n, dw.tinv_all.p, dw.trsv_m.p);
 			hipLaunchKernelGGL((trsv_back_chain2_kernel<8, true>), dim3((unsigned)nblk + 1), dim3(512), 0, s,
-				d_R, ld, n, (int)nblk, dw.tinv_all.p, dw.trsv_m.p, d_b, xpay, wpay, K, dw.info.p + 1);
+				d_R, ld, n, (int)nblk, dw.tinv_all.p, dw.trsv_m.p, d_b, xpay, wpay, K, dw.d_chain_err);
 		} else
 			hipLaunchKernelGGL((trsv_back_chain2_kernel<8, false>), dim3((unsigned)nblk + 1), dim3(512), 0, s,
-				d_R, ld, n, (int)nblk, dw.tinv_all.p, (const double*)nullptr, d_b, xpay, wpay, K, dw.info.p + 1);
+				d_R, ld, n, (int)nblk, dw.tinv_all.p, (const double*)nullptr, d_b, xpay, wpay, K, dw.d_chain_err);
 		SPP_HIP_CHECK(hipGetLastError());
-		SPP_HIP_CHECK(hipMemcpyAsync(dw.h_chain_err, dw.info.p + 1, sizeof(int), hipMemcpyDeviceToHost, s));
 		return;
 	}
 	if(use_chain && nblk > 1 && nblk <= 1024) {
@@ -1775,16 +1798,12 @@
 			SPP_HIP_CHECK(hipMemsetAsync(dw.flags.p, 0, (size_t)nblk * sizeof(int), s));
 			dw.epoch = 0;
 		}
-		if(!dw.h_chain_err) {
-			SPP_HIP_CHECK(hipHostMalloc((void**)&dw.h_chain_err, sizeof(int), hipHostMallocDefault));
-			*dw.h_chain_err = 0;
-		}
+		chain_err_ensure(dw);
 		++ dw.epoch;
 		hipLaunchKernelGGL(trsv_back_chain_kernel, dim3((unsigned)nblk), dim3(256), 0, s, d_R, ld, n, (int)nblk,
-			dw.tinv_all.p, d_b, dw.xtmp.p, dw.flags.p, (int)dw.epoch, dw.info.p + 1);
+			dw.tinv_all.p, d_b, dw.xtmp.p, dw.flags.p, (int)dw.epoch, dw.d_chain_err);
 		SPP_HIP_CHECK(hipGetLastError());
 		SPP_HIP_CHECK(hipMemcpyAsync(d_b, dw.xtmp.p, n * sizeof(double), hipMemcpyDeviceToDevice, s));
-		SPP_HIP_CHECK(hipMemcpyAsync(dw.h_chain_err, dw.info.p + 1, sizeof(int), hipMemcpyDeviceToHost, s));
 		return;
 	}
 	for(int64_t k = nblk; k > 0;) {
diff --git a/slam_plus_plus_amd/csrc/spp_internal.h b/slam_plus_plus_amd/csrc/spp_internal.h
--- a/slam_plus_plus_amd/csrc/spp_internal.h
+++ b/slam_plus_plus_amd/csrc/spp_internal.h
@@ -235,6 +235,7 @@
 	bool unlisted_dirty = true;
 	bool side_pending = false, side_padded = false;
 	int side_last = 0, clear_last = 0;
+	int async_last = 0;
 	void release_all();
 };
 
@@ -262,6 +263,7 @@
 	DevBuf<double> trsv_pay;
 	uint64_t epoch = 0;
 	int *h_chain_err = nullptr;
+	int *d_chain_err = nullptr;
 	hipStream_t aux = nullptr;
 	hipEvent_t ev[2] = {nullptr, nullptr};
 	DevBuf<int> sync;
@@ -300,6 +302,9 @@
 	bool own_stream = false;
 	hipStream_t side_stream = nullptr;
 	hipEvent_t side_ev[2] = {nullptr, nullptr};
+	hipEvent_t status_ev[2] = {nullptr, nullptr};
+	int *h_status = nullptr;
+	bool status_pending = false;
 	std::string last_error;
 	int mode = -1;
 	int shard_rank = 0, shard_world = 1;
@@ -402,6 +407,8 @@
 int dense_potrf_upper(spp_ctx *ctx, double *d_A, int64_t n, int64_t ld, bool keep_inverses);
 bool dense_potrf_upper_enqueue(spp_ctx *ctx, double *d_A, int64_t n, int64_t ld, bool info_reset = true);
 int dense_info_fetch(spp_ctx *ctx, bool *dag_aborted = nullptr);
+void dense_info_copy_on(spp_ctx *ctx, hipStream_t st, int *h_status4);
+int dense_info_eval(spp_ctx *ctx, const int *h_status4, bool *dag_aborted = nullptr, bool drain_first = false);
 void dense_potrs_upper(spp_ctx *ctx, const double *d_R, int64_t n, int64_t ld, double *d_b);
 void dense_aux_park(int device, hipStream_t s);
 void dense_factor_steps(spp_ctx *ctx, double *d_A, int64_t ld, int64_t n, int64_t rows, int64_t ncols,
diff --git a/slam_plus_plus_amd/csrc/spp_schur.hip b/slam_plus_plus_amd/csrc/spp_schur.hip
--- a/slam_plus_plus_amd/csrc/spp_schur.hip
+++ b/slam_plus_plus_amd/csrc/spp_schur.hip
@@ -1098,6 +1098,18 @@
 	SPP_HIP_CHECK(hipStreamCreateWithFlags(&ctx->side_stream, hipStreamNonBlocking));
 	SPP_HIP_CHECK(hipEventCreateWithFlags(&ctx->side_ev[0], hipEventDisableTiming));
 	SPP_HIP_CHECK(hipEventCreateWithFlags(&ctx->side_ev[1], hipEventDisableTiming));
+}
+
+static void status_ensure(spp_ctx *ctx)
+{
+	side_stream_ensure(ctx);
+	if(ctx->h_status)
+		return;
+	if(!ctx->status_ev[0])
+		SPP_HIP_CHECK(hipEventCreateWithFlags(&ctx->status_ev[0], hipEventDisableTiming));
+	if(!ctx->status_ev[1])
+		SPP_HIP_CHECK(hipEventCreateWithFlags(&ctx->status_ev[1], hipEventDisableTiming));
+	SPP_HIP_CHECK(hipHostMalloc((void**)&ctx->h_status, 4 * sizeof(int), hipHostMallocDefault));
 }
 
 static void side_stream_join(spp_ctx *ctx)
@@ -1228,6 +1240,15 @@
 	const int64_t ld = sp.ld;
 	double *xcol;
 	side_stream_join(ctx);
+	const bool early = !sp.sparse_S && switches().solve_async != 0 && !(ctx->flags & SPP_FLAG_PROFILE) && !stream_capturing(s);
+	sp.async_last = early ? 1 : 0;
+	if(early) {
+		status_ensure(ctx);
+		if(ctx->status_pending) {
+			SPP_HIP_CHECK(hipStreamSynchronize(ctx->side_stream));
+			ctx->status_pending = false;
+		}
+	}
 	if(sp.sparse_S) {
 		xcol = S + sp.s_st.nvals;
 		const int ret = sparse_factor_solve(ctx, S, xcol);
@@ -1247,6 +1268,13 @@
 				sp.unlisted_dirty = false;
 		}
 		sp.side_padded = false;
+		if(early) {
+			SPP_HIP_CHECK(hipEventRecord(ctx->status_ev[0], s));
+			SPP_HIP_CHECK(hipStreamWaitEvent(ctx->side_stream, ctx->status_ev[0], 0));
+			dense_info_copy_on(ctx, ctx->side_stream, ctx->h_status);
+			SPP_HIP_CHECK(hipEventRecord(ctx->status_ev[1], ctx->side_stream));
+			ctx->status_pending = true;
+		}
 		phase_end(ctx, SPP_PHASE_FACTOR);
 		xcol = S + sp.n_red * ld;
 		phase_begin(ctx, SPP_PHASE_TRISOLVE);
@@ -1281,6 +1309,11 @@
 			sp.nc, sp.pose_rbase.p, xcol, d_rhs);
 	phase_end(ctx, SPP_PHASE_BACKSUBST);
 	SPP_HIP_CHECK(hipGetLastError());
+	if(early) {
+		SPP_HIP_CHECK(hipEventSynchronize(ctx->status_ev[1]));
+		ctx->status_pending = false;
+		return dense_info_eval(ctx, ctx->h_status, nullptr, true) ? SPP_NOT_POSDEF : SPP_OK;
+	}
 	if(!sp.sparse_S && dense_info_fetch(ctx))
 		return SPP_NOT_POSDEF;
 	return SPP_OK;
diff --git a/slam_plus_plus_amd/csrc/spp_switches.h b/slam_plus_plus_amd/csrc/spp_switches.h
--- a/slam_plus_plus_amd/csrc/spp_switches.h
+++ b/slam_plus_plus_amd/csrc/spp_switches.h
@@ -46,6 +46,7 @@
 	int schur_cam_order;
 	int backsubst_fused;
 	int schur_side;
+	int solve_async;
 	int lm_stream;
 
 	int mid_front_max;
@@ -117,6 +118,7 @@
 	w.schur_cam_order = env_int("SPP_SCHUR_CAM_ORDER", 1);
 	w.backsubst_fused = env_int("SPP_BACKSUBST_FUSED", 1);
 	w.schur_side = env_int("SPP_SCHUR_SIDE", 1);
+	w.solve_async = env_int("SPP_SOLVE_ASYNC", 1);
 	w.lm_stream = env_int("SPP_LM_STREAM", 1);
 
 	w.mid_front_max = std::max(128, std::min(MID_FRONT_MAX, env_int("SPP_MID_FRONT_MAX", 320)));
```
